# turpaultn/DCASE2019_task4

Measured on AMD Instinct MI355X. Metric: 10-s clips/sec mean-teacher train step (64-mel x 628), higher is better.
Workload: dtype f32

## Files before the change

dcase2019_task4_amd/_lib.py:

```python
import ctypes as C
import os

_HERE = os.path.dirname(os.path.abspath(__file__))
LIB_PATH = os.path.join(_HERE, "libdcase_sed_mi355.so")
if os.environ.get("SED_LIB"):
    if os.environ.get("SED_ALLOW_VARIANT") != "1":
        raise ImportError("SED_LIB is set but SED_ALLOW_VARIANT != 1: refusing to load a variant build of the library")
    LIB_PATH = os.environ["SED_LIB"]


class SedError(RuntimeError):
    pass


class SedDims(C.Structure):
    _fields_ = [("B", C.c_int32), ("T", C.c_int32), ("F", C.c_int32), ("C", C.c_int32), ("H", C.c_int32),
                ("nclass", C.c_int32), ("n_layers_rnn", C.c_int32), ("p_drop", C.c_float),
                ("bn_eps", C.c_float), ("bn_momentum", C.c_float), ("dtype", C.c_int32)]


FORK_CALLBACK = C.CFUNCTYPE(None, C.c_void_p)
DTYPE_F32, DTYPE_BF16, DTYPE_BF16X3, DTYPE_F16 = 0, 1, 2, 3
FFT_F64, FFT_F32 = 0, 1
FFT_DTYPES = {"f64": FFT_F64, "float64": FFT_F64, "f32": FFT_F32, "float32": FFT_F32}
DTYPES = {"f32": DTYPE_F32, "fp32": DTYPE_F32, "float32": DTYPE_F32, "bf16": DTYPE_BF16, "bfloat16": DTYPE_BF16,
          "bf16x3": DTYPE_BF16X3, "f16": DTYPE_F16, "fp16": DTYPE_F16, "float16": DTYPE_F16}


class SedStepState(C.Structure):
    _fields_ = [("global_step", C.c_int64), ("opt_step", C.c_int64), ("rampup_length", C.c_int64),
                ("base_seed", C.c_uint64), ("seed_student", C.c_uint64), ("seed_teacher", C.c_uint64),
                ("lr", C.c_double), ("beta1", C.c_double), ("beta2", C.c_double), ("eps", C.c_double),
                ("ema_decay", C.c_double), ("max_cons_cost", C.c_double),
                ("cons_weight", C.c_float), ("ema_alpha", C.c_float), ("adam_step_size", C.c_float),
                ("adam_sqrt_bc2", C.c_float)]


_P = C.c_void_p
_SIGS = {
    "sed_last_error": (C.c_char_p, []),
    "sed_resample": (C.c_int, [C.c_void_p, C.c_int, C.c_int, C.c_double, C.c_void_p, C.c_int, C.c_int, C.c_void_p, C.c_void_p,
                               C.c_int, C.c_void_p]),
    "sed_scaler_stats": (C.c_int, [C.c_void_p, C.c_longlong, C.c_int, C.c_void_p, C.c_void_p]),
    "sed_postprocess": (C.c_int, [C.c_void_p, C.c_int, C.c_int, C.c_int, C.c_float, C.c_int, C.c_void_p, C.c_void_p,
                                  C.c_void_p, C.c_int, C.c_void_p]),
    "sed_stitch_decode_ws_bytes": (C.c_size_t, [C.c_longlong, C.c_int, C.c_int]),
    "sed_stitch_tile_frames": (C.c_int, []),
    "sed_stitch_decode": (C.c_int, [_P, _P, _P, C.c_int, C.c_int, C.c_int, C.c_int, C.c_int, _P, _P, _P, _P, _P, _P, C.c_longlong,
                                    _P, C.c_size_t, _P, _P]),
    "sed_stitch_sweep_ws_bytes": (C.c_size_t, [C.c_longlong, C.c_int, C.c_int, C.c_int]),
    "sed_stitch_sweep_point_group": (C.c_int, []),
    "sed_stitch_sweep": (C.c_int, [_P, _P, _P, C.c_int, C.c_int, C.c_int, C.c_int, C.c_int, C.c_int, _P, _P, _P, _P, _P,
                                   C.c_longlong, _P, C.c_size_t, _P, _P]),
    "sed_event_counts": (C.c_int, [_P, C.c_int, C.c_int, C.c_int, C.c_int, _P, _P, C.c_double, C.c_double, _P, _P, _P, _P, _P, _P,
                                   C.c_double, C.c_double, C.c_double, _P, _P, _P, _P, _P, _P]),
    "sed_psds_counts": (C.c_int, [_P, C.c_int, C.c_int, C.c_int, C.c_int, _P, _P, C.c_double, C.c_double, _P, _P, _P, _P, _P, _P,
                                  C.c_double, C.c_double, C.c_double, _P, _P, _P, _P]),
    "sed_long_score_ws_bytes": (C.c_size_t, [C.c_longlong, C.c_longlong, C.c_int, C.c_int]),
    "sed_long_tile_events": (C.c_int, []),
    "sed_long_event_counts": (C.c_int, [_P, _P, C.c_double, C.c_double, _P, _P, C.c_longlong, _P, _P, _P, C.c_longlong, C.c_int,
                                        C.c_int, C.c_double, C.c_double, C.c_double, _P, _P, _P, _P, _P, _P, C.c_size_t, _P]),
    "sed_long_psds_counts": (C.c_int, [_P, _P, C.c_double, C.c_double, _P, _P, C.c_longlong, _P, _P, _P, C.c_longlong, C.c_int,
                                       C.c_int, C.c_double, C.c_double, C.c_double, _P, _P, _P, _P, C.c_size_t, _P]),
    "sed_long_sweep_ws_bytes": (C.c_size_t, [C.c_longlong, C.c_longlong, C.c_int, C.c_int, C.c_int]),
    "sed_long_sweep_event_counts": (C.c_int, [_P, _P, C.c_double, C.c_double, _P, _P, C.c_longlong, _P, _P, _P, C.c_longlong,
                                              C.c_int, C.c_int, C.c_int, C.c_double, C.c_double, C.c_double, _P, _P, _P, _P, _P,
                                              _P, C.c_size_t, _P]),
    "sed_long_sweep_psds_counts": (C.c_int, [_P, _P, C.c_double, C.c_double, _P, _P, C.c_longlong, _P, _P, _P, C.c_longlong,
                                             C.c_int, C.c_int, C.c_int, C.c_double, C.c_double, C.c_double, _P, _P, _P, _P,
                                             C.c_size_t, _P]),
    "sed_weak_counts": (C.c_int, [_P, _P, C.c_int, C.c_int, _P, C.c_int, _P, _P]),
    "sed_version": (C.c_int, []),
    "sed_param_count": (C.c_int, [C.POINTER(SedDims)]),
    "sed_param_layout": (C.c_int, [C.POINTER(SedDims), C.POINTER(C.c_int64)]),
    "sed_crnn_ctx_bytes": (C.c_size_t, [C.POINTER(SedDims)]),
    "sed_crnn_bwd_ws_bytes": (C.c_size_t, [C.POINTER(SedDims)]),
    "sed_crnn_forward": (C.c_int, [C.POINTER(SedDims), _P, _P, _P, _P, C.c_int, C.c_int, _P, _P, C.c_size_t, _P, _P, _P]),
    "sed_crnn_moments": (C.c_int, [C.POINTER(SedDims), _P, _P, C.c_size_t, _P]),
    "sed_crnn_backward": (C.c_int, [C.POINTER(SedDims), _P, _P, _P, _P, C.c_size_t, _P, _P, _P, _P, C.c_size_t, C.c_int, _P]),
    "sed_crnn_buffers_init": (C.c_int, [C.POINTER(SedDims), _P, C.c_size_t, _P, C.c_size_t, _P]),
    "sed_crnn_ctx_view": (C.c_int, [C.POINTER(SedDims), C.c_char_p, C.POINTER(C.c_size_t), C.POINTER(C.c_size_t)]),
    "sed_mt_loss": (C.c_int, [C.POINTER(SedDims), _P, _P, _P, _P, _P, C.c_int, C.c_int, C.c_int, C.c_int, _P, _P, _P, _P, _P]),
    "sed_mt_loss_backward": (C.c_int, [C.POINTER(SedDims), _P, _P, _P, _P, C.c_size_t, _P, _P, _P, C.c_int, C.c_int, C.c_int,
                                       C.c_int, _P, C.c_int, _P, _P, _P, _P, _P, C.c_size_t, C.c_int, _P]),
    "sed_mt_step_backward": (C.c_int, [C.POINTER(SedDims), _P, _P, _P, _P, C.c_size_t, _P, _P, _P, _P, _P, C.c_int, C.c_int, C.c_int,
                                       C.c_int, _P, C.c_int, _P, _P, _P, _P, _P, C.c_size_t, C.c_int, _P]),
    "sed_p2p_buffer_bytes": (C.c_size_t, [C.c_longlong]),
    "sed_p2p_alloc": (C.c_int, [C.c_size_t, C.c_int, C.POINTER(C.c_void_p), _P, C.POINTER(C.c_int)]),
    "sed_p2p_open": (C.c_int, [_P, C.POINTER(C.c_void_p)]),
    "sed_p2p_close": (C.c_int, [_P]),
    "sed_p2p_free": (C.c_int, [_P]),
    "sed_p2p_can_access": (C.c_int, [C.c_int]),
    "sed_p2p_errors": (C.c_int, [_P, C.POINTER(C.c_uint)]),
    "sed_p2p_configure": (C.c_int, [_P, C.c_double, _P, C.c_int]),
    "sed_p2p_allreduce": (C.c_int, [_P, C.c_longlong, C.c_int, C.c_int, C.POINTER(C.c_void_p), C.c_longlong, C.c_int, _P]),
    "sed_adam_ema": (C.c_int, [C.c_int64, _P, _P, _P, _P, _P, _P, C.c_float, _P]),
    "sed_ema_update": (C.c_int, [C.c_int64, _P, _P, C.c_float, _P]),
    "sed_step_state_init": (C.c_int, [_P, C.c_uint64, C.c_int64, C.c_double, C.c_double, C.c_double, C.c_double,
                                      C.c_double, C.c_double, _P]),
    "sed_step_state_advance": (C.c_int, [_P, _P]),
    "sed_step_state_update": (C.c_int, [_P, C.c_uint64, C.c_double, C.c_int, _P]),
    "sed_step_state_set_global_step": (C.c_int, [_P, C.c_int64, _P]),
    "sed_stream_prepare": (C.c_int, [_P]),
    "sed_stream_release": (C.c_int, [_P]),
    "sed_crnn_fork_callback": (C.c_int, [_P, _P, _P]),
    "sed_mel_spec_ws_bytes": (C.c_size_t, [C.c_int, C.c_int, C.c_int, C.c_int, C.c_int]),
    "sed_mel_spec": (C.c_int, [_P, C.c_int, C.c_int, C.c_int, C.c_int, _P, _P, C.c_int, _P, _P, C.c_size_t, _P]),
    "sed_mel_tables": (C.c_int, [C.c_int, _P, _P, C.c_int, _P, C.c_size_t, _P]),
    "sed_mel_frames": (C.c_int, [_P, C.c_int, C.c_int, C.c_int, C.c_int, _P, C.c_int, _P, _P, C.c_size_t, C.c_int, C.c_int, _P]),
    "sed_seed_advance": (C.c_int, [_P, _P]),
    "sed_logmel_transform_ws_bytes": (C.c_size_t, [C.c_int]),
    "sed_logmel_transform": (C.c_int, [_P, C.c_int, C.c_int, C.c_int, C.c_int, _P, _P, _P, _P, _P, _P, C.c_size_t, C.c_int, _P]),
    "sed_gather_logmel_transform": (C.c_int, [_P, _P, _P, C.c_int, C.c_int, _P, C.c_int, C.c_int, C.c_int, _P, _P, _P, _P, _P,
                                              _P, C.c_int, _P, _P, C.c_size_t, C.c_int, _P]),
    "sed_gather_window_logmel_transform": (C.c_int, [_P, _P, _P, C.c_int, C.c_int, _P, C.c_int, C.c_int, C.c_int, C.c_int, _P, _P,
                                                     _P, _P, _P, _P, _P, _P, C.c_int, C.c_int, _P, _P, C.c_size_t, C.c_int, _P]),
    "sed_batch_augment": (C.c_int, [_P, _P, _P, _P, C.c_int, C.c_int, C.c_int, C.c_int, C.c_int, _P, _P, _P, _P]),
    "sed_selftest": (C.c_int, [_P, _P, C.c_size_t, _P]),
    "sed_debug_set": (C.c_int, [C.c_int]),
    "sed_build_flags": (C.c_int, []),
    "sed_kernel_replay": (C.c_int, [C.c_char_p, C.POINTER(SedDims), _P, _P, _P, _P, C.c_size_t, _P, _P, C.c_size_t, _P]),
}

_lib = None


def exported_symbols():
    return sorted(_SIGS)


def lib():
    global _lib
    if _lib is None:
        if not os.path.exists(LIB_PATH):
            raise SedError(
                f"{LIB_PATH} not found: build it with `python -c 'import __graft_entry__ as g; g.build()'` "
                "or `make -C dcase2019_task4_amd/csrc` (needs hipcc). There is no CPU fallback.")
        l = C.CDLL(LIB_PATH)
        for name, (res, args) in _SIGS.items():
            fn = getattr(l, name)
            fn.restype = res
            fn.argtypes = args
        _lib = l
        if os.environ.get("SED_DEBUG"):
            l.sed_debug_set(int(os.environ["SED_DEBUG"]))
    return _lib


def scratch(nbytes, device):
    import torch
    t = torch.empty(nbytes, device=device, dtype=torch.uint8)
    if os.environ.get("SED_POISON") == "1" and nbytes:
        t.fill_(0xFF)
    return t


def check(status, what):
    if status != 0:
        msg = lib().sed_last_error()
        raise SedError(f"{what} failed with status {status}: {msg.decode() if msg else ''}")


def ptr(t):
    if t is None:
        return None
    return C.c_void_p(t.data_ptr())


def stream_ptr():
    import torch
    return C.c_void_p(torch.cuda.current_stream().cuda_stream)


def make_dims(B, T, F=64, C_=64, H=64, nclass=10, n_layers_rnn=2, p_drop=0.5, bn_eps=1e-3, bn_momentum=0.99, dtype=DTYPE_F32):
    return SedDims(B, T, F, C_, H, nclass, n_layers_rnn, p_drop, bn_eps, bn_momentum, dtype)


def param_layout(dims):
    l = lib()
    n = l.sed_param_count(C.byref(dims))
    if n <= 0:
        raise SedError(f"sed_param_count: {l.sed_last_error().decode()}")
    off = (C.c_int64 * (n + 1))()
    check(l.sed_param_layout(C.byref(dims), off), "sed_param_layout")
    return list(off)
```

dcase2019_task4_amd/crnn.py:

```python
import ctypes as C
import warnings

import torch
import torch.nn as nn

from . import _lib


class GLU(nn.Module):

    def __init__(self, input_num):
        super().__init__()
        self.sigmoid = nn.Sigmoid()
        self.linear = nn.Linear(input_num, input_num)

    def forward(self, x):
        lin = self.linear(x.permute(0, 2, 3, 1)).permute(0, 3, 1, 2)
        return lin * self.sigmoid(x)


class ContextGating(nn.Module):

    def __init__(self, input_num):
        super().__init__()
# ... 150 lines not shown
        self._C, self._H = int(self.cnn.nb_filters[-1]), int(n_RNN_cell)
        self._dtype = _lib.DTYPE_F32
        self.set_mfma_dtype(mfma_dtype)
        self._flat = None
        self._bn_flat = None
        self._bn_tracked = None
        self._layout = None
        self._flat_gen = 0
        self._last_ctx = None
        self._seed_base = None
        self._seed_calls = 0

    def load_cnn(self, parameters):
        self.cnn.load(parameters)
        if not self.train_cnn:
            for param in self.cnn.parameters():
                param.requires_grad = False

    def load(self, filename=None, parameters=None):
        if filename is not None:
            parameters = torch.load(filename)
        if parameters is None:
            raise NotImplementedError("load is a filename or a list of parameters (state_dict)")
        self.cnn.load(parameters=parameters["cnn"])
        self.rnn.load_state_dict(parameters["rnn"])
        self.dense.load_state_dict(parameters["dense"])
        if "dense_softmax" in parameters and self.attention:
            self.dense_softmax.load_state_dict(parameters["dense_softmax"])

    def state_dict(self, destination=None, prefix='', keep_vars=False):
        sd = {"cnn": self.cnn.state_dict(destination=destination, prefix=prefix, keep_vars=keep_vars),
              "rnn": self.rnn.state_dict(destination=destination, prefix=prefix, keep_vars=keep_vars),
              "dense": self.dense.state_dict(destination=destination, prefix=prefix, keep_vars=keep_vars)}
        if self.attention:
            sd["dense_softmax"] = self.dense_softmax.state_dict(destination=destination, prefix=prefix, keep_vars=keep_vars)
        return sd

    def save(self, filename):
        torch.save({k: v for k, v in self.state_dict().items()}, filename)

    def set_mfma_dtype(self, name):
        if name not in _lib.DTYPES:
            raise ValueError(f"mfma_dtype must be one of {sorted(_lib.DTYPES)}, got {name!r}")
        self._dtype = _lib.DTYPES[name]
        return self

    def make_dims(self, B, T, F=64, p_drop=None):
        if not self.hot_path:
            raise _lib.SedError("this CRNN configuration is outside the MI355X hot path (CRNN.hot_path is False): it runs on stock "
                                "torch operators through forward() only - no flat buffers, no fused step, no HIP inference")
        return _lib.make_dims(B, T, F, self._C, self._H, self._nclass, self._n_layers,
                              self._p_drop if p_drop is None else p_drop, 1e-3, 0.99, self._dtype)

    def _dims(self, x):
        B, _, T, F = x.shape
        return self.make_dims(B, T, F)

    def _bn_modules(self):
        return [getattr(self.cnn.cnn, f"batchnorm{i}") for i in range(3)]

    def flatten_parameters_(self, device=None):
        params = list(self.parameters())
        device = device if device is not None else params[0].device
        if self._layout is None:
            offs = _lib.param_layout(self.make_dims(1, 16, 64, 0.0))
            assert len(offs) == len(params) + 1, "parameter order does not match sed_param_layout"
            self._layout = [(offs[i], offs[i + 1], tuple(p.shape)) for i, p in enumerate(params)]
            for (o0, o1, shp), p in zip(self._layout, params):
                assert o1 - o0 == p.numel(), "parameter shape does not match sed_param_layout"
        ok = self._flat is not None and self._flat.device == device
        if ok:
            base = self._flat.data_ptr()
            for (o0, _, _), p in zip(self._layout, params):
                if p.data_ptr() != base + 4 * o0 or p.device != device or p.dtype != torch.float32:
                    ok = False
                    break
            bns = self._bn_modules()
            Cn = self._C
            for i, bn in enumerate(bns):
                if bn.running_mean.data_ptr() != self._bn_flat.data_ptr() + 4 * (2 * i) * Cn or \
                        bn.running_var.data_ptr() != self._bn_flat.data_ptr() + 4 * (2 * i + 1) * Cn or \
                        bn.num_batches_tracked.data_ptr() != self._bn_tracked.data_ptr() + 8 * i:
                    ok = False
                    break
        if ok:
            return
        with torch.no_grad():
            total = self._layout[-1][1]
            flat = torch.empty(total, device=device, dtype=torch.float32)
            for (o0, o1, shp), p in zip(self._layout, params):
                flat[o0:o1].copy_(p.data.reshape(-1).to(device=device, dtype=torch.float32))
                p.data = flat[o0:o1].view(shp)
                p.grad = None
            Cn = self._C
            bn_flat = torch.empty(3 * 2 * Cn, device=device, dtype=torch.float32)
            trk = torch.empty(3, device=device, dtype=torch.int64)
            for i, bn in enumerate(self._bn_modules()):
                bn_flat[(2 * i) * Cn:(2 * i + 1) * Cn].copy_(bn.running_mean.to(device))
                bn_flat[(2 * i + 1) * Cn:(2 * i + 2) * Cn].copy_(bn.running_var.to(device))
                trk[i] = bn.num_batches_tracked.to(device)
                bn._buffers["running_mean"] = bn_flat[(2 * i) * Cn:(2 * i + 1) * Cn]
                bn._buffers["running_var"] = bn_flat[(2 * i + 1) * Cn:(2 * i + 2) * Cn]
                bn._buffers["num_batches_tracked"] = trk[i]
            self._flat, self._bn_flat, self._bn_tracked = flat, bn_flat, trk
            self._flat_gen += 1

    def _next_seed(self, device):
        if self._seed_base is None:
            self._seed_base = int(torch.randint(0, 2 ** 62, (1,), dtype=torch.int64).item())
        self._seed_calls += 1
        s = (self._seed_base + 0x9E3779B97F4A7C15 * self._seed_calls) & 0x7FFFFFFFFFFFFFFF
        return torch.tensor([s], dtype=torch.int64, device=device)

    def forward(self, x, seed=None):
        if not self.hot_path:
            return self._stock_forward(x)
        if x.dim() != 4 or x.shape[1] != 1:
            raise ValueError(f"expected input [B, 1, T, F], got {tuple(x.shape)}")
        if not x.is_cuda:
            raise _lib.SedError("CRNN.forward needs a GPU tensor: the HIP path is the only path (no CPU fallback)")
        if x.shape[3] // 64 != 1 or x.shape[3] != 64:
            warnings.warn("Output shape is: {}".format((x.shape[0], x.shape[2] // 8, 64 * (x.shape[3] // 64))))
            raise NotImplementedError("hot path implements freq == 1 after pooling, i.e. 64 mel bins (CRNN.py:64-70)")
        x = x.contiguous().float()
        self.flatten_parameters_(x.device)
        use_drop = self.training and self._p_drop > 0
        seed_t = (seed if seed is not None else self._next_seed(x.device)) if use_drop else None
        params = list(self.parameters())
        strong, weak = _CRNNFunction.apply(self, x, self.training, seed_t, *params)
        return strong, weak

    def _stock_forward(self, x):
        if not self._warned_stock:
            self._warned_stock = True
            warnings.warn("CRNN: this configuration is outside the MI355X hot path (activation='glu', attention=True, 3 x 64 / 128 "
                          "filters, pooling (2,4) x 3, n_RNN_cell 64 / 256): running the reference graph on stock torch operators")
        x = self.cnn(x)
        bs, chan, frames, freq = x.size()
        if freq != 1:
            warnings.warn("Output shape is: {}".format((bs, frames, chan * freq)))
            x = x.permute(0, 2, 1, 3).contiguous().view(bs, frames, chan * freq)
        else:
            x = x.squeeze(-1).permute(0, 2, 1)
        x = self.dropout(self.rnn(x))
        strong = self.sigmoid(self.dense(x))
        if self.attention:
            sof = torch.clamp(self.softmax(self.dense_softmax(x)), min=1e-7, max=1)
            weak = (strong * sof).sum(1) / sof.sum(1)
        else:
            weak = strong.mean(1)
        return strong, weak

    def check_recurrence(self):
        if self._H == 256 and self._last_ctx is not None:
            n = int(self.ctx_view("gru_err").view(torch.int32)[0].item())
            if n:
                raise _lib.SedError(f"cluster GRU recurrence: {n} cross-workgroup waits timed out; the outputs are invalid")

    def ctx_view(self, name):
        cbuf, dims = self._last_ctx
        off, nb = C.c_size_t(), C.c_size_t()
        _lib.check(_lib.lib().sed_crnn_ctx_view(C.byref(dims), name.encode(), C.byref(off), C.byref(nb)), "sed_crnn_ctx_view")
        raw = cbuf[off.value:off.value + nb.value]
        if name in ("mom0", "stat1", "stat2"):
            return raw.view(torch.float64)
        if dims.dtype in (_lib.DTYPE_BF16, _lib.DTYPE_F16) and name in ("p0", "y1", "p1", "y2"):
            return raw.view(torch.bfloat16).float()
        return raw.view(torch.float32)
```

dcase2019_task4_amd/csrc/common.h:

```cpp
#pragma once
#include <hip/hip_runtime.h>
#include <stdint.h>
#include <stddef.h>
#include "../../include/dcase_sed.h"

typedef __attribute__((ext_vector_type(16))) float f32x16;
typedef __attribute__((ext_vector_type(4))) float f32x4;

#define SED_C 64
#define SED_HID 64
#define SED_WAVE 64

void sed_set_error(const char* fmt, ...);
#define SED_CHECK_ARG(cond, msg)                                   \
    do {                                                           \
        if (!(cond)) {                                             \
            sed_set_error("%s:%d: %s", __FILE__, __LINE__, msg);   \
            return SED_ERR_BAD_ARG;                                \
        }                                                          \
    } while (0)
#define SED_CHECK_HIP(expr)                                                                 \
    do {                                                                                    \
        hipError_t _e = (expr);                                                             \
        if (_e != hipSuccess) {                                                             \
            sed_set_error("%s:%d: %s -> %s", __FILE__, __LINE__, #expr, hipGetErrorString(_e)); \
            return SED_ERR_LAUNCH;                                                          \
        }                                                                                   \
    } while (0)
#define SED_CHECK_LAUNCH() SED_CHECK_HIP(hipGetLastError())
struct SedAttrOnce {
    bool done[64] = {};
    bool need() {
        int d = 0;
        if (hipGetDevice(&d) != hipSuccess || d < 0 || d >= 64) return true;
        if (done[d]) return false;
        done[d] = true;
        return true;
    }
};
#define SED_TRY(expr)               \
    do {                            \
        int _s = (expr);            \
        if (_s != SED_OK) return _s; \
    } while (0)

struct Geo {
    int B, T, F, C, H, NC, L;
    int mode;
    bool f16;
    bool generic;
    int H1, W1;
    int H2, W2;
    int T3;
    float p, eps, mom;
};
static inline Geo make_geo(const sed_dims* d) {
    Geo g;
    g.B = d->B; g.T = d->T; g.F = d->F; g.C = d->C; g.H = d->H; g.NC = d->nclass; g.L = d->n_layers_rnn;
    g.f16 = d->dtype == SED_DTYPE_F16;
    g.mode = g.f16 ? SED_DTYPE_BF16 : d->dtype;
    g.generic = !(d->C == 64 && d->H == 64 && d->dtype == SED_DTYPE_F32);
    g.H1 = g.T / 2; g.W1 = g.F / 4;
    g.H2 = g.H1 / 2; g.W2 = g.W1 / 4;
    g.T3 = g.H2 / 2;
    g.p = d->p_drop; g.eps = d->bn_eps; g.mom = d->bn_momentum;
    return g;
}
int sed_validate_dims(const sed_dims* d);

struct ParamOff {
    int64_t conv_w[3], conv_b[3], bn_g[3], bn_b[3], glu_w[3], glu_b[3];
    int64_t w_ih[2][2], w_hh[2][2], b_ih[2][2], b_hh[2][2];
    int64_t dense_w, dense_b, soft_w, soft_b;
    int64_t total;
    int count;
};
ParamOff make_param_off(const Geo& g, int64_t* offsets_out );

struct CtxLayout {
    size_t acc0;
    size_t mom0, wz0, wl0, bn0;
    size_t mompart;
    size_t wpkT1, wpkT2;
    size_t p0;
    size_t wpk1, y1, stat1, bn1, p1;
    size_t wpk2, y2, stat2, bn2, p2;
    size_t gates[2], out[2];
    size_t logits_s, strong_sv, weak_sv, den_sv;
    size_t mask0, mask1, mask2;
    size_t total;
};
CtxLayout make_ctx_layout(const Geo& g);

struct WsLayout {
    size_t d_out, dgi[2], dgh[2], hprev[2], d_in, heads_part;
    size_t dz2, dp1, dz1, dp0, dp2;
    size_t bwd_acc;
    size_t pad0;
    size_t gluacc1, gluacc2, coef[3], wg_part, de0, gemm_part;
    size_t total;
    int wgrad_blocks;
};
WsLayout make_ws_layout(const Geo& g);
#define SED_WGRAD_MAX_BLOCKS 256
#ifndef SED_GRU_SPLITK
#define SED_GRU_SPLITK 16
#endif
#define SED_GLUACC_N 4296
#define SED_WINO_OFF (9 * 4096)

__device__ __forceinline__ float wave_sum(float v) {
#pragma unroll
    for (int o = 32; o > 0; o >>= 1) v += __shfl_xor(v, o);
    return v;
}
__device__ __forceinline__ float wave_max(float v) {
#pragma unroll
    for (int o = 32; o > 0; o >>= 1) v = fmaxf(v, __shfl_xor(v, o));
    return v;
}
__device__ __forceinline__ void lds_barrier() { asm volatile("s_waitcnt lgkmcnt(0)\n\ts_barrier" ::: "memory"); }
__device__ __forceinline__ float rcp_fast(float x) { return __builtin_amdgcn_rcpf(x); }
__device__ __forceinline__ float sigmoidf_fast(float x) { return rcp_fast(1.0f + __expf(-x)); }
#define SED_NEG_LOG2E (-1.4426950408889634f)
__device__ __forceinline__ float sigmoid_from_scaled(float e) { return rcp_fast(1.0f + __builtin_amdgcn_exp2f(e)); }
struct TileWalk { int first, end, step; };
__device__ __forceinline__ TileWalk xcd_walk(int n_tiles) {
    const int w = blockIdx.x, g = (int)gridDim.x;
#ifndef SED_NO_XCD_ORDER
    if ((g & 7) == 0) {
        const int chunk = (n_tiles + 7) >> 3, lo = (w & 7) * chunk, hi = lo + chunk < n_tiles ? lo + chunk : n_tiles;
        return {lo + (w >> 3), hi, g >> 3};
    }
#endif
    return {w, n_tiles, g};
}
extern int g_sed_debug;

__device__ __forceinline__ f32x16 mfma32(float a, float b, f32x16 c) {
    return __builtin_amdgcn_mfma_f32_32x32x2f32(a, b, c, 0, 0, 0);
}
__device__ __forceinline__ int mfma32_row(int r, int lane) { return (r & 3) + 8 * (r >> 2) + 4 * (lane >> 5); }


#ifdef SED_TS
#define SED_TS_DEFINE(tag)                                                                                          \
    static __device__ unsigned long long g_ts[1024 * 16];                                                           \
    extern "C" int sed_debug_ts_##tag(unsigned long long* out, int n) {                                             \
        return (int)hipMemcpyFromSymbol(out, HIP_SYMBOL(g_ts), sizeof(unsigned long long) * (n < 1024 * 16 ? n : 1024 * 16)); \
    }
#define TS(k) do { if (threadIdx.x == 0 && blockIdx.x < 1024 && blockIdx.y == 0) g_ts[blockIdx.x * 16 + (k)] = wall_clock64(); } while (0)
#define TSC(k) do { if (threadIdx.x == 0 && blockIdx.x < 1024 && blockIdx.y == 0) g_ts[blockIdx.x * 16 + (k)] = clock64(); } while (0)
#else
#define SED_TS_DEFINE(tag)
#define TS(k) do { } while (0)
#define TSC(k) do { } while (0)
#endif
```

dcase2019_task4_amd/csrc/crnn.hip:

```cpp
#include <stdarg.h>
#include <map>
#include <mutex>
#include <utility>
#include <stdio.h>
#include <string.h>
#include "common.h"
#include "kernels.h"
#include "gkernels.h"
#include "rnn.h"

static thread_local char g_err[512] = "";
void sed_set_error(const char* fmt, ...) {
    va_list ap;
    va_start(ap, fmt);
    vsnprintf(g_err, sizeof(g_err), fmt, ap);
    va_end(ap);
}
extern "C" const char* sed_last_error(void) { return g_err; }
extern "C" int sed_version(void) { return 100; }
int g_sed_debug = 0;
extern "C" int sed_debug_set(int flags) { const int old = g_sed_debug; g_sed_debug = flags; return old; }

int sed_validate_dims(const sed_dims* d) {
    SED_CHECK_ARG(d != nullptr, "null dims");
    if (d->F != 64 || (d->C != 64 && d->C != 128) || (d->H != 64 && d->H != 256) ||
        (d->dtype != SED_DTYPE_F32 && d->dtype != SED_DTYPE_BF16 && d->dtype != SED_DTYPE_BF16X3 && d->dtype != SED_DTYPE_F16)) {
        sed_set_error("supported: F = 64, C in {64, 128}, H in {64, 256}, dtype in {f32, bf16, bf16x3, f16} (got F=%d C=%d H=%d dtype=%d)",
                      d->F, d->C, d->H, d->dtype);
        return SED_ERR_UNSUPPORTED;
    }
    SED_CHECK_ARG(d->B >= 1 && d->T >= 16, "need B >= 1 and T >= 16");
    SED_CHECK_ARG(d->nclass >= 1 && d->nclass <= 16, "nclass must be in [1, 16]");
    SED_CHECK_ARG(d->n_layers_rnn == 1 || d->n_layers_rnn == 2, "n_layers_rnn must be 1 or 2");
    SED_CHECK_ARG(d->p_drop >= 0.f && d->p_drop < 1.f, "p_drop must be in [0, 1)");
    SED_CHECK_ARG((int64_t)d->B * d->T * d->F * d->C < (1ll << 31), "batch too large for 32-bit pixel indices");
    return SED_OK;
}

ParamOff make_param_off(const Geo& g, int64_t* out) {
    ParamOff P;
    int64_t o = 0;
    int k = 0;
    auto put = [&](int64_t& field, int64_t n) {
        field = o;
        if (out) out[k] = o;
        ++k;
        o += n;
    };
    for (int i = 0; i < 3; ++i) {
        const int cin = (i == 0) ? 1 : g.C;
        put(P.conv_w[i], (int64_t)g.C * cin * 9);
        put(P.conv_b[i], g.C);
        put(P.bn_g[i], g.C);
        put(P.bn_b[i], g.C);
        put(P.glu_w[i], (int64_t)g.C * g.C);
        put(P.glu_b[i], g.C);
    }
    for (int l = 0; l < g.L; ++l) {
        const int nin = (l == 0) ? g.C : 2 * g.H;
        for (int dir = 0; dir < 2; ++dir) {
            put(P.w_ih[l][dir], (int64_t)3 * g.H * nin);
            put(P.w_hh[l][dir], (int64_t)3 * g.H * g.H);
            put(P.b_ih[l][dir], 3 * g.H);
            put(P.b_hh[l][dir], 3 * g.H);
        }
    }
    put(P.dense_w, (int64_t)g.NC * 2 * g.H);
    put(P.dense_b, g.NC);
    put(P.soft_w, (int64_t)g.NC * 2 * g.H);
    put(P.soft_b, g.NC);
    P.total = o;
    P.count = k;
    if (out) out[k] = o;
    return P;
}

static inline size_t al(size_t x) { return (x + 255) & ~(size_t)255; }

CtxLayout make_ctx_layout(const Geo& g) {
    CtxLayout L;
    size_t o = 0;
    auto put = [&](size_t& f, size_t bytes) { f = o; o = al(o + bytes); };
    const size_t n0 = (size_t)g.B * g.H1 * g.W1 * 64, n1 = (size_t)g.B * g.H2 * g.W2 * 64, n2 = (size_t)g.B * g.T3 * 64;
    put(L.acc0, 320 * sizeof(double));
    L.mom0 = L.acc0; L.stat1 = L.acc0 + 64 * sizeof(double); L.stat2 = L.acc0 + 192 * sizeof(double);
    put(L.wz0, 64 * 12 * 4); put(L.wl0, 64 * 12 * 4); put(L.bn0, 256 * 4);
    put(L.mompart, (size_t)x_moments_parts(g) * 54 * sizeof(double));
    put(L.p0, n0 * 4);
    put(L.wpk1, (9 + 16) * 4096 * 4); put(L.wpkT1, (9 + 16) * 4096 * 4); put(L.y1, n0 * 4); put(L.bn1, 256 * 4); put(L.p1, n1 * 4);
    put(L.wpk2, (9 + 16) * 4096 * 4); put(L.wpkT2, (9 + 16) * 4096 * 4); put(L.y2, n1 * 4); put(L.bn2, 256 * 4); put(L.p2, n2 * 4);
    const size_t bt = (size_t)g.B * g.T3;
    for (int l = 0; l < 2; ++l) {
        put(L.gates[l], bt * 512 * 4); put(L.out[l], bt * 128 * 4);
    }
    put(L.logits_s, bt * g.NC * 4); put(L.strong_sv, bt * g.NC * 4);
    put(L.weak_sv, (size_t)g.B * g.NC * 4); put(L.den_sv, (size_t)g.B * g.NC * 4);
    auto mask_bytes = [](size_t Q) { return ((Q + 3) / 4) * 2 * 64 * sizeof(uint16_t); };
    put(L.mask0, mask_bytes((size_t)g.B * g.H1 * g.W1)); put(L.mask1, mask_bytes((size_t)g.B * g.H2 * g.W2));
    put(L.mask2, mask_bytes((size_t)g.B * g.T3));
    L.total = o;
    return L;
}

WsLayout make_ws_layout(const Geo& g) {
    WsLayout W;
    size_t o = 0;
    auto put = [&](size_t& f, size_t bytes) { f = o; o = al(o + bytes); };
    const size_t n0 = (size_t)g.B * g.H1 * g.W1 * 64, n1 = (size_t)g.B * g.H2 * g.W2 * 64, bt = (size_t)g.B * g.T3;
    put(W.d_out, bt * 128 * 4);
    for (int l = 0; l < 2; ++l) { put(W.dgi[l], bt * 384 * 4); put(W.dgh[l], bt * 384 * 4); put(W.hprev[l], bt * 128 * 4); }
    put(W.d_in, 2 * bt * 128 * 4); put(W.heads_part, (size_t)g.B * 2 * (g.NC * 128 + g.NC) * 4);
    put(W.dp2, 2 * bt * 64 * 4); put(W.dz2, n1 * 4); put(W.dp1, n1 * 4); put(W.dz1, n0 * 4); put(W.dp0, n0 * 4);
    put(W.pad0, 256 * sizeof(double)); W.coef[0] = 0; put(W.coef[1], 192 * 4); put(W.coef[2], 192 * 4);
    put(W.bwd_acc, (2 * SED_GLUACC_N + 2 * 64 * 10) * sizeof(double));
    W.gluacc1 = W.bwd_acc; W.gluacc2 = W.bwd_acc + SED_GLUACC_N * sizeof(double); W.de0 = W.bwd_acc + 2 * SED_GLUACC_N * sizeof(double);
    W.wgrad_blocks = SED_WGRAD_MAX_BLOCKS;
    put(W.wg_part, (size_t)W.wgrad_blocks * 9 * 4096 * 4);
    put(W.gemm_part, gemm_part_floats(4, SED_GRU_SPLITK, 192, 129) * 4);
    W.total = o;
    return W;
}

extern "C" int sed_param_count(const sed_dims* d) {
    if (sed_validate_dims(d) != SED_OK) return -1;
    const Geo g = make_geo(d);
    return make_param_off(g, nullptr).count;
}
extern "C" int sed_param_layout(const sed_dims* d, int64_t* offsets) {
    SED_TRY(sed_validate_dims(d));
    SED_CHECK_ARG(offsets != nullptr, "null offsets");
    const Geo g = make_geo(d);
    make_param_off(g, offsets);
    return SED_OK;
}
extern "C" size_t sed_crnn_ctx_bytes(const sed_dims* d) {
    if (sed_validate_dims(d) != SED_OK) return 0;
    const Geo g = make_geo(d);
    return g.generic ? gen_ctx_bytes(g) : make_ctx_layout(g).total;
}
extern "C" size_t sed_crnn_bwd_ws_bytes(const sed_dims* d) {
    if (sed_validate_dims(d) != SED_OK) return 0;
    const Geo g = make_geo(d);
    return g.generic ? gen_ws_bytes(g) : make_ws_layout(g).total;
}

extern "C" int sed_crnn_buffers_init(const sed_dims* d, void* ctx, size_t ctx_bytes, void* ws, size_t ws_bytes, void* stream) {
    SED_TRY(sed_validate_dims(d));
    const Geo g = make_geo(d);
    if (g.generic) return gen_buffers_init(g, ctx, ctx_bytes, ws, ws_bytes, (hipStream_t)stream);
    return SED_OK;
}

extern "C" int sed_crnn_ctx_view(const sed_dims* d, const char* name, size_t* offset, size_t* bytes) {
    SED_TRY(sed_validate_dims(d));
    SED_CHECK_ARG(name && offset && bytes, "null argument");
    const Geo g = make_geo(d);
    if (g.generic) return gen_ctx_view(g, name, offset, bytes);
    const CtxLayout L = make_ctx_layout(g);
    const size_t n0 = (size_t)g.B * g.H1 * g.W1 * 64 * 4, n1 = (size_t)g.B * g.H2 * g.W2 * 64 * 4, bt = (size_t)g.B * g.T3;
    struct { const char* n; size_t o, b; } tab[] = {
        {"mom0", L.mom0, 64 * 8}, {"wz0", L.wz0, 64 * 12 * 4}, {"wl0", L.wl0, 64 * 12 * 4}, {"bn0", L.bn0, 1024},
        {"p0", L.p0, n0}, {"y1", L.y1, n0}, {"stat1", L.stat1, 1024}, {"bn1", L.bn1, 1024}, {"p1", L.p1, n1},
        {"y2", L.y2, n1}, {"stat2", L.stat2, 1024}, {"bn2", L.bn2, 1024}, {"p2", L.p2, bt * 64 * 4},
        {"gates0", L.gates[0], bt * 512 * 4}, {"gates1", L.gates[1], bt * 512 * 4},
        {"gru0", L.out[0], bt * 128 * 4}, {"gru1", L.out[1], bt * 128 * 4},
        {"logits_s", L.logits_s, bt * g.NC * 4}, {"den", L.den_sv, (size_t)g.B * g.NC * 4},
    };
    for (auto& t : tab)
        if (strcmp(t.n, name) == 0) { *offset = t.o; *bytes = t.b; return SED_OK; }
    sed_set_error("sed_crnn_ctx_view: unknown buffer '%s'", name);
    return SED_ERR_BAD_ARG;
}

struct SideStream {
    hipStream_t s = nullptr;
    hipEvent_t fork = nullptr, join = nullptr;
    hipStream_t idle = nullptr;
    hipEvent_t idle_ev = nullptr;
    bool ok = false;
};
static std::mutex g_side_mu;
static std::map<std::pair<int, hipStream_t>, SideStream*> g_side;
struct ForkHook { void (*fn)(void*) = nullptr; void* user = nullptr; };
static std::map<std::pair<int, hipStream_t>, ForkHook> g_fork_hooks;
static SideStream& side_stream(hipStream_t caller) {
    static SideStream none;
    int dev = 0;
    if (hipGetDevice(&dev) != hipSuccess) return none;
    std::lock_guard<std::mutex> lk(g_side_mu);
    SideStream*& slot = g_side[std::make_pair(dev, caller)];
    if (slot == nullptr) {
        slot = new SideStream();
        if (hipStreamCreateWithFlags(&slot->s, hipStreamNonBlocking) == hipSuccess &&
            hipEventCreateWithFlags(&slot->fork, hipEventDisableTiming) == hipSuccess &&
            hipEventCreateWithFlags(&slot->join, hipEventDisableTiming) == hipSuccess &&
            hipStreamCreateWithFlags(&slot->idle, hipStreamNonBlocking) == hipSuccess &&
            hipEventCreateWithFlags(&slot->idle_ev, hipEventDisableTiming) == hipSuccess)
            slot->ok = true;
    }
    return *slot;
}
extern "C" int sed_stream_prepare(void* stream) {
    SideStream& sd = side_stream((hipStream_t)stream);
    if (!sd.ok) {
        sed_set_error("sed_stream_prepare: could not create the helper stream / events");
        return SED_ERR_LAUNCH;
    }
    return SED_OK;
}
extern "C" int sed_stream_release(void* stream) {
    int dev = 0;
    SED_CHECK_HIP(hipGetDevice(&dev));
    SideStream* sd = nullptr;
    {
        std::lock_guard<std::mutex> lk(g_side_mu);
        const auto key = std::make_pair(dev, (hipStream_t)stream);
        auto it = g_side.find(key);
        if (it != g_side.end()) { sd = it->second; g_side.erase(it); }
        g_fork_hooks.erase(key);
    }
    if (sd == nullptr) return SED_OK;
    int rc = SED_OK;
    auto note = [&](hipError_t e) { if (e != hipSuccess && rc == SED_OK) { sed_set_error("sed_stream_release: %s", hipGetErrorString(e)); rc = SED_ERR_LAUNCH; } };
    if (sd->s) { note(hipStreamSynchronize(sd->s)); note(hipStreamDestroy(sd->s)); }
    if (sd->idle) note(hipStreamDestroy(sd->idle));
    if (sd->fork) note(hipEventDestroy(sd->fork));
    if (sd->join) note(hipEventDestroy(sd->join));
    if (sd->idle_ev) note(hipEventDestroy(sd->idle_ev));
    delete sd;
    return rc;
}
extern "C" int sed_crnn_fork_callback(void* stream, void (*fn)(void*), void* user) {
    int dev = 0;
    SED_CHECK_HIP(hipGetDevice(&dev));
    std::lock_guard<std::mutex> lk(g_side_mu);
    const auto key = std::make_pair(dev, (hipStream_t)stream);
    if (fn == nullptr) { g_fork_hooks.erase(key); return SED_OK; }
    ForkHook& h = g_fork_hooks[key];
    h.fn = fn;
    h.user = user;
    return SED_OK;
}
int sed_fork_point(hipStream_t st) {
    int dev = 0;
    if (hipGetDevice(&dev) != hipSuccess) return SED_OK;
    ForkHook h;
    {
        std::lock_guard<std::mutex> lk(g_side_mu);
        auto it = g_fork_hooks.find(std::make_pair(dev, st));
        if (it == g_fork_hooks.end()) return SED_OK;
        h = it->second;
        g_fork_hooks.erase(it);
    }
    if (h.fn) h.fn(h.user);
    return SED_OK;
}
static SideFork side_fork(hipStream_t st) {
    SideStream& sd = side_stream(st);
    const bool ok = sd.ok && !(g_sed_debug & SED_DEBUG_NO_SIDE_STREAM);
    return SideFork{ok ? sd.s : st, sd.fork, sd.join, ok, false};
}

#define CTXF(off) ((float*)((char*)ctx + (off)))
#define CTXD(off) ((double*)((char*)ctx + (off)))
#define WSF(off) ((float*)((char*)ws + (off)))
#define WSD(off) ((double*)((char*)ws + (off)))
#define CTXM(off) ((uint16_t*)((char*)ctx + (off)))

static RnnBufs rnn_bufs(const CtxLayout& L, void* ctx, const WsLayout* Wp, void* ws) {
    RnnBufs R;
    R.p2 = CTXF(L.p2);
    for (int l = 0; l < 2; ++l) { R.out[l] = CTXF(L.out[l]); R.gates[l] = CTXF(L.gates[l]); }
    R.logits_s = CTXF(L.logits_s); R.strong_sv = CTXF(L.strong_sv); R.weak_sv = CTXF(L.weak_sv); R.den_sv = CTXF(L.den_sv);
    if (ws == nullptr) return R;
    const WsLayout& W = *Wp;
    R.d_out = WSF(W.d_out); R.d_in = WSF(W.d_in); R.dp2 = WSF(W.dp2); R.heads_part = WSF(W.heads_part);
    for (int l = 0; l < 2; ++l) { R.dgi[l] = WSF(W.dgi[l]); R.dgh[l] = WSF(W.dgh[l]); R.hprev[l] = WSF(W.hprev[l]); }
    R.gemm_part = WSF(W.gemm_part); R.gemm_part_floats = gemm_part_floats(4, SED_GRU_SPLITK, 192, 129); R.splitk = SED_GRU_SPLITK;
    R.zero = WSD(W.bwd_acc); R.n_zero = 2 * SED_GLUACC_N + 2 * 64 * 10;
    return R;
}

extern "C" int sed_crnn_forward(const sed_dims* d, const float* params, float* bn_running, int64_t* bn_tracked,
                                const float* x, int train, int update_bn, const uint64_t* seed_dev, void* ctx,
                                size_t ctx_bytes, float* strong, float* weak, void* stream) {
    SED_TRY(sed_validate_dims(d));
    SED_CHECK_ARG(params && bn_running && x && ctx, "sed_crnn_forward: null argument");
    const int mom_ready = (train & 4) ? 1 : 0;
    train &= 3;
    SED_CHECK_ARG((strong && weak) || (!strong && !weak && train), "sed_crnn_forward: strong and weak must both be given (or both NULL in train mode: heads deferred)");
    const Geo g = make_geo(d);
    const ParamOff P = make_param_off(g, nullptr);
    if (g.generic) {
        SED_CHECK_ARG(!(train && g.p > 0.f) || seed_dev, "sed_crnn_forward: dropout enabled but seed_dev is null");
        side_stream((hipStream_t)stream);
        return gen_forward(g, P, params, bn_running, bn_tracked, x, train | (mom_ready ? 4 : 0), update_bn, seed_dev, ctx, ctx_bytes, strong,
                           weak, (hipStream_t)stream);
    }
    const CtxLayout L = make_ctx_layout(g);
    if (ctx_bytes < L.total) {
        sed_set_error("sed_crnn_forward: ctx has %zu bytes, needs %zu", ctx_bytes, L.total);
        return SED_ERR_WORKSPACE;
    }
    const int use_drop = (train && g.p > 0.f) ? 1 : 0;
    SED_CHECK_ARG(!use_drop || seed_dev, "sed_crnn_forward: dropout enabled but seed_dev is null");
    hipStream_t st = (hipStream_t)stream;
    const int upd = (train && update_bn) ? 1 : 0;
    int64_t* trk[3] = {bn_tracked ? bn_tracked + 0 : nullptr, bn_tracked ? bn_tracked + 1 : nullptr,
                       bn_tracked ? bn_tracked + 2 : nullptr};

    const ConvPackArgs pack = {params + P.conv_w[1], params + P.conv_w[2], CTXF(L.wpk1), CTXF(L.wpk2),
                               train ? CTXF(L.wpkT1) : nullptr, train ? CTXF(L.wpkT2) : nullptr, CTXD(L.stat1), train ? 256 : 0};
    SED_TRY(launch_blk0_forward(g, x, params + P.conv_w[0], params + P.conv_b[0], params + P.bn_g[0], params + P.bn_b[0],
                                params + P.glu_w[0], params + P.glu_b[0], bn_running + 0, bn_running + 64, trk[0], train,
                                upd, seed_dev, CTXD(L.mom0), CTXD(L.mompart), CTXF(L.wz0), CTXF(L.wl0), CTXF(L.bn0), CTXF(L.p0),
                                use_drop ? CTXM(L.mask0) : nullptr, train ? &pack : nullptr, st, 0, nullptr, nullptr, mom_ready));
    if (!train) SED_TRY(launch_conv_pack(pack, st));
    const float* in = CTXF(L.p0);
    const size_t wpk[3] = {0, L.wpk1, L.wpk2}, yo[3] = {0, L.y1, L.y2}, so[3] = {0, L.stat1, L.stat2},
                 bo[3] = {0, L.bn1, L.bn2}, po[3] = {0, L.p1, L.p2}, mo[3] = {L.mask0, L.mask1, L.mask2};
    const int Hs[3] = {0, g.H1, g.H2}, Ws[3] = {0, g.W1, g.W2};
    for (int i = 1; i <= 2; ++i) {
        SED_TRY(launch_conv_fwd(in, CTXF(wpk[i]), params + P.conv_b[i], CTXF(yo[i]), train ? CTXD(so[i]) : nullptr, 0, g.B,
                                Hs[i], Ws[i], st));
        SED_TRY(launch_glu_pool_fwd(CTXF(yo[i]), CTXD(so[i]), (double)g.B * Hs[i] * Ws[i], params + P.bn_g[i], params + P.bn_b[i],
                                    bn_running + (2 * i) * 64, bn_running + (2 * i + 1) * 64, trk[i], train, upd, g.eps, g.mom,
                                    CTXF(bo[i]), params + P.glu_w[i], params + P.glu_b[i], CTXF(po[i]), g.B, Hs[i], Ws[i], i,
                                    use_drop, g.p, seed_dev, use_drop ? CTXM(mo[i]) : nullptr, st));
        in = CTXF(po[i]);
    }
    return rnn_forward(g, P, params, rnn_bufs(L, ctx, nullptr, nullptr), train, seed_dev, strong, weak, 0, st);
}

extern "C" int sed_crnn_moments(const sed_dims* d, const float* x, void* ctx, size_t ctx_bytes, void* stream) {
    SED_TRY(sed_validate_dims(d));
    SED_CHECK_ARG(x && ctx, "sed_crnn_moments: null argument");
    const Geo g = make_geo(d);
    double* mompart = nullptr;
    if (g.generic) {
        SED_TRY(gen_mompart(g, ctx, ctx_bytes, &mompart));
    } else {
        const CtxLayout L = make_ctx_layout(g);
        if (ctx_bytes < L.total) {
            sed_set_error("sed_crnn_moments: ctx has %zu bytes, needs %zu", ctx_bytes, L.total);
            return SED_ERR_WORKSPACE;
        }
        mompart = CTXD(L.mompart);
    }
    return launch_x_moments(g, x, mompart, nullptr, (hipStream_t)stream);
}

static int crnn_backward_impl(const sed_dims* d, const float* params, const float* x, const uint64_t* seed_dev,
                              void* ctx, size_t ctx_bytes, const float* d_strong, const float* d_weak, float* grads,
                              void* ws, size_t ws_bytes, int parts, void* stream, const HeadsLoss* hl,
                              const HeadsOut* ho = nullptr) {
    SED_TRY(sed_validate_dims(d));
    SED_CHECK_ARG(params && x && ctx && (hl || (d_strong && d_weak)) && grads && ws, "sed_crnn_backward: null argument");
    SED_CHECK_ARG(parts == 1 || parts == 2 || parts == 3 || parts == 5 || parts == 8,
                  "sed_crnn_backward: parts must be 1, 2, 3, 5 or 8");
    const Geo g = make_geo(d);
    const ParamOff P = make_param_off(g, nullptr);
    if (g.generic) {
        SED_CHECK_ARG(!(g.p > 0.f) || seed_dev, "sed_crnn_backward: dropout enabled but seed_dev is null");
        SideFork side0 = side_fork((hipStream_t)stream);
        return gen_backward(g, P, params, x, seed_dev, ctx, ctx_bytes, d_strong, d_weak, grads, ws, ws_bytes, parts, (hipStream_t)stream,
                            side0, hl, ho);
    }
    const CtxLayout L = make_ctx_layout(g);
    const WsLayout W = make_ws_layout(g);
    if (ctx_bytes < L.total || ws_bytes < W.total) {
        sed_set_error("sed_crnn_backward: ctx %zu/%zu bytes, ws %zu/%zu bytes", ctx_bytes, L.total, ws_bytes, W.total);
        return SED_ERR_WORKSPACE;
    }
    const int use_drop = (g.p > 0.f) ? 1 : 0;
    SED_CHECK_ARG(!use_drop || seed_dev, "sed_crnn_backward: dropout enabled but seed_dev is null");
    hipStream_t st = (hipStream_t)stream;
    const int BT = g.B * g.T3;
    SideFork side = side_fork(st);
    const RnnBwd rb = rnn_backward_plan(g, P, rnn_bufs(L, ctx, &W, ws), params, grads, seed_dev, hl, ho, parts, &side);
    SED_TRY(rnn_backward(rb, d_strong, d_weak, st));
    if (!(parts & 2)) return SED_OK;
    const size_t wpkT[3] = {0, L.wpkT1, L.wpkT2}, yo[3] = {0, L.y1, L.y2}, bo[3] = {0, L.bn1, L.bn2};
    const size_t pin[3] = {0, L.p0, L.p1}, gacc[3] = {0, W.gluacc1, W.gluacc2}, mo[3] = {L.mask0, L.mask1, L.mask2};
    const size_t dzo[3] = {0, W.dz1, W.dz2}, dpo[3] = {W.dp0, W.dp1, W.dp2};
    const int Hs[3] = {0, g.H1, g.H2}, Wd[3] = {0, g.W1, g.W2};
    if (!(parts & 1)) SED_CHECK_HIP(hipMemsetAsync(WSD(W.bwd_acc), 0, (2 * SED_GLUACC_N + 2 * 64 * 10) * sizeof(double), st));
    const bool fuse_prep = (g_sed_debug & (SED_DEBUG_DIRECT_CONV | SED_DEBUG_DIRECT_WGRAD)) == 0;
    BnBwdPrepArgs prep[3] = {};
    for (int i = 2; i >= 1; --i) {
        const BnBwdPrepArgs* pp = fuse_prep ? &prep[i] : nullptr;
        SED_TRY(launch_glu_pool_bwd(CTXF(yo[i]), CTXF(bo[i]), params + P.glu_w[i], params + P.glu_b[i], WSF(dpo[i]),
                                    i == 2 ? WSF(dpo[i]) + (size_t)BT * 64 : nullptr,
                                    WSF(dzo[i]), WSD(gacc[i]), 0, g.B, Hs[i], Wd[i], use_drop, g.p, CTXM(mo[i]),
                                    params + P.bn_g[i], WSF(W.coef[i]), grads + P.bn_g[i], grads + P.bn_b[i],
                                    grads + P.glu_w[i], grads + P.glu_b[i], grads + P.conv_b[i], fuse_prep ? &prep[i] : nullptr, st));
        SED_TRY(side.mark(st));
        if (i == 1) SED_TRY(side.start());
        SED_TRY(launch_conv_dgrad(WSF(dzo[i]), CTXF(yo[i]), WSF(W.coef[i]), CTXF(wpkT[i]), WSF(dpo[i - 1]), g.B, Hs[i], Wd[i], pp, st));
        if (i == 2) SED_TRY(side.start());
        SED_TRY(launch_conv_wgrad(WSF(dzo[i]), CTXF(yo[i]), WSF(W.coef[i]), CTXF(pin[i]), WSF(W.wg_part), W.wgrad_blocks,
                                  grads + P.conv_w[i], g.B, Hs[i], Wd[i], pp, side.s));
        if (i == 2) SED_TRY(rnn_deferred_weight_grads(rb));
        if (i == 1) SED_TRY(rnn_tail_weight_grads(rb));
    }
    SED_TRY(launch_blk0_backward(g, x, params + P.conv_w[0], params + P.conv_b[0], params + P.bn_g[0], params + P.bn_b[0],
                                 params + P.glu_w[0], CTXM(L.mask0), CTXD(L.mom0), CTXF(L.wz0), CTXF(L.wl0), CTXF(L.bn0),
                                 WSF(W.dp0), WSD(W.de0), 0, grads + P.conv_w[0], grads + P.conv_b[0], grads + P.bn_g[0],
                                 grads + P.bn_b[0], grads + P.glu_w[0], grads + P.glu_b[0], st));
    return side.join(st);
}

extern "C" int sed_crnn_backward(const sed_dims* d, const float* params, const float* x, const uint64_t* seed_dev,
                                 void* ctx, size_t ctx_bytes, const float* d_strong, const float* d_weak, float* grads,
                                 void* ws, size_t ws_bytes, int parts, void* stream) {
    return crnn_backward_impl(d, params, x, seed_dev, ctx, ctx_bytes, d_strong, d_weak, grads, ws, ws_bytes, parts, stream, nullptr);
}

extern "C" int sed_mt_loss_backward(const sed_dims* d, const float* params, const float* x, const uint64_t* seed_dev,
                                    void* ctx, size_t ctx_bytes, const float* strong_ema, const float* weak_ema,
                                    const float* target, int weak_lo, int weak_hi, int strong_lo, int strong_hi,
                                    sed_step_state* state_dev, int advance_state, float* losses, float* d_strong,
                                    float* d_weak, float* grads, void* ws, size_t ws_bytes, int parts, void* stream) {
    SED_CHECK_ARG(d && strong_ema && weak_ema && target && state_dev && losses, "sed_mt_loss_backward: null argument");
    SED_CHECK_ARG(parts == 1 || parts == 3 || parts == 5, "sed_mt_loss_backward: parts must include the heads (1, 3 or 5)");
    SED_CHECK_ARG(weak_lo >= 0 && weak_hi <= d->B && weak_lo <= weak_hi && strong_lo >= 0 && strong_hi <= d->B &&
                      strong_lo <= strong_hi, "sed_mt_loss_backward: bad mask range");
// ... 103 lines not shown
```

dcase2019_task4_amd/csrc/gcrnn.hip:

```cpp
#include <string.h>
#include "common.h"
#include "kernels.h"
#include "gkernels.h"
#include "gpack.h"
#include "rnn.h"

static inline size_t al(size_t x) { return (x + 255) & ~(size_t)255; }
static inline size_t esz(const Geo& g) { return g.mode == SED_DTYPE_BF16 ? 2 : 4; }
static inline int gru_splitk(const Geo& g) { return g.H == 64 ? SED_GRU_SPLITK : 4; }
static inline size_t gru_gemm_part_floats(const Geo& g) {
    int max_n = g.H > g.C ? g.H : g.C;
    if (g.L > 1 && 2 * g.H > max_n) max_n = 2 * g.H;
    return gemm_part_floats(4, gru_splitk(g), 3 * g.H, max_n + 1);
}

struct GCtx {
    size_t acc0, mom0, stat1, stat2;
    size_t wz0, wl0, bn0, mompart, p0;
    size_t wpk[3], wpkT[3], wg[3], wgT[3], bg[3], y[3], bn[3], p[3];
    size_t ph[2], yh[3];
    size_t gi[2], gates[2], out[2], whh[2], whhT[2];
    size_t wihT[2];
    size_t xch[2], epoch[2], err;
    size_t logits_s, strong_sv, weak_sv, den_sv;
    size_t mask[3];
    size_t sg0;
    size_t total;
};
static inline bool blk0_saves_gates(const Geo& g) { return g.mode == SED_DTYPE_BF16 && (g_sed_debug & SED_DEBUG_SAVED_GATES); }
static size_t mask_bytes(size_t Q, int C) { return ((Q + 3) / 4) * (size_t)(C / 32) * 64 * sizeof(uint16_t); }

static GCtx make_gctx(const Geo& g) {
    GCtx L;
    size_t o = 0;
    auto put = [&](size_t& f, size_t bytes) { f = o; o = al(o + bytes); };
    const size_t C = g.C, H = g.H, E = esz(g);
    const size_t n0 = (size_t)g.B * g.H1 * g.W1 * C, n1 = (size_t)g.B * g.H2 * g.W2 * C, n2 = (size_t)g.B * g.T3 * C;
    put(L.acc0, (64 + 4 * C) * sizeof(double));
    L.mom0 = L.acc0; L.stat1 = L.acc0 + 64 * sizeof(double); L.stat2 = L.stat1 + 2 * C * sizeof(double);
    put(L.wz0, C * 12 * 4); put(L.wl0, C * 12 * 4); put(L.bn0, 4 * C * 4);
    put(L.mompart, (size_t)x_moments_parts(g) * 54 * sizeof(double));
    put(L.p0, n0 * E);
    L.p[0] = L.p0;
    const size_t nn[3] = {0, n0, n1}, np[3] = {n0, n1, n2};
    for (int i = 1; i <= 2; ++i) {
        put(L.wpk[i], 9 * C * C * E); put(L.wpkT[i], 9 * C * C * E); put(L.wg[i], C * C * E); put(L.wgT[i], C * C * E);
        put(L.bg[i], C * 4); put(L.y[i], nn[i] * E); put(L.bn[i], 4 * C * 4); put(L.p[i], np[i] * (i == 2 ? 4 : E));
    }
    L.ph[0] = L.ph[1] = 0; L.yh[0] = L.yh[1] = L.yh[2] = 0;
    if (g.f16) { put(L.ph[0], n0 * 2); put(L.yh[1], n0 * 2); put(L.ph[1], n1 * 2); put(L.yh[2], n1 * 2); }
    const size_t bt = (size_t)g.B * g.T3;
    for (int l = 0; l < 2; ++l) {
        put(L.gi[l], g.H == 64 ? 0 : bt * 6 * H * 4);
        put(L.gates[l], bt * 8 * H * 4); put(L.out[l], bt * 2 * H * 4);
        put(L.whh[l], g.H == 64 ? 0 : 2 * 3 * H * H * 4); put(L.whhT[l], g.H == 64 ? 0 : 2 * 3 * H * H * 4);
        put(L.xch[l], g.H == 256 ? gclu_xch_bytes(g.B, g.H, 0) : 0); put(L.epoch[l], (size_t)2 * g.B * 4);
        put(L.wihT[l], g.H == 64 ? 0 : (size_t)(l == 0 ? C : 2 * H) * 6 * H * 4);
    }
    put(L.err, 256);
    put(L.logits_s, bt * g.NC * 4); put(L.strong_sv, bt * g.NC * 4);
    put(L.weak_sv, (size_t)g.B * g.NC * 4); put(L.den_sv, (size_t)g.B * g.NC * 4);
    put(L.mask[0], mask_bytes((size_t)g.B * g.H1 * g.W1, g.C)); put(L.mask[1], mask_bytes((size_t)g.B * g.H2 * g.W2, g.C));
    put(L.mask[2], mask_bytes((size_t)g.B * g.T3, g.C));
    put(L.sg0, g.mode == SED_DTYPE_BF16 ? mask_bytes((size_t)g.B * g.H1 * g.W1, g.C) * 8 : 0);
    L.total = o;
    return L;
}

struct GWs {
    size_t d_out, dgi[2], dgh[2], hprev[2], d_in, heads_part;
    size_t dp[3], dz[3], coef[3];
    size_t glu_part, glu_part2, de0, wg_part, gemm_part;
    size_t xch[2], epoch[2];
    size_t total;
};
static GWs make_gws(const Geo& g) {
    GWs W;
    size_t o = 0;
    auto put = [&](size_t& f, size_t bytes) { f = o; o = al(o + bytes); };
    const size_t C = g.C, H = g.H, bt = (size_t)g.B * g.T3;
    const size_t n0 = (size_t)g.B * g.H1 * g.W1 * C, n1 = (size_t)g.B * g.H2 * g.W2 * C;
    put(W.d_out, bt * 2 * H * 4);
    for (int l = 0; l < 2; ++l) { put(W.dgi[l], bt * 6 * H * 4); put(W.dgh[l], bt * 6 * H * 4); put(W.hprev[l], bt * 2 * H * 4); }
    put(W.d_in, 2 * bt * 2 * H * 4);
    put(W.heads_part, heads_part_floats(g.B, g.T3, g.NC, 2 * H) * 4);
    const size_t E = esz(g);
    put(W.dp[2], 2 * bt * C * 4); put(W.dz[2], n1 * E); put(W.dp[1], n1 * E); put(W.dz[1], n0 * E); put(W.dp[0], n0 * E);
    W.dz[0] = 0; W.coef[0] = 0;
    put(W.coef[1], 3 * C * 4); put(W.coef[2], 3 * C * 4);
    put(W.glu_part, (size_t)(g.mode == SED_DTYPE_BF16 ? bglu_bwd_grid(g.C, g.B, g.H1, g.W1) : gglu_bwd_grid(g.B, g.H1, g.W1)) * (C * C + 3 * C) * 4);
    put(W.glu_part2, (size_t)GPART_SLICES * (C * C + 3 * C) * 4);
    put(W.de0, 2 * C * 10 * sizeof(double));
    put(W.wg_part, (size_t)gwgrad_slabs(g.C) * 9 * C * C * 4);
    put(W.gemm_part, 2 * gru_gemm_part_floats(g) * 4);
    for (int l = 0; l < 2; ++l) { put(W.xch[l], g.H == 256 ? gclu_xch_bytes(g.B, g.H, 1) : 0); put(W.epoch[l], (size_t)2 * g.B * 4); }
    W.total = o;
    return W;
}

size_t gen_ctx_bytes(const Geo& g) { return make_gctx(g).total; }
size_t gen_ws_bytes(const Geo& g) { return make_gws(g).total; }

int gen_ctx_view(const Geo& g, const char* name, size_t* offset, size_t* bytes) {
    const GCtx L = make_gctx(g);
    const size_t C = g.C, H = g.H, bt = (size_t)g.B * g.T3;
    const size_t n0 = (size_t)g.B * g.H1 * g.W1 * C * esz(g), n1 = (size_t)g.B * g.H2 * g.W2 * C * esz(g);
    struct { const char* n; size_t o, b; } tab[] = {
        {"mom0", L.mom0, 64 * 8}, {"bn0", L.bn0, 4 * C * 4}, {"p0", L.p[0], n0}, {"y1", L.y[1], n0}, {"stat1", L.stat1, 2 * C * 8},
        {"bn1", L.bn[1], 4 * C * 4}, {"p1", L.p[1], n1}, {"y2", L.y[2], n1}, {"stat2", L.stat2, 2 * C * 8}, {"bn2", L.bn[2], 4 * C * 4},
        {"p2", L.p[2], bt * C * 4}, {"gates0", L.gates[0], bt * 8 * H * 4}, {"gates1", L.gates[1], bt * 8 * H * 4},
        {"gru0", L.out[0], bt * 2 * H * 4}, {"gru1", L.out[1], bt * 2 * H * 4}, {"logits_s", L.logits_s, bt * g.NC * 4},
        {"den", L.den_sv, (size_t)g.B * g.NC * 4}, {"gru_err", L.err, 4},
    };
    for (auto& t : tab)
        if (strcmp(t.n, name) == 0) { *offset = t.o; *bytes = t.b; return SED_OK; }
    sed_set_error("sed_crnn_ctx_view: unknown buffer '%s'", name);
    return SED_ERR_BAD_ARG;
}

int gen_buffers_init(const Geo& g, void* ctx, size_t ctx_bytes, void* ws, size_t ws_bytes, hipStream_t st) {
    if (ctx) {
        const GCtx L = make_gctx(g);
        if (ctx_bytes < L.total) { sed_set_error("sed_crnn_buffers_init: ctx has %zu bytes, needs %zu", ctx_bytes, L.total); return SED_ERR_WORKSPACE; }
        for (int l = 0; l < 2; ++l) {
            if (g.H == 256) SED_CHECK_HIP(hipMemsetAsync((char*)ctx + L.xch[l], 0, gclu_xch_bytes(g.B, g.H, 0), st));
            SED_CHECK_HIP(hipMemsetAsync((char*)ctx + L.epoch[l], 0, (size_t)2 * g.B * 4, st));
        }
        SED_CHECK_HIP(hipMemsetAsync((char*)ctx + L.err, 0, 256, st));
    }
    if (ws) {
        const GWs W = make_gws(g);
        if (ws_bytes < W.total) { sed_set_error("sed_crnn_buffers_init: ws has %zu bytes, needs %zu", ws_bytes, W.total); return SED_ERR_WORKSPACE; }
        for (int l = 0; l < 2; ++l) {
            if (g.H == 256) SED_CHECK_HIP(hipMemsetAsync((char*)ws + W.xch[l], 0, gclu_xch_bytes(g.B, g.H, 1), st));
            SED_CHECK_HIP(hipMemsetAsync((char*)ws + W.epoch[l], 0, (size_t)2 * g.B * 4, st));
        }
    }
    return SED_OK;
}

#define CTXF(off) ((float*)((char*)ctx + (off)))
#define CTXD(off) ((double*)((char*)ctx + (off)))
#define CTXV(off) ((void*)((char*)ctx + (off)))
#define CTXM(off) ((uint16_t*)((char*)ctx + (off)))
#define WSF(off) ((float*)((char*)ws + (off)))
#define WSD(off) ((double*)((char*)ws + (off)))

static RnnBufs rnn_bufs(const Geo& g, const GCtx& L, void* ctx, const GWs* Wp, void* ws) {
    RnnBufs R;
    R.p2 = CTXF(L.p[2]);
    R.logits_s = CTXF(L.logits_s); R.strong_sv = CTXF(L.strong_sv); R.weak_sv = CTXF(L.weak_sv); R.den_sv = CTXF(L.den_sv);
    R.err = (int*)CTXV(L.err);
    for (int l = 0; l < 2; ++l) {
        R.out[l] = CTXF(L.out[l]); R.gates[l] = CTXF(L.gates[l]);
        R.gi[l] = CTXF(L.gi[l]); R.wihT[l] = CTXF(L.wihT[l]); R.whh[l] = CTXV(L.whh[l]); R.whhT[l] = CTXV(L.whhT[l]);
        R.xch[l] = ws ? (void*)((char*)ws + Wp->xch[l]) : CTXV(L.xch[l]);
        R.epoch[l] = (unsigned int*)(ws ? (void*)((char*)ws + Wp->epoch[l]) : CTXV(L.epoch[l]));
    }
    if (ws == nullptr) return R;
    const GWs& W = *Wp;
    R.d_out = WSF(W.d_out); R.d_in = WSF(W.d_in); R.dp2 = WSF(W.dp[2]); R.heads_part = WSF(W.heads_part);
    for (int l = 0; l < 2; ++l) { R.dgi[l] = WSF(W.dgi[l]); R.dgh[l] = WSF(W.dgh[l]); R.hprev[l] = WSF(W.hprev[l]); }
    R.gemm_part = WSF(W.gemm_part); R.gemm_part_floats = R.gemm_part_stride = gru_gemm_part_floats(g); R.splitk = gru_splitk(g);
    R.zero = WSD(W.de0); R.n_zero = 2 * g.C * 10;
    return R;
}

int gen_mompart(const Geo& g, void* ctx, size_t ctx_bytes, double** out) {
    const GCtx L = make_gctx(g);
    if (ctx_bytes < L.total) {
        sed_set_error("sed_crnn_moments: ctx has %zu bytes, needs %zu", ctx_bytes, L.total);
        return SED_ERR_WORKSPACE;
    }
    *out = (double*)((char*)ctx + L.mompart);
    return SED_OK;
}

int gen_forward(const Geo& g, const ParamOff& P, const float* params, float* bn_running, int64_t* bn_tracked, const float* x,
                int train, int update_bn, const uint64_t* seed_dev, void* ctx, size_t ctx_bytes, float* strong, float* weak,
                hipStream_t st) {
    const int mom_ready = (train & 4) ? 1 : 0;
    train &= 3;
    const GCtx L = make_gctx(g);
    if (ctx_bytes < L.total) {
        sed_set_error("sed_crnn_forward: ctx has %zu bytes, needs %zu", ctx_bytes, L.total);
        return SED_ERR_WORKSPACE;
    }
    const int C = g.C, H = g.H;
    const int use_drop = (train && g.p > 0.f) ? 1 : 0;
    const int upd = (train && update_bn) ? 1 : 0;
    const bool keep_b16 = train && !(train & 2);
    int64_t* trk[3] = {bn_tracked ? bn_tracked + 0 : nullptr, bn_tracked ? bn_tracked + 1 : nullptr,
                       bn_tracked ? bn_tracked + 2 : nullptr};
    GenPackArgs pk = {};
    pk.C = C;
    pk.w1 = params + P.conv_w[1]; pk.w2 = params + P.conv_w[2];
    pk.wpk1 = CTXV(L.wpk[1]); pk.wpk2 = CTXV(L.wpk[2]);
    pk.wpkT1 = train ? CTXV(L.wpkT[1]) : nullptr; pk.wpkT2 = train ? CTXV(L.wpkT[2]) : nullptr;
    pk.glu_w1 = params + P.glu_w[1]; pk.glu_w2 = params + P.glu_w[2]; pk.glu_b1 = params + P.glu_b[1]; pk.glu_b2 = params + P.glu_b[2];
    pk.gamma1 = params + P.bn_g[1]; pk.gamma2 = params + P.bn_g[2]; pk.beta1 = params + P.bn_b[1]; pk.beta2 = params + P.bn_b[2];
    pk.wg1 = CTXV(L.wg[1]); pk.wg2 = CTXV(L.wg[2]);
    pk.wgT1 = train ? CTXV(L.wgT[1]) : nullptr; pk.wgT2 = train ? CTXV(L.wgT[2]) : nullptr;
    pk.bg1 = CTXF(L.bg[1]); pk.bg2 = CTXF(L.bg[2]);
    pk.zero = CTXD(L.stat1); pk.n_zero = train ? 4 * C : 0;
    pk.f16 = g.f16 ? 1 : 0;
    const bool aux_pack = train != 0;
    GenAuxPack aux = {};
    if (aux_pack) {
        aux.pk = pk; aux.mode = g.mode; aux.n_gnt = 0;
        if (H != 64)
            for (int l = 0; l < g.L && l < 2; ++l) {
                aux.gw0[l] = params + P.w_ih[l][0]; aux.gw1[l] = params + P.w_ih[l][1]; aux.gout[l] = CTXF(L.wihT[l]);
                aux.gR[l] = 3 * H; aux.gN[l] = (l == 0) ? C : 2 * H;
                aux.n_gnt = l + 1;
            }
        if (H == 256 && g.mode == SED_DTYPE_BF16)
            for (int l = 0; l < g.L && l < 2; ++l) {
                aux.rw0[l] = params + P.w_hh[l][0]; aux.rw1[l] = params + P.w_hh[l][1];
                aux.rwp[l] = CTXV(L.whh[l]); aux.rwpT[l] = CTXV(L.whhT[l]);
                aux.n_grec = l + 1;
            }
    } else {
        SED_TRY(launch_gen_pack(pk, g.mode, st));
    }

    SED_TRY(launch_blk0_forward(g, x, params + P.conv_w[0], params + P.conv_b[0], params + P.bn_g[0], params + P.bn_b[0],
                                params + P.glu_w[0], params + P.glu_b[0], bn_running + 0, bn_running + C, trk[0], train, upd,
                                seed_dev, CTXD(L.mom0), CTXD(L.mompart), CTXF(L.wz0), CTXF(L.wl0), CTXF(L.bn0),
                                g.f16 ? CTXF(L.ph[0]) : CTXF(L.p[0]),
                                use_drop ? CTXM(L.mask[0]) : nullptr, nullptr, st, 0, aux_pack ? &aux : nullptr,
                                (g.f16 && keep_b16) ? CTXV(L.p[0]) : nullptr, mom_ready,
                                (train && !(train & 2) && blk0_saves_gates(g)) ? CTXV(L.sg0) : nullptr));
    const size_t so[3] = {0, L.stat1, L.stat2};
    const int Hs[3] = {0, g.H1, g.H2}, Wd[3] = {0, g.W1, g.W2};
    auto bn_args = [&](int i) {
        GBnArgs bn;
        bn.stat = CTXD(so[i]); bn.N = (double)g.B * Hs[i] * Wd[i]; bn.gamma = params + P.bn_g[i]; bn.beta = params + P.bn_b[i];
        bn.run_mean = bn_running + (2 * i) * C; bn.run_var = bn_running + (2 * i + 1) * C; bn.tracked = trk[i];
        bn.train = train; bn.update = upd; bn.eps = g.eps; bn.momentum = g.mom; bn.bn = CTXF(L.bn[i]);
        return bn;
    };
    for (int i = 1; i <= 2; ++i) {
        const GBnArgs bn = bn_args(i);
        if (g.f16) {
            SED_TRY(launch_bconv_fwd(2, C, CTXV(L.ph[i - 1]), CTXV(L.wpk[i]), params + P.conv_b[i], CTXV(L.yh[i]),
                                     train ? CTXD(so[i]) : nullptr, g.B, Hs[i], Wd[i], st));
            SED_TRY(launch_bglu_fwd(C, CTXV(L.yh[i]), bn, params + P.glu_w[i], params + P.glu_b[i], i == 1 ? CTXV(L.ph[1]) : CTXV(L.p[2]),
                                    i == 1 ? 1 : 0, g.B, Hs[i], Wd[i], i, use_drop, g.p, seed_dev, use_drop ? CTXM(L.mask[i]) : nullptr,
                                    train ? CTXV(L.wg[i]) : nullptr, train ? CTXF(L.bg[i]) : nullptr, st, 1,
                                    (i == 1 && keep_b16) ? CTXV(L.p[1]) : nullptr, keep_b16 ? CTXV(L.y[i]) : nullptr));
            continue;
        }
        if (g.mode != SED_DTYPE_F32)
            SED_TRY(launch_bconv_fwd(g.mode == SED_DTYPE_BF16X3, C, CTXV(L.p[i - 1]), CTXV(L.wpk[i]), params + P.conv_b[i], CTXV(L.y[i]),
                                     train ? CTXD(so[i]) : nullptr, g.B, Hs[i], Wd[i], st));
        else
            SED_TRY(launch_gconv_fwd(C, CTXF(L.p[i - 1]), CTXV(L.wpk[i]), params + P.conv_b[i], CTXF(L.y[i]),
                                     train ? CTXD(so[i]) : nullptr, g.B, Hs[i], Wd[i], st));
        if (g.mode == SED_DTYPE_BF16)
            SED_TRY(launch_bglu_fwd(C, CTXV(L.y[i]), bn, params + P.glu_w[i], params + P.glu_b[i], CTXV(L.p[i]), i == 1 ? 1 : 0, g.B,
                                    Hs[i], Wd[i], i, use_drop, g.p, seed_dev, use_drop ? CTXM(L.mask[i]) : nullptr,
                                    train ? CTXV(L.wg[i]) : nullptr, train ? CTXF(L.bg[i]) : nullptr, st));
        else if (g.mode == SED_DTYPE_BF16X3)
            SED_TRY(launch_bglu_fwd_x3(C, CTXV(L.y[i]), bn, params + P.glu_w[i], params + P.glu_b[i], CTXV(L.p[i]), g.B, Hs[i], Wd[i], i,
                                       use_drop, g.p, seed_dev, use_drop ? CTXM(L.mask[i]) : nullptr, st));
        else
            SED_TRY(launch_gglu_fwd(C, CTXV(L.y[i]), bn, CTXV(L.wg[i]), CTXF(L.bg[i]), CTXV(L.p[i]), g.B, Hs[i], Wd[i], i, use_drop, g.p,
                                    seed_dev, use_drop ? CTXM(L.mask[i]) : nullptr, st));
    }
// ... 56 lines not shown
```

dcase2019_task4_amd/csrc/gkernels.h:

```cpp
#pragma once
#include "common.h"

struct GenPackArgs {
    int C;
    const float *w1, *w2;
    void *wpk1, *wpk2, *wpkT1, *wpkT2;
    const float *glu_w1, *glu_w2, *glu_b1, *glu_b2, *gamma1, *gamma2, *beta1, *beta2;
    void *wg1, *wg2, *wgT1, *wgT2;
    float *bg1, *bg2;
    double* zero; int n_zero;
    void* pad0;
    int f16;
};
int launch_gen_pack(const GenPackArgs& a, int mode, hipStream_t st);
int launch_gconv_fwd(int C, const float* in, const void* wpk, const float* bias, float* y, double* stat, int B, int H, int W,
                     hipStream_t st);
int launch_gconv_dgrad(int C, const float* dz, const float* yin, const float* coef, const void* wpkT, float* dx, int B, int H,
                       int W, hipStream_t st);
int gwgrad_slabs(int C);
int launch_gwgrad(int mode, int C, const void* dz, const void* yin, const float* coef, const void* xin, float* part, float* g_w, int B,
                  int H, int W, hipStream_t st);

int launch_bconv_fwd(int x3, int C, const void* in, const void* wpk, const float* bias, void* y, double* stat, int B, int H, int W,
                     hipStream_t st, void* y_bf16_copy = nullptr);
int launch_bconv_dgrad(int x3, int C, const void* dz, const void* yin, const float* coef, const void* wpkT, void* dx, int B, int H,
                       int W, hipStream_t st);

struct GBnArgs {
    const double* stat; double N;
    const float *gamma, *beta;
    float *run_mean, *run_var; int64_t* tracked;
    int train, update; float eps, momentum;
    float* bn;
};
int launch_gglu_fwd(int C, const void* y, const GBnArgs& bn, const void* wg, const float* bg, void* p, int B, int H, int W,
                    int block_id, int use_drop, float p_drop, const uint64_t* seed, uint16_t* mask_out, hipStream_t st);
int gglu_bwd_grid(int B, int H, int W);
int launch_gglu_bwd(int C, const void* y, const float* bn, const float* gamma, const float* beta, const void* wg, const void* wgT,
                    const float* bg, const void* dp, void* dz, float* part, int B, int H, int W, int use_drop, float p_drop,
                    const uint16_t* mask_in, hipStream_t st, const float* dp2 = nullptr);
#define GPART_SLICES 8
struct GBnBwdArgs {
    const float* part; int n_part; int C; double N;
    float* part2;
    const float *gamma, *beta, *bn;
    float *coef, *g_gamma, *g_beta, *g_wglu, *g_bglu, *g_convb;
};
int launch_gbn_bwd_prep(const GBnBwdArgs& a, hipStream_t st);

size_t gclu_xch_bytes(int B, int H, int bwd);
int launch_gclu_fwd(const float* gi, const float* w_hh_f, const float* w_hh_r, const float* b_hh_f, const float* b_hh_r, float* out,
                    float* gates, void* xch, unsigned int* epoch, int* err, int B, int T, hipStream_t st);
int launch_gclu_bwd(const float* d_out, const float* out, const float* gates, const float* w_hh_f, const float* w_hh_r, float* dgi,
                    float* dgh, float* hprev, void* xch, unsigned int* epoch, int* err, int B, int T, hipStream_t st);

int launch_bglu_fwd(int C, const void* y, const GBnArgs& bn, const float* wglu, const float* bglu, void* p, int p_bf16, int B, int H,
                    int W, int block_id, int use_drop, float p_drop, const uint64_t* seed, uint16_t* mask_out, void* wfold_out,
                    float* bfold_out, hipStream_t st, int f16 = 0 , void* p_b16 = nullptr ,
                    void* y_b16 = nullptr );

int launch_bglu_fwd_x3(int C, const void* y, const GBnArgs& bn, const float* wglu, const float* bglu, void* p, int B, int H, int W,
                       int block_id, int use_drop, float p_drop, const uint64_t* seed, uint16_t* mask_out, hipStream_t st);
int bglu_bwd_grid(int C, int B, int H, int W);
int launch_bglu_bwd(int C, const void* y, const float* bn, const void* wfold, const float* bfold, const void* wgT,
                    const void* dp, int dp_bf16, void* dz, float* part, int B, int H, int W, int use_drop, float p_drop,
                    const uint16_t* mask_in, hipStream_t st, const float* dp2 = nullptr);

int launch_grec_pack(const float* w_hh_f, const float* w_hh_r, void* wp, void* wpT , hipStream_t st, int f16 = 0);
int launch_grec_fwd(const float* gi, const void* wp, const float* b_hh_f, const float* b_hh_r, float* out, float* gates, int B, int T,
                    hipStream_t st, int f16 = 0);
int launch_grec_bwd(const float* d_out, const float* out, const float* gates, const void* wpT, float* dgi, float* dgh, float* hprev,
                    int B, int T, hipStream_t st);

struct GntProb { const float* A; int lda; const float* B; int ldb; float* C; int ldc; const float* bias; int M, N, K; };
struct GntBatch { GntProb p[2]; int n_prob; };
int launch_gnt_gemm(const GntBatch& gb, hipStream_t st);
int launch_gnt_gemm_bf16(const GntBatch& gb, hipStream_t st, int x3 = 0);

struct HeadsLoss;
struct SideFork;
size_t gen_ctx_bytes(const Geo& g);
size_t gen_ws_bytes(const Geo& g);
int gen_buffers_init(const Geo& g, void* ctx, size_t ctx_bytes, void* ws, size_t ws_bytes, hipStream_t st);
int gen_ctx_view(const Geo& g, const char* name, size_t* offset, size_t* bytes);
int gen_mompart(const Geo& g, void* ctx, size_t ctx_bytes, double** out);
int gen_forward(const Geo& g, const ParamOff& P, const float* params, float* bn_running, int64_t* bn_tracked, const float* x,
                int train, int update_bn, const uint64_t* seed_dev, void* ctx, size_t ctx_bytes, float* strong, float* weak,
                hipStream_t st);
int gen_backward(const Geo& g, const ParamOff& P, const float* params, const float* x, const uint64_t* seed_dev, void* ctx,
                 size_t ctx_bytes, const float* d_strong, const float* d_weak, float* grads, void* ws, size_t ws_bytes, int parts,
                 hipStream_t st, SideFork& side, const HeadsLoss* hl, const HeadsOut* ho);
```

dcase2019_task4_amd/csrc/gru4.hip:

```cpp
#include "common.h"
#include "kernels.h"
#include "hfuse.h"
#include <type_traits>
SED_TS_DEFINE(gru4)
#ifdef SED_TS
#define TSW(k, t) do { if (threadIdx.x == (t) && blockIdx.y == 0 && blockIdx.x < 1024) g_ts[blockIdx.x * 16 + (k)] = wall_clock64(); } while (0)
#else
#define TSW(k, t) do { } while (0)
#endif

typedef float v2f __attribute__((ext_vector_type(2)));
typedef float v4f __attribute__((ext_vector_type(4)));

#define G4_SB 16
#define G4_THREADS 576
#define G4B_THREADS 640
#define G4_HS 452

__device__ __forceinline__ float g4_tanh(float x) { return 1.0f - 2.0f * rcp_fast(1.0f + __expf(2.0f * x)); }
__device__ __forceinline__ v2f g4_pkfma(v2f a, v2f b, v2f c) { return __builtin_elementwise_fma(a, b, c); }
__device__ __forceinline__ float g4_quad_sum(float x) {
    x += __int_as_float(__builtin_amdgcn_mov_dpp(__float_as_int(x), 0xB1, 0xF, 0xF, true));
    x += __int_as_float(__builtin_amdgcn_mov_dpp(__float_as_int(x), 0x4E, 0xF, 0xF, true));
    return x;
// ... 319 lines not shown
            for (int a = 3; a < 6; ++a) dgh[bt * 192 + 64 * (a - 3) + l] = v[a];
            hprev_out[bt * 64 + l] = v[6];
        };
        if constexpr (HEADS) {
            float first2[G4_SB / 2];
#pragma unroll
            for (int i = 0; i < G4_SB / 2; ++i) {
                bool ok = false;
                pre[6 * i] = op_load(2 * i + io, 0, ok);
                pre_ok |= (ok ? 1ull : 0ull) << (6 * i);
                first2[i] = 0.f;
            }
            ops_store(0, pre, first2, pre_ok);
        } else {
            float first[6 * G4_SB / 2], first2[G4_SB / 2];
            unsigned long long okm;
            ops_load(0, first, first2, okm);
            ops_store(0, first, first2, okm);
        }
        __syncthreads();
        for (int blk = 0; blk < nblk; ++blk) {
            const int s0 = blk * G4_SB, sb = min(G4_SB, T - s0);
            float nxt[6 * G4_SB / 2], nxt2[G4_SB / 2];
            unsigned long long okm = 0;
            const bool more = s0 + G4_SB < T;
            if (more) ops_load(blk + 1, nxt, nxt2, okm);
            for (int s = 0; s < sb; ++s) {
#ifndef G4_EXP_NOIO
                if (blk > 0 && (s & 1) == io) put_row(blk - 1, s);
#endif
                if (s == sb - 1 && more) ops_store(blk + 1, nxt, nxt2, okm);
                lds_barrier();
            }
        }
        {
            const int blk = nblk - 1, sb = T - blk * G4_SB;
            if (blk > 0)
                for (int s = sb + ((sb ^ io) & 1); s < G4_SB; s += 2) put_row(blk - 1, s);
            for (int s = io; s < sb; s += 2) put_row(blk, s);
        }
        TSW(4, 256);
        return;
    }
    if (role >= 6) {
        constexpr int CT = NIN / 64;
        const int gw = role - 6, i16 = l & 15, kq = l >> 4;
        const float* wih = dir ? w_ih_r : w_ih_f;
        float bw[CT][48];
#pragma unroll
        for (int c = 0; c < CT; ++c)
#pragma unroll
            for (int s4 = 0; s4 < 48; ++s4) bw[c][s4] = wih[(size_t)(4 * s4 + kq) * NIN + 16 * (gw * CT + c) + i16];
        float* plane = dx_planes + (size_t)dir * B * T * NIN;
        lds_barrier();
        auto gemm_block = [&](int blk, int n_sync, auto sync_tag) {
            constexpr bool SYNC = decltype(sync_tag)::value;
            const int s0 = blk * G4_SB, sb = min(G4_SB, T - s0);
            const float* hp = hist + (blk & 1) * G4_SB * G4_HS + i16 * G4_HS + kq;
            const bool rowok = i16 < sb;
            v4f acc[CT];
#pragma unroll
            for (int c = 0; c < CT; ++c) acc[c] = (v4f){0.f, 0.f, 0.f, 0.f};
#pragma unroll
            for (int s4 = 0; s4 < 48; ++s4) {
                const float a = rowok ? hp[4 * s4] : 0.f;
#ifndef G4_EXP_NODX
#pragma unroll
                for (int c = 0; c < CT; ++c) acc[c] = __builtin_amdgcn_mfma_f32_16x16x4f32(a, bw[c][s4], acc[c], 0, 0, 0);
#endif
                if (SYNC && (s4 + 1) % 3 == 0 && (s4 + 1) / 3 <= n_sync) lds_barrier();
            }
#pragma unroll
            for (int r = 0; r < 4; ++r) {
                const int s = 4 * kq + r;
                if (s < sb) {
                    float* dst = plane + (size_t)(b * T + t_of(s0 + s)) * NIN + 16 * gw * CT + i16;
#pragma unroll
                    for (int c = 0; c < CT; ++c) dst[16 * c] = acc[c][r];
                }
            }
        };
        for (int blk = 0; blk < nblk; ++blk) {
            const int sb = min(G4_SB, T - blk * G4_SB);
            if (blk > 0) gemm_block(blk - 1, sb, std::true_type{});
            else
                for (int s = 0; s < sb; ++s) lds_barrier();
        }
        TSW(5, 384);
        gemm_block(nblk - 1, 0, std::false_type{});
        TSW(6, 384);
        return;
    }
    const int w = role, kq = l >> 4, u = l & 15, j = 16 * w + u;
    const float* whh = dir ? w_hh_r : w_hh_f;
    float (&wt)[48] = pre;
    if constexpr (!HEADS) G4Rot<0>::load_bwd(wt, whh, kq, u, j);
    for (int e = tid; e < 192; e += 256) zero[e] = 0.f;
#pragma unroll
    for (int i = 0; i < 48; ++i) asm volatile("" : "+v"(wt[i]));
    TSW(7, 0);
    __syncthreads();
    TSW(1, 0);
    __builtin_amdgcn_s_setprio(3);
    const int wofs1 = (kq < 3) ? 64 * kq + j : 384 + j;
    const int wofs2 = (kq < 3) ? 192 + 64 * kq + j : 384 + j;
    const int rofs = 48 * kq + u;
    const float* dgrow = zero;
    float dhz = 0.f;
    const bool is1 = kq == 1, is2 = kq == 2, is3 = kq == 3;
    for (int blk = 0; blk < nblk; ++blk) {
        const int cur = blk & 1, sb = min(G4_SB, T - blk * G4_SB);
        const float* ob = ops + cur * G4_SB * 384;
        float* hb = hist + cur * G4_SB * G4_HS;
        float dout = ob[j], r = ob[64 + j], z = ob[128 + j], nn = ob[192 + j], ghn = ob[256 + j], hp = ob[320 + j];
        for (int s = 0; s < sb; ++s) {
            float dgv[3];
#pragma unroll
            for (int m = 0; m < 3; ++m) dgv[m] = dgrow[rofs + 16 * m];
            const float* o = ob + min(s + 1, G4_SB - 1) * 384;
            const float n_dout = o[j], n_r = o[64 + j], n_z = o[128 + j], n_nn = o[192 + j], n_ghn = o[256 + j], n_hp = o[320 + j];
            __builtin_amdgcn_sched_barrier(0);
            float acc[3] = {0.f, 0.f, 0.f};
#ifdef G4_EXP_NOMV
            acc[0] = dgv[0] * wt[0]; acc[1] = dgv[1] * wt[1]; acc[2] = dgv[2] * wt[2];
#else
            G4Rot<0>::dot3(acc, dgv, wt);
#endif
#ifdef G4_EXP_NOSUM
            const float dh = dout + (dhz + ((acc[0] + acc[1]) + acc[2]));
#else
            const float dh = dout + (dhz + g4_row4_sum((acc[0] + acc[1]) + acc[2]));
#endif
            const float dn_pre = dh * (1.0f - z) * (1.0f - nn * nn);
            const float dz_pre = dh * (hp - nn) * z * (1.0f - z);
            const float dr_pre = dn_pre * ghn * r * (1.0f - r);
            const float dghn = dn_pre * r;
            float* ho = hb + s * G4_HS;
            float v1 = dr_pre, v2 = dr_pre;
            v1 = is1 ? dz_pre : v1; v2 = is1 ? dz_pre : v2;
            v1 = is2 ? dn_pre : v1; v2 = is2 ? dghn : v2;
            v1 = is3 ? hp : v1;     v2 = is3 ? hp : v2;
            ho[wofs1] = v1;
            ho[wofs2] = v2;
            dgrow = ho + 192;
            dhz = dh * z;
            dout = n_dout; r = n_r; z = n_z; nn = n_nn; ghn = n_ghn; hp = n_hp;
            lds_barrier();
        }
        if (blk == 0) TSW(2, 0);
    }
    TSW(3, 0);
}

template <int NIN> static constexpr size_t gru4_fwd_lds() { return (size_t)(64 + 2 * G4_SB * 192 + 2 * G4_SB * 320 + 2 * G4_SB * (NIN + 4)) * sizeof(float); }
static const size_t GRU4_BWD_LDS = (size_t)(192 + 2 * G4_SB * 384 + 2 * G4_SB * G4_HS) * sizeof(float);
static_assert(2 * G4_SB * 384 + 2 * G4_SB * G4_HS >= HF_TMAX * HF_S + HF_MAXO * HF_S + HF_TMAX * HF_SD + HF_TMAX * 8 + HF_MISC,
              "the heads phase's scratch must fit the ops / history rings it aliases");
static const size_t GRU4_BWD_HEADS_LDS_MAX = GRU4_BWD_LDS + (size_t)HF_TMAX * 64 * sizeof(float);

int launch_gru_fwd(const float* x, int nin, const float* w_ih_f, const float* w_ih_r, const float* b_ih_f, const float* b_ih_r,
                   const float* w_hh_f, const float* w_hh_r, const float* b_hh_f, const float* b_hh_r, float* out, float* gates,
                   int B, int T, hipStream_t st) {
    static thread_local SedAttrOnce attr_done;
    if (attr_done.need()) {
        SED_CHECK_HIP(hipFuncSetAttribute((const void*)k_gru4_fwd<64>, hipFuncAttributeMaxDynamicSharedMemorySize, (int)gru4_fwd_lds<64>()));
        SED_CHECK_HIP(hipFuncSetAttribute((const void*)k_gru4_fwd<128>, hipFuncAttributeMaxDynamicSharedMemorySize, (int)gru4_fwd_lds<128>()));
    }
    if (nin == 128)
        k_gru4_fwd<128><<<dim3(B, 2), G4_THREADS, gru4_fwd_lds<128>(), st>>>(x, w_ih_f, w_ih_r, b_ih_f, b_ih_r, w_hh_f, w_hh_r, b_hh_f, b_hh_r, out, gates, T);
    else if (nin == 64)
        k_gru4_fwd<64><<<dim3(B, 2), G4_THREADS, gru4_fwd_lds<64>(), st>>>(x, w_ih_f, w_ih_r, b_ih_f, b_ih_r, w_hh_f, w_hh_r, b_hh_f, b_hh_r, out, gates, T);
    else {
        sed_set_error("gru forward: unsupported input width %d", nin);
        return SED_ERR_UNSUPPORTED;
    }
    SED_CHECK_LAUNCH();
    return SED_OK;
}

int launch_gru_bwd(const float* d_out, const float* d_out2, const float* out, const float* gates, const float* w_hh_f,
                   const float* w_hh_r, const float* w_ih_f, const float* w_ih_r, int nin, float* dgi, float* dgh, float* hprev,
                   float* dx_planes, int B, int T, hipStream_t st) {
    static thread_local SedAttrOnce attr_done;
    if (attr_done.need()) {
        SED_CHECK_HIP(hipFuncSetAttribute((const void*)k_gru4_bwd<64, false>, hipFuncAttributeMaxDynamicSharedMemorySize, (int)GRU4_BWD_LDS));
        SED_CHECK_HIP(hipFuncSetAttribute((const void*)k_gru4_bwd<128, false>, hipFuncAttributeMaxDynamicSharedMemorySize, (int)GRU4_BWD_LDS));
    }
    if (nin == 128)
        k_gru4_bwd<128, false><<<dim3(B, 2), G4B_THREADS, GRU4_BWD_LDS, st>>>(d_out, d_out2, out, gates, w_hh_f, w_hh_r, w_ih_f, w_ih_r, dgi, dgh,
                                                                             hprev, dx_planes, B, T, HeadsFuse{});
    else if (nin == 64)
        k_gru4_bwd<64, false><<<dim3(B, 2), G4B_THREADS, GRU4_BWD_LDS, st>>>(d_out, d_out2, out, gates, w_hh_f, w_hh_r, w_ih_f, w_ih_r, dgi, dgh,
                                                                            hprev, dx_planes, B, T, HeadsFuse{});
    else {
        sed_set_error("gru backward: unsupported input width %d", nin);
        return SED_ERR_UNSUPPORTED;
    }
    SED_CHECK_LAUNCH();
    return SED_OK;
}

int launch_gru_bwd_heads(const float* out, const float* gates, const float* w_hh_f, const float* w_hh_r, const float* w_ih_f,
                         const float* w_ih_r, int nin, float* dgi, float* dgh, float* hprev, float* dx_planes, int B, int T,
                         const HeadsFuse& hf, hipStream_t st) {
    if (T > HF_TMAX || hf.NC < 1 || hf.NC > 16 || hf.hl.strong_ema == nullptr) {
        sed_set_error("fused heads + gru backward: needs T/8 <= %d, nclass <= 16 and the loss inputs (got T/8 = %d)", HF_TMAX, T);
        return SED_ERR_UNSUPPORTED;
    }
    static thread_local SedAttrOnce attr_done;
    if (attr_done.need()) {
        SED_CHECK_HIP(hipFuncSetAttribute((const void*)k_gru4_bwd<64, true>, hipFuncAttributeMaxDynamicSharedMemorySize, (int)GRU4_BWD_HEADS_LDS_MAX));
        SED_CHECK_HIP(hipFuncSetAttribute((const void*)k_gru4_bwd<128, true>, hipFuncAttributeMaxDynamicSharedMemorySize, (int)GRU4_BWD_HEADS_LDS_MAX));
    }
    const size_t lds = GRU4_BWD_LDS + (size_t)((T + 15) & ~15) * 64 * sizeof(float);
    if (nin == 128)
        k_gru4_bwd<128, true><<<dim3(B, 2), G4B_THREADS, lds, st>>>(nullptr, nullptr, out, gates, w_hh_f, w_hh_r, w_ih_f, w_ih_r, dgi, dgh,
                                                                    hprev, dx_planes, B, T, hf);
    else if (nin == 64)
        k_gru4_bwd<64, true><<<dim3(B, 2), G4B_THREADS, lds, st>>>(nullptr, nullptr, out, gates, w_hh_f, w_hh_r, w_ih_f, w_ih_r, dgi, dgh,
                                                                   hprev, dx_planes, B, T, hf);
    else {
        sed_set_error("gru backward: unsupported input width %d", nin);
        return SED_ERR_UNSUPPORTED;
    }
    SED_CHECK_LAUNCH();
    return SED_OK;
}
```

dcase2019_task4_amd/csrc/kernels.h:

```cpp
#pragma once
#include "common.h"

struct ConvPackArgs;
int x_moments_parts(const Geo& g);
struct GenAuxPack;
int launch_x_moments(const Geo& g, const float* x, double* mompart, const ConvPackArgs* pack, hipStream_t st,
                     const GenAuxPack* aux = nullptr);
int launch_blk0_forward(const Geo& g, const float* x, const float* w0, const float* b0, const float* gamma,
                        const float* beta, const float* wglu, const float* bglu, float* run_mean, float* run_var,
                        int64_t* tracked, int train, int update, const uint64_t* seed, double* mom, double* mompart,
                        float* wz, float* wl, float* bn, float* p0, uint16_t* mask_out, const ConvPackArgs* pack ,
                        hipStream_t st,
                        int main_kernel_only = 0, const GenAuxPack* aux = nullptr,
                        void* p0_b16 = nullptr ,
                        int mom_ready = 0 ,
                        void* sg_out = nullptr );
int launch_blk0_backward(const Geo& g, const float* x, const float* w0, const float* b0, const float* gamma,
                         const float* beta, const float* wglu, const uint16_t* mask_in, const double* mom,
                         const float* wz, const float* wl, const float* bn, const float* dp0, double* de, int zero_de,
                         float* g_w0, float* g_b0, float* g_gamma, float* g_beta, float* g_wglu, float* g_bglu,
                         hipStream_t st, const void* sg_in = nullptr );

struct ConvPackArgs {
    const float *w1, *w2;
// ... 10 lines not shown
        t[0][b] = g[0][b];
        t[1][b] = 0.5f * (g[0][b] + g[1][b] + g[2][b]);
        t[2][b] = 0.5f * (g[0][b] - g[1][b] + g[2][b]);
        t[3][b] = g[2][b];
    }
    const int kq = k & 3, s4 = k >> 2, sq = s4 >> 2, e = s4 & 3, cg = n >> 4, i16 = n & 15;
#pragma unroll
    for (int i2 = 0; i2 < 4; ++i2) {
        const int ph = i2 >> 1, p8b = (i2 == 0 || i2 == 3) ? 0 : 4;
        float* d = U + ((((size_t)(ph * 4 + cg) * 8 + p8b) * 4 + sq) * 64 + 16 * kq + i16) * 4 + e;
        const size_t pstride = 4 * 64 * 4;
        d[0 * pstride] = t[i2][0];
        d[1 * pstride] = 0.5f * (t[i2][0] + t[i2][1] + t[i2][2]);
        d[2 * pstride] = 0.5f * (t[i2][0] - t[i2][1] + t[i2][2]);
        d[3 * pstride] = t[i2][2];
    }
}
__device__ __forceinline__ void conv_pack_body(const ConvPackArgs& a, int i) {
    if (i < a.n_zero) a.zero[i] = 0.0;
    if (i < 4 * 4096) {
        const int which = i >> 12, kn = i & 4095, k = kn >> 6, n2 = kn & 63;
        const float* w = (which >> 1) ? a.w2 : a.w1;
        float* dst = (which >> 1) ? ((which & 1) ? a.wpkT2 : a.wpk2) : ((which & 1) ? a.wpkT1 : a.wpk1);
        if (dst != nullptr) {
            float g[3][3];
#pragma unroll
            for (int a = 0; a < 3; ++a)
#pragma unroll
                for (int b = 0; b < 3; ++b)
                    g[a][b] = (which & 1) ? w[(k * 64 + n2) * 9 + 3 * (2 - a) + (2 - b)] : w[(n2 * 64 + k) * 9 + 3 * a + b];
            wino_u(g, dst + SED_WINO_OFF, k, n2);
        }
    }
    const int layer = i / (9 * 4096);
    i -= layer * 9 * 4096;
    const float* w = layer ? a.w2 : a.w1;
    float* wpk = layer ? a.wpk2 : a.wpk1;
    float* wpkT = layer ? a.wpkT2 : a.wpkT1;
    const int tap = i / 4096, ci = (i / 64) % 64, co = i % 64;
    wpk[i] = w[(co * 64 + ci) * 9 + tap];
    if (wpkT) {
        const int k = ci, n = co;
        wpkT[i] = w[(k * 64 + n) * 9 + (8 - tap)];
    }
}
#endif

int launch_conv_pack(const ConvPackArgs& a, hipStream_t st);
int launch_conv_fwd(const float* in, const float* wpk, const float* bias, float* y, double* stat, int zero_stat, int B,
                    int H, int W, hipStream_t st);
struct BnBwdPrepArgs {
    const double* acc; double N;
    const float *gamma, *bn;
    float *coef, *g_gamma, *g_beta, *g_wglu, *g_bglu, *g_convb;
};
#ifdef __HIPCC__
__device__ __forceinline__ void bn_bwd_coef(const BnBwdPrepArgs& a, int c, float& ca, float& cb, float& cc) {
    const double mean = a.bn[c], invstd = a.bn[64 + c], scale = a.bn[128 + c];
    const double Sdz = a.acc[4160 + c], Sdzy = a.acc[4224 + c];
    const double Sdzxhat = invstd * (Sdzy - mean * Sdz);
    const double m1 = Sdz / a.N, m2 = Sdzxhat / a.N;
    ca = (float)scale;
    cb = (float)(-scale * m2 * invstd);
    cc = (float)(scale * (m2 * invstd * mean - m1));
}
__device__ __forceinline__ void bn_bwd_prep_body(const BnBwdPrepArgs& a, int tid, int nthreads) {
    if (tid < 64) {
        const int c = tid;
        const double mean = a.bn[c], invstd = a.bn[64 + c];
        const double Sdz = a.acc[4160 + c], Sdzy = a.acc[4224 + c];
        a.g_beta[c] = (float)Sdz;
        a.g_gamma[c] = (float)(invstd * (Sdzy - mean * Sdz));
        float ca, cb, cc;
        bn_bwd_coef(a, c, ca, cb, cc);
        a.coef[c] = ca; a.coef[64 + c] = cb; a.coef[128 + c] = cc;
        a.g_bglu[c] = (float)a.acc[4096 + c];
        a.g_convb[c] = 0.f;
    }
    for (int e = tid; e < 4096; e += nthreads) a.g_wglu[e] = (float)a.acc[e];
}
#endif
int launch_conv_dgrad(const float* dz, const float* yin, const float* coef , const float* wpkT, float* dx,
                      int B, int H, int W, const BnBwdPrepArgs* prep, hipStream_t st);
int launch_conv_wgrad(const float* dz, const float* yin, const float* coef, const float* xin, float* part, int n_blocks,
                      float* g_w , int B, int H, int W, const BnBwdPrepArgs* prep, hipStream_t st);

int launch_glu_pool_fwd(const float* y, const double* stat, double N, const float* gamma, const float* beta, float* run_mean,
                        float* run_var, int64_t* tracked, int train, int update, float eps, float momentum, float* bn ,
                        const float* wglu, const float* bglu, float* p, int B, int H, int W, int block_id, int use_drop,
                        float p_drop, const uint64_t* seed, uint16_t* mask_out, hipStream_t st);
int launch_glu_pool_bwd(const float* y, const float* bn, const float* wglu, const float* bglu, const float* dp, const float* dp_b, float* dz,
                        double* acc, int zero_acc, int B, int H, int W, int use_drop, float p_drop,
                        const uint16_t* mask_in, const float* gamma, float* coef, float* g_gamma, float* g_beta, float* g_wglu,
                        float* g_bglu, float* g_convb, BnBwdPrepArgs* prep_out ,
                        hipStream_t st);

struct GemmProb {
    const float* A; int64_t sAm, sAk;
    const float* B; int64_t sBk, sBn;
    const float* B2; int k2;
    float* C; int64_t ldc;
    const float* bias;
    float* Cones;
    int M, N, K;
    int accumulate;
    int vec_ok;
};
struct GemmBatch {
    GemmProb p[4];
    int n_prob;
    int splits;
    float* part;
    size_t part_floats;
    size_t part_stride;
    int bf16 = 0;
};
static inline GemmProb gemm_prob(const float* A, int64_t sAm, int64_t sAk, const float* B, int64_t sBk, int64_t sBn, float* C,
                                 int64_t ldc, int M, int N, int K) {
    GemmProb q;
    q.A = A; q.sAm = sAm; q.sAk = sAk; q.B = B; q.sBk = sBk; q.sBn = sBn; q.B2 = nullptr; q.k2 = 0;
    q.C = C; q.ldc = ldc; q.bias = nullptr; q.Cones = nullptr; q.M = M; q.N = N; q.K = K; q.accumulate = 0; q.vec_ok = 0;
    return q;
}
size_t gemm_part_floats(int n_prob, int splits, int max_m, int max_nx);
int launch_gemm_batch(GemmBatch& gb, hipStream_t st);
int launch_colsum(const float* A, int M, int N, int64_t lda, float* out, hipStream_t st);

struct GruWgradLayer {
    const float *dgi, *dgh;
    const float* hprev;
    const float* input; int nin;
    float *w_ih[2], *w_hh[2], *b_ih[2], *b_hh[2];
};
struct GruWgradTile {
    const float *A, *B; float *C, *bias;
    int lda, ldb, ldc;
};
#define SED_GRUW_MAX_TILES 36
struct GruWgradArgs {
    GruWgradTile t[SED_GRUW_MAX_TILES];
    int n_tiles, BT;
    float* part;
};
size_t gru_wgrad_part_floats(int n_tiles);
int launch_gru_wgrad(const GruWgradLayer* layers, int n_layers, int BT, float* part, size_t part_floats, hipStream_t st);

int sed_fork_point(hipStream_t st);
int launch_gru_fwd(const float* x, int nin, const float* w_ih_f, const float* w_ih_r, const float* b_ih_f, const float* b_ih_r,
                   const float* w_hh_f, const float* w_hh_r, const float* b_hh_f, const float* b_hh_r, float* out, float* gates,
                   int B, int T, hipStream_t st);
int launch_gru_bwd(const float* d_out, const float* d_out2, const float* out, const float* gates, const float* w_hh_f,
                   const float* w_hh_r, const float* w_ih_f, const float* w_ih_r, int nin, float* dgi, float* dgh, float* hprev,
                   float* dx_planes, int B, int T, hipStream_t st);

int launch_heads_fwd(const float* h , const float* wd, const float* bd, const float* ws, const float* bs,
                     float* strong, float* weak, float* strong_sv, float* weak_sv, float* logits_s, float* den, int B, int T,
                     int NC, int use_drop, float p_drop, const uint64_t* seed, hipStream_t st, int HF = 128);
int launch_heads_colsum(const float* part, float* g_wd, int B, int NC, hipStream_t st, int HF = 128);
#ifdef __HIPCC__
__device__ __forceinline__ uint64_t splitmix64(uint64_t x) {
    x += 0x9E3779B97F4A7C15ull;
    x = (x ^ (x >> 30)) * 0xBF58476D1CE4E5B9ull;
    x = (x ^ (x >> 27)) * 0x94D049BB133111EBull;
    return x ^ (x >> 31);
}
__device__ __forceinline__ void step_state_derive_forward(sed_step_state* s) {
    const int64_t gs = s->global_step;
    double r = 1.0;
    if (gs < s->rampup_length && s->rampup_length > 0) {
        double cur = (double)gs;
        if (cur < 0) cur = 0;
        const double phase = 1.0 - cur / (double)s->rampup_length;
        r = exp(-5.0 * phase * phase);
    }
    s->cons_weight = (float)(s->max_cons_cost * r);
    s->seed_student = splitmix64(s->base_seed + 2ull * (uint64_t)gs * 0x9E3779B97F4A7C15ull + 1ull);
    s->seed_teacher = splitmix64(s->base_seed + (2ull * (uint64_t)gs + 1ull) * 0x9E3779B97F4A7C15ull + 1ull);
}
__device__ __forceinline__ void step_state_derive_update(sed_step_state* s) {
    const int64_t gs = s->global_step;
    const double a = 1.0 - 1.0 / ((double)(gs + 1) + 1.0);
    s->ema_alpha = (float)(a < s->ema_decay ? a : s->ema_decay);
    const double bc1 = 1.0 - pow(s->beta1, (double)s->opt_step);
    const double bc2 = 1.0 - pow(s->beta2, (double)s->opt_step);
    s->adam_step_size = (float)(s->lr / bc1);
    s->adam_sqrt_bc2 = (float)sqrt(bc2);
}
__device__ __forceinline__ void step_state_derive(sed_step_state* s) {
    step_state_derive_forward(s);
    step_state_derive_update(s);
}
__device__ __forceinline__ void step_state_advance_early(sed_step_state* s) {
    step_state_derive_update(s);
    s->global_step += 1;
    s->opt_step += 1;
    step_state_derive_forward(s);
}
#endif

struct HeadsLoss {
    const float* strong_ema; const float* weak_ema; const float* target;
    int wlo, whi, slo, shi;
    const sed_step_state* state;
    float* losses; float* d_strong_out; float* d_weak_out;
    sed_step_state* advance;
};
int launch_heads_bwd(const float* h, const float* wd, const float* ws, const float* strong, const float* weak,
                     const float* logits_s, const float* den, const float* d_strong, const float* d_weak, float* dh,
                     float* part, float* g_wd, float* g_bd, float* g_ws, float* g_bs, int B, int T, int NC, int use_drop,
                     float p_drop, const uint64_t* seed, double* zero, int n_zero, int defer_colsum, const HeadsLoss* hl, hipStream_t st,
                     int HF = 128);

struct HeadsFuse {
    const float* wd;
    float *strong, *weak;
    float* part;
    int NC, use_drop;
    float p_drop;
    const uint64_t* seed;
    double* zero; int n_zero;
    HeadsLoss hl;
};
static inline int heads_bwd_chunks(int HF, int T3) {
    if (HF != 512) return 1;
    const int n = (T3 + 31) / 32;
    return n < 1 ? 1 : (n > 8 ? 8 : n);
}
static inline size_t heads_part_floats(int B, int T3, int NC, int HF) {
    const int ny = heads_bwd_chunks(HF, T3);
    return (size_t)B * ny * 2 * (NC * HF + NC) + (size_t)8 * B * ny;
}
struct HeadsOut { float *strong, *weak; };
static inline bool heads_fusable(int H, int T3) { return H == 64 && T3 <= 128; }
int launch_gru_bwd_heads(const float* out, const float* gates, const float* w_hh_f, const float* w_hh_r, const float* w_ih_f,
                         const float* w_ih_r, int nin, float* dgi, float* dgh, float* hprev, float* dx_planes, int B, int T,
                         const HeadsFuse& hf, hipStream_t st);
int launch_heads_fin(const float* part, float* g_wd, int B, int T, int NC, int n_cols, const HeadsLoss& hl, hipStream_t st);
```

dcase2019_task4_amd/csrc/rnn.hip:

```cpp
#include "rnn.h"
#include "gkernels.h"

int rnn_forward(const Geo& g, const ParamOff& P, const float* params, const RnnBufs& R, int train, const uint64_t* seed_dev,
                float* strong, float* weak, int n_whh_packed, hipStream_t st) {
    const int H = g.H, BT = g.B * g.T3, use_drop = (train && g.p > 0.f) ? 1 : 0;
    const bool rec16 = H == 256 && g.mode == SED_DTYPE_BF16;
    SED_TRY(sed_fork_point(st));
    const float* in = R.p2;
    int nin = g.C;
    for (int l = 0; l < g.L; ++l) {
        if (H == 64) {
            SED_TRY(launch_gru_fwd(in, nin, params + P.w_ih[l][0], params + P.w_ih[l][1], params + P.b_ih[l][0], params + P.b_ih[l][1],
                                   params + P.w_hh[l][0], params + P.w_hh[l][1], params + P.b_hh[l][0], params + P.b_hh[l][1],
                                   R.out[l], train ? R.gates[l] : nullptr, g.B, g.T3, st));
        } else {
            GntBatch gb;
            gb.n_prob = 2;
            for (int dir = 0; dir < 2; ++dir)
                gb.p[dir] = GntProb{in, nin, params + P.w_ih[l][dir], nin, R.gi[l] + dir * 3 * H, 6 * H, params + P.b_ih[l][dir], BT, 3 * H, nin};
            SED_TRY(g.mode != SED_DTYPE_F32 ? launch_gnt_gemm_bf16(gb, st, g.f16 ? 2 : (g.mode == SED_DTYPE_BF16X3 ? 1 : 0)) : launch_gnt_gemm(gb, st));
            if (rec16) {
                if (l >= n_whh_packed)
                    SED_TRY(launch_grec_pack(params + P.w_hh[l][0], params + P.w_hh[l][1], R.whh[l], train ? R.whhT[l] : nullptr, st, g.f16 ? 1 : 0));
                SED_TRY(launch_grec_fwd(R.gi[l], R.whh[l], params + P.b_hh[l][0], params + P.b_hh[l][1], R.out[l],
                                        train ? R.gates[l] : nullptr, g.B, g.T3, st, g.f16 ? 1 : 0));
            } else
                SED_TRY(launch_gclu_fwd(R.gi[l], params + P.w_hh[l][0], params + P.w_hh[l][1], params + P.b_hh[l][0], params + P.b_hh[l][1],
                                        R.out[l], train ? R.gates[l] : nullptr, R.xch[l], R.epoch[l], R.err, g.B, g.T3, st));
        }
        in = R.out[l];
        nin = 2 * H;
    }
    if (strong == nullptr) return SED_OK;
    return launch_heads_fwd(in, params + P.dense_w, params + P.dense_b, params + P.soft_w, params + P.soft_b, strong, weak,
                            train ? R.strong_sv : nullptr, train ? R.weak_sv : nullptr, R.logits_s, R.den_sv, g.B, g.T3, g.NC,
                            use_drop, g.p, seed_dev, st, 2 * H);
}

RnnBwd rnn_backward_plan(const Geo& g, const ParamOff& P, const RnnBufs& R, const float* params, float* grads,
                         const uint64_t* seed_dev, const HeadsLoss* hl, const HeadsOut* ho, int parts, SideFork* side) {
    RnnBwd rb = {g, P, R, params, grads, seed_dev, hl, ho, parts, side, false, false, false};
    rb.fuse = ho && hl && (parts & 1) && heads_fusable(g.H, g.T3) && !(g_sed_debug & SED_DEBUG_SEPARATE_HEADS) && !hl->d_strong_out && !hl->d_weak_out;
    rb.defer_colsum = ((parts & 2) && side->ok) || (parts & 4);
    rb.early_gru_w = parts == 3 && side->ok && g.H != 64;
    return rb;
}

int rnn_weight_grads_layer(const RnnBwd& rb, int l, hipStream_t s2) {
    const Geo& g = rb.g; const ParamOff& P = rb.P; const RnnBufs& R = rb.R;
    const int H = g.H, BT = g.B * g.T3, nin = (l == 0) ? g.C : 2 * H;
    const float* input = (l == 0) ? R.p2 : R.out[l - 1];
    GemmBatch gb;
    gb.n_prob = 4; gb.splits = R.splitk; gb.part = R.gemm_part + (size_t)l * R.gemm_part_stride; gb.part_floats = R.gemm_part_floats; gb.part_stride = 0;
    gb.bf16 = g.mode == SED_DTYPE_BF16 ? 1 : (g.mode == SED_DTYPE_BF16X3 ? 2 : 0);
    for (int dir = 0; dir < 2; ++dir) {
        gb.p[2 * dir] = gemm_prob(R.dgi[l] + dir * 3 * H, 1, 6 * H, input, nin, 1, rb.grads + P.w_ih[l][dir], nin, 3 * H, nin, BT);
        gb.p[2 * dir].Cones = rb.grads + P.b_ih[l][dir];
        gb.p[2 * dir + 1] = gemm_prob(R.dgh[l] + dir * 3 * H, 1, 6 * H, R.hprev[l] + dir * H, 2 * H, 1, rb.grads + P.w_hh[l][dir], H, 3 * H, H, BT);
        gb.p[2 * dir + 1].Cones = rb.grads + P.b_hh[l][dir];
    }
    return launch_gemm_batch(gb, s2);
}
static bool rnn_weight_grads_fused(const Geo& g) { return g.H == 64 && g.mode == SED_DTYPE_F32 && (g.C == 64 || g.C == 128); }
int rnn_weight_grads(const RnnBwd& rb, hipStream_t s2) {
    const Geo& g = rb.g; const ParamOff& P = rb.P; const RnnBufs& R = rb.R;
    if (!rnn_weight_grads_fused(g)) {
        for (int l = g.L - 1; l >= 0; --l) SED_TRY(rnn_weight_grads_layer(rb, l, s2));
        return SED_OK;
    }
    GruWgradLayer ly[2];
    for (int l = 0; l < g.L; ++l) {
        ly[l].dgi = R.dgi[l]; ly[l].dgh = R.dgh[l]; ly[l].hprev = R.hprev[l];
        ly[l].input = (l == 0) ? R.p2 : R.out[l - 1];
        ly[l].nin = (l == 0) ? g.C : 2 * g.H;
        for (int dir = 0; dir < 2; ++dir) {
            ly[l].w_ih[dir] = rb.grads + P.w_ih[l][dir]; ly[l].w_hh[dir] = rb.grads + P.w_hh[l][dir];
            ly[l].b_ih[dir] = rb.grads + P.b_ih[l][dir]; ly[l].b_hh[dir] = rb.grads + P.b_hh[l][dir];
        }
    }
    return launch_gru_wgrad(ly, g.L, g.B * g.T3, R.gemm_part, R.gemm_part_floats + R.gemm_part_stride, s2);
}

int rnn_heads_colsum(const RnnBwd& rb, hipStream_t s2) {
    const Geo& g = rb.g;
    if (rb.fuse)
        return launch_heads_fin(rb.R.heads_part, rb.grads + rb.P.dense_w, g.B, g.T3, g.NC, 2 * (g.NC * 2 * g.H + g.NC), *rb.hl, s2);
    return launch_heads_colsum(rb.R.heads_part, rb.grads + rb.P.dense_w, g.B * heads_bwd_chunks(2 * g.H, g.T3), g.NC, s2, 2 * g.H);
}

static bool rnn_gru_w_at_tail(const RnnBwd& rb) { return rb.parts == 3 && !rb.early_gru_w && !rb.g.generic && rnn_weight_grads_fused(rb.g); }
int rnn_deferred_weight_grads(const RnnBwd& rb) {
    if (rb.parts != 3 || rb.early_gru_w) return SED_OK;
    if (rb.defer_colsum) SED_TRY(rnn_heads_colsum(rb, rb.side->s));
    return rnn_gru_w_at_tail(rb) ? SED_OK : rnn_weight_grads(rb, rb.side->s);
}
int rnn_tail_weight_grads(const RnnBwd& rb) { return rnn_gru_w_at_tail(rb) ? rnn_weight_grads(rb, rb.side->s) : SED_OK; }

int rnn_backward(const RnnBwd& rb, const float* d_strong, const float* d_weak, hipStream_t st) {
    const Geo& g = rb.g; const ParamOff& P = rb.P; const RnnBufs& R = rb.R;
    const float* params = rb.params; float* grads = rb.grads;
    const int H = g.H, BT = g.B * g.T3, parts = rb.parts, use_drop = (g.p > 0.f) ? 1 : 0;
    SideFork& side = *rb.side;
    if (parts & 1) {
        const float* h_last = R.out[g.L - 1];
        if (rb.ho && !rb.fuse)
            SED_TRY(launch_heads_fwd(h_last, params + P.dense_w, params + P.dense_b, params + P.soft_w, params + P.soft_b, rb.ho->strong,
                                     rb.ho->weak, R.strong_sv, R.weak_sv, R.logits_s, R.den_sv, g.B, g.T3, g.NC, use_drop, g.p,
                                     rb.seed_dev, st, 2 * H));
        if (!rb.fuse)
            SED_TRY(launch_heads_bwd(h_last, params + P.dense_w, params + P.soft_w, R.strong_sv, R.weak_sv, R.logits_s, R.den_sv, d_strong,
                                     d_weak, R.d_out, R.heads_part, grads + P.dense_w, grads + P.dense_b, grads + P.soft_w,
                                     grads + P.soft_b, g.B, g.T3, g.NC, use_drop, g.p, rb.seed_dev, (parts & 2) ? R.zero : nullptr,
                                     R.n_zero, rb.defer_colsum ? 1 : 0, rb.hl, st, 2 * H));
        const float* d_cur = R.d_out;
        const float* d_cur2 = nullptr;
        for (int l = g.L - 1; l >= 0; --l) {
            const int nin = (l == 0) ? g.C : 2 * H;
            float* d_in = (l == 0) ? R.dp2 : R.d_in;
            if (H == 64) {
                if (rb.fuse && l == g.L - 1) {
                    HeadsFuse hf = {};
                    hf.wd = params + P.dense_w; hf.strong = rb.ho->strong; hf.weak = rb.ho->weak; hf.part = R.heads_part;
                    hf.NC = g.NC; hf.use_drop = use_drop; hf.p_drop = g.p; hf.seed = rb.seed_dev;
                    hf.zero = (parts & 2) ? R.zero : nullptr; hf.n_zero = (parts & 2) ? R.n_zero : 0; hf.hl = *rb.hl;
                    SED_TRY(launch_gru_bwd_heads(R.out[l], R.gates[l], params + P.w_hh[l][0], params + P.w_hh[l][1], params + P.w_ih[l][0],
                                                 params + P.w_ih[l][1], nin, R.dgi[l], R.dgh[l], R.hprev[l], d_in, g.B, g.T3, hf, st));
                    if (!rb.defer_colsum) SED_TRY(rnn_heads_colsum(rb, st));
                    else if (parts & 4) SED_TRY(launch_heads_fin(R.heads_part, grads + P.dense_w, g.B, g.T3, g.NC, 0, *rb.hl, st));
                } else
                    SED_TRY(launch_gru_bwd(d_cur, d_cur2, R.out[l], R.gates[l], params + P.w_hh[l][0], params + P.w_hh[l][1], params + P.w_ih[l][0],
                                           params + P.w_ih[l][1], nin, R.dgi[l], R.dgh[l], R.hprev[l], d_in, g.B, g.T3, st));
            } else {
                if (g.mode == SED_DTYPE_BF16)
                    SED_TRY(launch_grec_bwd(d_cur, R.out[l], R.gates[l], R.whhT[l], R.dgi[l], R.dgh[l], R.hprev[l], g.B, g.T3, st));
                else
                    SED_TRY(launch_gclu_bwd(d_cur, R.out[l], R.gates[l], params + P.w_hh[l][0], params + P.w_hh[l][1], R.dgi[l], R.dgh[l],
                                            R.hprev[l], R.xch[l], R.epoch[l], R.err, g.B, g.T3, st));
                if (rb.early_gru_w) SED_TRY(side.mark(st));
                GntBatch gb;
                gb.n_prob = 1; gb.p[0] = GntProb{R.dgi[l], 6 * H, R.wihT[l], 6 * H, d_in, nin, nullptr, BT, nin, 6 * H};
                SED_TRY(g.mode != SED_DTYPE_F32 ? launch_gnt_gemm_bf16(gb, st, g.mode == SED_DTYPE_BF16X3) : launch_gnt_gemm(gb, st));
                if (rb.early_gru_w) {
                    SED_TRY(side.start());
                    if (l == g.L - 1) SED_TRY(rnn_heads_colsum(rb, side.s));
                    SED_TRY(rnn_weight_grads_layer(rb, l, side.s));
                }
            }
            d_cur = d_in;
            d_cur2 = (H == 64) ? d_in + (size_t)BT * nin : nullptr;
        }
    }
    if (parts == 1) SED_TRY(rnn_weight_grads(rb, st));
    if (parts == 8) {
        SED_TRY(rnn_heads_colsum(rb, st));
        SED_TRY(rnn_weight_grads(rb, st));
    }
    return SED_OK;
}
```

dcase2019_task4_amd/train.py:

```python
import ctypes as C
import os
import time

import numpy as np
import torch

from . import _lib
from . import dist as sdist
from .crnn import CRNN

LOSS_NAMES = ("loss", "weak_class_loss", "strong_loss", "cons_strong", "cons_weak", "weak_ema_loss",
              "strong_ema_loss", "cons_weight")


def update_ema_variables(model, ema_model, alpha, global_step):
    alpha = min(1 - 1 / (global_step + 1), alpha)
    model.flatten_parameters_()
    ema_model.flatten_parameters_()
    n = model._flat.numel()
    _lib.check(_lib.lib().sed_ema_update(n, _lib.ptr(model._flat), _lib.ptr(ema_model._flat), float(alpha),
                                         _lib.stream_ptr()), "sed_ema_update")


_STREAM_POOL = {}


def shared_stream(device, role, priority=0):
    key = (torch.device(device).index or 0, role, int(priority))
    st = _STREAM_POOL.get(key)
    if st is None:
        st = _STREAM_POOL[key] = torch.cuda.Stream(device=device, priority=int(priority))
    return st


def _slice_range(s, B):
    if s is None:
        return 0, 0
    lo, hi, st = s.indices(B)
    if st != 1:
        raise NotImplementedError("masks must be contiguous slices (main.py:241,247)")
    return lo, max(lo, hi)


class MeanTeacherStep:

    def __init__(self, student, teacher, batch_size, n_frames, rampup_length, weak_mask, strong_mask, lr=1e-3,
                 betas=(0.9, 0.999), eps=1e-8, ema_decay=0.999, max_consistency_cost=2.0, seed=0, use_graph=True,
                 process_group=None, overlap_streams=True, dp_schedule=None, pool_streams=True, collective=None):
        assert isinstance(student, CRNN) and (teacher is None or isinstance(teacher, CRNN))
        if not student.hot_path or (teacher is not None and not teacher.hot_path):
            raise _lib.SedError("MeanTeacherStep runs the HIP hot path only: this CRNN configuration is served by stock torch "
                                "operators (CRNN.hot_path is False) - use the reference's own loop for it")
        self.l = _lib.lib()
        self.student, self.teacher = student, teacher
        self.supervised = teacher is None
        dev = next(student.parameters()).device
        if dev.type != "cuda":
            raise _lib.SedError("MeanTeacherStep needs the models on the GPU (no CPU fallback)")
        self.device = dev
        student.flatten_parameters_(dev)
        if teacher is not None:
            teacher.flatten_parameters_(dev)
        self.B, self.T = int(batch_size), int(n_frames)
        if teacher is not None and (teacher._C, teacher._H, teacher._dtype) != (student._C, student._H, student._dtype):
            raise ValueError("student and teacher must have the same geometry and mfma_dtype")
        self.dims = student.make_dims(self.B, self.T)
        self._pool_streams = bool(pool_streams)
        self._owned_streams = []
        self.T3, self.NC = self.T // 8, student._nclass
        self._defer_heads = (student._H == 64 and self.T3 <= 128)
        if os.environ.get("SED_DEFER_HEADS") in ("0", "1"):
            self._defer_heads = os.environ["SED_DEFER_HEADS"] == "1"
        self.wlo, self.whi = _slice_range(weak_mask, self.B) if weak_mask is not None else (0, 0)
        self.slo, self.shi = _slice_range(strong_mask, self.B) if strong_mask is not None else (0, 0)
        n = student._flat.numel()
        self.n = n
        f32 = dict(device=dev, dtype=torch.float32)
        self.grads = torch.zeros(n, **f32)
        self.exp_avg = torch.zeros(n, **f32)
        self.exp_avg_sq = torch.zeros(n, **f32)
        self.state = torch.zeros(C.sizeof(_lib.SedStepState), device=dev, dtype=torch.uint8)
        self.steps_done = 0
        self._gs_offset = 0
        self.pg = process_group
        self.world, self.rank = 1, 0
        if process_group is not None:
            import torch.distributed as dist
            self.world = dist.get_world_size(process_group)
            self.rank = dist.get_rank(process_group)
        self.seed_user = int(seed) & (2 ** 64 - 1)
        _lib.check(self.l.sed_step_state_init(_lib.ptr(self.state), self._folded_seed(), int(rampup_length),
                                              float(lr), float(betas[0]), float(betas[1]), float(eps),
                                              float(ema_decay), float(max_consistency_cost), _lib.stream_ptr()),
                   "sed_step_state_init")
        self.lr = float(lr)
        base = self.state.data_ptr()
        self._seed_s = C.c_void_p(base + _lib.SedStepState.seed_student.offset)
        self._seed_t = C.c_void_p(base + _lib.SedStepState.seed_teacher.offset)
        self.ctx_bytes = self.l.sed_crnn_ctx_bytes(C.byref(self.dims))
        self.ws_bytes = self.l.sed_crnn_bwd_ws_bytes(C.byref(self.dims))
        if self.ctx_bytes == 0 or self.ws_bytes == 0:
            raise _lib.SedError(self.l.sed_last_error().decode())
        self.ctx_s = _lib.scratch(self.ctx_bytes, dev)
        self.ctx_t = _lib.scratch(self.ctx_bytes if teacher is not None else 0, dev)
        self.ws = _lib.scratch(self.ws_bytes, dev)
        _lib.check(self.l.sed_crnn_buffers_init(C.byref(self.dims), _lib.ptr(self.ctx_s), self.ctx_bytes, _lib.ptr(self.ws),
                                                self.ws_bytes, _lib.stream_ptr()), "sed_crnn_buffers_init")
        if teacher is not None:
            _lib.check(self.l.sed_crnn_buffers_init(C.byref(self.dims), _lib.ptr(self.ctx_t), self.ctx_bytes, None, 0,
                                                    _lib.stream_ptr()), "sed_crnn_buffers_init")
        self._err_view = None
        if student._H == 256:
            off, nb = C.c_size_t(), C.c_size_t()
            _lib.check(self.l.sed_crnn_ctx_view(C.byref(self.dims), b"gru_err", C.byref(off), C.byref(nb)), "sed_crnn_ctx_view")
            self._err_view = (off.value, nb.value)
        self.x = torch.zeros(self.B, 1, self.T, 64, **f32)
        self.x_ema = torch.zeros(self.B, 1, self.T, 64, **f32)
        self.target = torch.zeros(self.B, self.T3, self.NC, **f32)
        self.strong = torch.empty(self.B, self.T3, self.NC, **f32)
        self.weak = torch.empty(self.B, self.NC, **f32)
        self.strong_ema = torch.empty(self.B, self.T3, self.NC, **f32) if teacher is not None else self.strong
        self.weak_ema = torch.empty(self.B, self.NC, **f32) if teacher is not None else self.weak
        self.d_strong = torch.empty(self.B, self.T3, self.NC, **f32)
        self.d_weak = torch.empty(self.B, self.NC, **f32)
        self.losses = torch.zeros(8 + 8 * self.B + 8, **f32)
        self.dp = process_group is not None and (self.world > 1 or os.environ.get("SED_FORCE_DP") == "1")
        self._cap_stream = self._stream("capture")
        want_coll = collective or os.environ.get("SED_DP_COLLECTIVE") or "auto"
        if want_coll not in ("auto", "p2p", "pg"):
            raise ValueError(f"unknown collective {want_coll!r}")
        self._buckets = sdist.grad_buckets(student._layout)
        self._p2p = None
        self.collective_record = None
        if self.dp and want_coll != "pg":
            if sdist.PeerAllReduce.aligned(self.grads, self._buckets + ((0, n),)):
                self._p2p = sdist.PeerAllReduce.create(n, dev, process_group)
            else:
                sdist.PeerAllReduce.last_error = "a gradient bucket does not start on a 16-byte boundary"
            if self._p2p is None and want_coll == "p2p":
                raise _lib.SedError(f"collective='p2p' is not available here: {sdist.PeerAllReduce.last_error}")
            if want_coll == "auto":
                choice, self.collective_record = sdist.choose_collective(self._p2p, self.grads, self._buckets, process_group, dev)
                if choice == "pg" and self._p2p is not None:
                    self._p2p.close()
                    self._p2p = None
        self.collective = "p2p" if self._p2p is not None else ("pg" if self.dp else None)
        env_cap = os.environ.get("SED_DP_CAPTURE")
        want = dp_schedule or os.environ.get("SED_DP_SCHEDULE")
        if want == "split":
            want = "overlap"
        if want not in (None, "overlap", "single"):
            raise ValueError(f"unknown data-parallel schedule {want!r}")
        self.dp_capture = False
        if self.dp and use_graph and env_cap != "0" and (want != "single" or env_cap == "1"):
            self.dp_capture = (env_cap == "1") or self._p2p is not None or self._collective_capture_works()
        self.dp_schedule = want or ("overlap" if (self.dp_capture or not self.dp) else "single")
        self._dp_stream = self._stream("collective") if self.dp else None
        frozen = [not p.requires_grad for p in student.parameters()]
        self.cnn_frozen = all(frozen[:18]) and not any(frozen[18:])
        if any(frozen) and not self.cnn_frozen:
            raise NotImplementedError("MeanTeacherStep supports all parameters trainable, or the whole CNN frozen "
                                      "(train_cnn=False); other requires_grad patterns are not implemented")
        if process_group is not None:
            self.sync_replicas()
        self.use_graph = bool(use_graph)
        self.overlap = bool(overlap_streams)
        self._side = (self._stream("teacher", int(os.environ.get("SED_SIDE_PRIO", "0")))
                      if (self.overlap and teacher is not None) else None)
        self._capture_error = None
        self._graph_a = None
        self._graph_w = None
        self._graph_c = None
        self._graph_b = None
        for st in (torch.cuda.current_stream(dev), self._cap_stream, self._side, self._dp_stream):
            if st is not None:
                _lib.check(self.l.sed_stream_prepare(C.c_void_p(st.cuda_stream)), "sed_stream_prepare")
        self._warm = 0
        self.moments_ahead = os.environ.get("SED_MOMENTS_AHEAD", "0") == "1"
        self._mom_valid = False
        self._resident = False
        self._mom_ready = self._mom_next = False
        self._mom_stream = self._stream("moments", int(os.environ.get("SED_MOM_PRIO", "0")))
        self._mom_fork = os.environ.get("SED_MOM_FORK", "backward")
        self._graph_sets = {}

    @property
    def global_step_host(self):
        return self.steps_done + self._gs_offset

    def _stream(self, role, priority=0):
        if self._pool_streams:
            return shared_stream(self.device, role, priority)
        st = torch.cuda.Stream(device=self.device, priority=int(priority))
        self._owned_streams.append(st)
        return st

    def close(self):
        torch.cuda.synchronize(self.device)
        self._graph_a = self._graph_w = self._graph_c = self._graph_b = None
        self._graph_sets = {}
        if self._p2p is not None:
            self._p2p.close()
            self._p2p = None
        for st in self._owned_streams:
            _lib.check(self.l.sed_stream_release(C.c_void_p(st.cuda_stream)), "sed_stream_release")
        self._owned_streams = []

    def _forward(self, model, x, ctx, seed, strong, weak):
        train = 3 if (model is self.teacher and model is not None) else 1
        if self._mom_ready:
            train |= 4
        _lib.check(self.l.sed_crnn_forward(C.byref(self.dims), _lib.ptr(model._flat), _lib.ptr(model._bn_flat),
                                           _lib.ptr(model._bn_tracked), _lib.ptr(x), train, 1, seed, _lib.ptr(ctx),
                                           self.ctx_bytes, _lib.ptr(strong), _lib.ptr(weak), _lib.stream_ptr()),
                   "sed_crnn_forward")

    def _fwd_bwd(self, after_forward=None, at_recurrence=None):
        self._fork_exc = None
        if self._mom_next and self._mom_fork == "gru" and at_recurrence is None:
            at_recurrence = self._moments_ahead
        try:
            self._fwd_bwd_impl(after_forward, at_recurrence)
        finally:
            if at_recurrence is not None:
                self.l.sed_crnn_fork_callback(_lib.stream_ptr(), None, None)
        if self._fork_exc is not None:
            exc, self._fork_exc = self._fork_exc, None
            raise exc

    def _student_forward(self, at_recurrence):
        if at_recurrence is not None:
            def hook(_user):
                try:
                    at_recurrence()
                except BaseException as e:
                    self._fork_exc = e
            self._fork_cb = _lib.FORK_CALLBACK(hook)
            _lib.check(self.l.sed_crnn_fork_callback(_lib.stream_ptr(), self._fork_cb, None), "sed_crnn_fork_callback")
        if self._defer_heads:
            self._forward(self.student, self.x, self.ctx_s, self._seed_s, None, None)
        else:
            self._forward(self.student, self.x, self.ctx_s, self._seed_s, self.strong, self.weak)

    def _fwd_bwd_impl(self, after_forward=None, at_recurrence=None):
        if self.supervised:
            self._student_forward(at_recurrence)
        elif self._side is not None:
            cur = torch.cuda.current_stream()
            self._side.wait_stream(cur)
            with torch.cuda.stream(self._side):
                self._forward(self.teacher, self.x_ema, self.ctx_t, self._seed_t, self.strong_ema, self.weak_ema)
            self._student_forward(at_recurrence)
            cur.wait_stream(self._side)
        else:
            self._forward(self.teacher, self.x_ema, self.ctx_t, self._seed_t, self.strong_ema, self.weak_ema)
            self._student_forward(at_recurrence)
        if after_forward is not None:
            after_forward()
        if self._mom_next and self._mom_fork != "gru":
            self._moments_ahead()
        if self.cnn_frozen:
            parts = 1
        elif self.dp and self.dp_schedule == "overlap":
            parts = 5
        else:
            parts = 3
        if self._defer_heads:
            _lib.check(self.l.sed_mt_step_backward(C.byref(self.dims), _lib.ptr(self.student._flat), _lib.ptr(self.x),
# ... 120 lines not shown
        cur = torch.cuda.current_stream()
        self._graph_a.replay() if graph else self._fwd_bwd()
        self._dp_stream.wait_stream(cur)
        with torch.cuda.stream(self._dp_stream):
            self._graph_w.replay() if graph else self._dp_tail()
            w1 = self._allreduce(tlo, thi, True)
        self._graph_c.replay() if graph else self._backward(2)
        with torch.cuda.stream(self._dp_stream):
            if w1 is not None:
                w1.wait()
        cur.wait_stream(self._dp_stream)
        w2 = self._allreduce(hlo, hhi, True)
        if w2 is not None:
            w2.wait()
        self._graph_b.replay() if graph else self._update()

    def _dp_step_body(self, after_forward=None, at_recurrence=None):
        (tlo, thi), (hlo, hhi) = self._buckets
        self._fwd_bwd(after_forward, at_recurrence)
        if self.dp_schedule == "single" or self.cnn_frozen:
            self._allreduce(tlo if self.cnn_frozen else 0, thi if self.cnn_frozen else self.n, False)
        else:
            cur = torch.cuda.current_stream()
            self._dp_stream.wait_stream(cur)
            with torch.cuda.stream(self._dp_stream):
                self._dp_tail()
                self._allreduce(tlo, thi, False)
            self._backward(2)
            cur.wait_stream(self._dp_stream)
            self._allreduce(hlo, hhi, False)
        self._update()

    def _step_body(self, after_forward=None, at_recurrence=None):
        if self.dp:
            self._dp_step_body(after_forward, at_recurrence)
        else:
            self._fwd_bwd(after_forward, at_recurrence)
            self._update()

    @property
    def single_graph(self):
        return self.use_graph and (not self.dp or self.dp_capture)

    def load_batch(self, x, x_ema, target):
        self.invalidate_batch()
        self.x.copy_(x.reshape(self.x.shape), non_blocking=True)
        if x_ema is not None:
            self.x_ema.copy_(x_ema.reshape(self.x.shape), non_blocking=True)
        self.target.copy_(target, non_blocking=True)

    def run(self):
        if self._p2p is not None and self._p2p.poll():
            raise _lib.SedError(f"peer all-reduce: {self._p2p.poll()} cross-rank waits ran out of their budget (a rank did not "
                                "launch the same sequence of collectives, died, or fell further behind than SED_P2P_TIMEOUT_S); "
                                "the gradients of that step were filled with NaN")
        key = (self._mom_valid, self._resident and self.moments_ahead)
        self._mom_ready, self._mom_next = key
        graph = self.use_graph and self._warm >= 2
        if graph:
            gs = self._graph_sets.get(key)
            if gs is None:
                mode = (self.dp_capture, self.dp_schedule)
                self._graph_a = self._graph_w = self._graph_c = self._graph_b = None
                self._capture()
                if (self.dp_capture, self.dp_schedule) != mode:
                    self._graph_sets = {}
                gs = self._graph_sets[key] = (self._graph_a, self._graph_w, self._graph_c, self._graph_b)
            self._graph_a, self._graph_w, self._graph_c, self._graph_b = gs
        if not self.dp:
            if graph:
                self._graph_a.replay()
            else:
                self._fwd_bwd()
                self._update()
        elif self.dp_capture:
            self._graph_a.replay() if graph else self._dp_step_body()
        else:
            self._dp_step_eager_collectives(graph)
        self._warm += 1
        self.steps_done += 1
        self._mom_valid = self._mom_next
        self._resident = True
        self._mom_ready = self._mom_next = False

    def step(self, x, x_ema, target):
        self.load_batch(x, x_ema, target)
        self.run()

    def _capture(self):
        torch.cuda.synchronize(self.device)
        cap = dict(stream=self._cap_stream)
        if self.dp:
            cap["capture_error_mode"] = "thread_local"
        if self.dp and not self.dp_capture:
            overlap = self.dp_schedule == "overlap" and not self.cnn_frozen
            ga, gb = torch.cuda.CUDAGraph(), torch.cuda.CUDAGraph()
            with torch.cuda.graph(ga, **cap):
                self._fwd_bwd()
            if overlap:
                gw, gc = torch.cuda.CUDAGraph(), torch.cuda.CUDAGraph()
                with torch.cuda.graph(gw, **cap):
                    self._dp_tail()
                with torch.cuda.graph(gc, **cap):
                    self._backward(2)
                self._graph_w, self._graph_c = gw, gc
            with torch.cuda.graph(gb, **cap):
                self._update()
            self._graph_a, self._graph_b = ga, gb
        elif self.dp:
            import torch.distributed as dist
            ok = 1.0
            try:
                ga = torch.cuda.CUDAGraph()
                with torch.cuda.graph(ga, **cap):
                    self._dp_step_body()
            except Exception as e:
                ok, ga = 0.0, None
                self._capture_error = repr(e)
            flag = torch.tensor([ok], device=self.device)
            dist.all_reduce(flag, op=dist.ReduceOp.MIN, group=self.pg)
            if flag.item() == 1.0:
                self._graph_a = ga
            else:
                self.dp_capture, self.dp_schedule = False, "single"
                torch.cuda.synchronize(self.device)
                self._capture()
        else:
            ga = torch.cuda.CUDAGraph()
            with torch.cuda.graph(ga, **cap):
                self._fwd_bwd()
                self._update()
            self._graph_a = ga

    def meters(self, reduce=False):
        m = self.losses[:8].clone()
        if reduce and self.pg is not None and self.world > 1:
            import torch.distributed as dist
            dist.all_reduce(m, op=dist.ReduceOp.SUM, group=self.pg)
            m /= self.world
        return dict(zip(LOSS_NAMES, m.tolist()))

    def rendezvous(self):
        torch.cuda.synchronize(self.device)
        if self.pg is not None and self.world > 1:
            import torch.distributed as dist
            dist.barrier(group=self.pg)

    def check_health(self):
        if self._p2p is not None:
            n = self._p2p.errors()
            if n:
                raise _lib.SedError(f"peer all-reduce: {n} cross-rank waits timed out (a rank did not launch the same "
                                    "sequence of collectives, or died); gradients since then are invalid")
        if self._err_view is None:
            return
        off, nb = self._err_view
        for name, ctx in (("student", self.ctx_s), ("teacher", self.ctx_t)):
            if ctx.numel():
                n = int(ctx[off:off + 4].view(torch.int32).item())
                if n:
                    raise _lib.SedError(f"cluster GRU recurrence: {n} cross-workgroup waits timed out in the {name} model "
                                        "(the four workgroups of a chain were not co-resident); results are invalid")

    def read_state(self):
        raw = bytes(self.state.cpu().numpy().tobytes())
        return _lib.SedStepState.from_buffer_copy(raw)

    def optimizer_state_dict(self):
        st = self.read_state()
        params = list(self.student.parameters())
        state = {}
        for i, ((o0, o1, shp), _) in enumerate(zip(self.student._layout, params)):
            state[i] = {"step": torch.tensor(float(st.opt_step - 1)),
                        "exp_avg": self.exp_avg[o0:o1].reshape(shp).detach().cpu().clone(),
                        "exp_avg_sq": self.exp_avg_sq[o0:o1].reshape(shp).detach().cpu().clone()}
        group = {"lr": st.lr, "betas": (st.beta1, st.beta2), "eps": st.eps, "weight_decay": 0, "amsgrad": False,
                 "maximize": False, "foreach": None, "capturable": False, "differentiable": False, "fused": None,
                 "params": list(range(len(params)))}
        return {"state": state, "param_groups": [group]}

    def load_optimizer_state_dict(self, sd):
        for i, (o0, o1, _) in enumerate(self.student._layout):
            if i in sd["state"]:
                self.exp_avg[o0:o1].copy_(sd["state"][i]["exp_avg"].reshape(-1))
                self.exp_avg_sq[o0:o1].copy_(sd["state"][i]["exp_avg_sq"].reshape(-1))

    def state_dict(self):
        return {"format": 1,
                "model": {k: {n: t.detach().cpu().clone() for n, t in v.items()} for k, v in self.student.state_dict().items()},
                "model_ema": ({k: {n: t.detach().cpu().clone() for n, t in v.items()}
                               for k, v in self.teacher.state_dict().items()} if self.teacher is not None else None),
                "optimizer": self.optimizer_state_dict(),
                "step_state": bytes(self.state.cpu().numpy().tobytes()),
                "seed_user": self.seed_user,
                "steps_done": self.steps_done}

    def load_state_dict(self, sd):
        assert sd.get("format") == 1, "unknown checkpoint format"
        self.invalidate_batch()
        self.student.load(parameters=sd["model"])
        if self.teacher is not None and sd.get("model_ema") is not None:
            self.teacher.load(parameters=sd["model_ema"])
        self.student.flatten_parameters_(self.device)
        if self.teacher is not None:
            self.teacher.flatten_parameters_(self.device)
        self.load_optimizer_state_dict(sd["optimizer"])
        raw = np.frombuffer(sd["step_state"], dtype=np.uint8).copy()
        assert raw.size == self.state.numel(), "step state size mismatch"
        self.state.copy_(torch.from_numpy(raw))
        self.seed_user = int(sd.get("seed_user", self.seed_user))
        self.steps_done = int(sd.get("steps_done", 0))
        self._gs_offset = int(_lib.SedStepState.from_buffer_copy(bytes(sd["step_state"])).global_step) - self.steps_done
        if self.rank != 0:
            _lib.check(self.l.sed_step_state_update(_lib.ptr(self.state), self._folded_seed(), 0.0, 1, _lib.stream_ptr()),
                       "sed_step_state_update")
        torch.cuda.synchronize(self.device)

    def save_checkpoint(self, path, extra=None):
        self.check_health()
        torch.save(dict(self.state_dict(), **(extra or {})), path)

    def load_checkpoint(self, path):
        sd = torch.load(path, map_location="cpu", weights_only=False)
        self.load_state_dict(sd)
        return sd


def _check_loss(m):
    loss = m["loss"]
    assert not (loss != loss or loss > 1e5), 'Loss explosion: {}'.format(loss)
    assert not loss < 0, 'Loss problem, cannot be negative'


def _epoch_start(step_obj, pg0, epoch, n_batches):
    step_obj.set_lr(pg0["lr"])
    if step_obj.global_step_host != int(epoch) * n_batches:
        step_obj.set_global_step(int(epoch) * n_batches)


def _epoch_end(step_obj, epoch, start, log):
    m = step_obj.meters()
    _check_loss(m)
    step_obj.check_health()
    log('Epoch: {}\tTime {:.2f}\t{}'.format(epoch, time.time() - start,
                                            "\t".join(f"{k} {v:.4g}" for k, v in m.items())))
    return m


def _train_resident(rset, model, optimizer, epoch, ema_model, weak_mask, strong_mask, n_epoch, log, check_every):
    from .resident import ResidentFrontEnd
    start = time.time()
    n_batches = len(rset)
    pg0 = optimizer.param_groups[0]
    weak_mask, strong_mask = rset.step_masks(weak_mask, strong_mask)
    step_obj = getattr(model, "_mt_step", None)
    if step_obj is not None and rset.process_group is not None:
        B = step_obj.B
        have = (step_obj.wlo, step_obj.whi, step_obj.slo, step_obj.shi)
        want = (_slice_range(weak_mask, B) if weak_mask is not None else (0, 0)) + \
               (_slice_range(strong_mask, B) if strong_mask is not None else (0, 0))
        if have != want:
            raise ValueError(f"the model's step was built with masks {have} (weak lo, hi, strong lo, hi); this rank's share of the "
                             f"set needs {want}")
    if step_obj is None:
        model.to(rset.device)
        if ema_model is not None:
            ema_model.to(rset.device)
        step_obj = MeanTeacherStep(model, ema_model, rset.batch, rset.frames, n_batches * n_epoch // 2, weak_mask, strong_mask,
                                   lr=pg0["lr"], betas=pg0["betas"], eps=pg0["eps"], process_group=rset.process_group)
        model._mt_step = step_obj
    fe = getattr(model, "_mt_frontend", None)
    if fe is None or fe.rs is not rset or fe.step is not step_obj:
        fe = model._mt_frontend = ResidentFrontEnd(step_obj, rset)
        fe.aug_epoch = int(epoch)
    _epoch_start(step_obj, pg0, epoch, n_batches)
    for i in range(n_batches):
        fe.run()
        if (i + 1) % check_every == 0:
            _check_loss(step_obj.meters())
            step_obj.check_health()
    return _epoch_end(step_obj, epoch, start, log)


def train(train_loader, model, optimizer, epoch, ema_model=None, weak_mask=None, strong_mask=None, n_epoch=100,
          log=print, check_every=50):
    from .resident import ResidentFeatureSet
    if isinstance(train_loader, ResidentFeatureSet):
        return _train_resident(train_loader, model, optimizer, epoch, ema_model, weak_mask, strong_mask, n_epoch, log,
                               check_every)
    start = time.time()
    step_obj = getattr(model, "_mt_step", None)
    it = iter(train_loader)
    n_batches = len(train_loader)
    pg0 = optimizer.param_groups[0]

    for i in range(n_batches):
        batch = next(it)
        if ema_model is None:
            (batch_input, target), ema_batch_input = batch, None
        else:
            batch_input, ema_batch_input, target = batch
        if step_obj is None:
            B, T = batch_input.shape[0], batch_input.shape[-2]
            dev = torch.device("cuda", torch.cuda.current_device())
            model.to(dev)
            if ema_model is not None:
                ema_model.to(dev)
            step_obj = MeanTeacherStep(model, ema_model, B, T, n_batches * n_epoch // 2, weak_mask, strong_mask,
                                       lr=pg0["lr"], betas=pg0["betas"], eps=pg0["eps"])
            model._mt_step = step_obj
        if i == 0:
            _epoch_start(step_obj, pg0, epoch, n_batches)
        step_obj.step(batch_input.to(step_obj.device, non_blocking=True),
                      ema_batch_input.to(step_obj.device, non_blocking=True) if ema_batch_input is not None else None,
                      target.to(step_obj.device, non_blocking=True))
# ... 5 lines not shown
```

include/dcase_sed.h:

```cpp
#ifndef DCASE_SED_H
#define DCASE_SED_H

#include <stddef.h>
#include <stdint.h>

#ifdef __cplusplus
extern "C" {
#endif

typedef enum {
    SED_OK = 0,
    SED_ERR_BAD_ARG = -1,
    SED_ERR_WORKSPACE = -2,
    SED_ERR_LAUNCH = -3,
    SED_ERR_UNSUPPORTED = -4
} sed_status;

#define SED_DTYPE_F32 0
#define SED_DTYPE_BF16 1
#define SED_DTYPE_BF16X3 2
#define SED_DTYPE_F16 3
typedef struct {
    int32_t B;
    int32_t T;
    int32_t F;
    int32_t C;
    int32_t H;
    int32_t nclass;
    int32_t n_layers_rnn;
    float   p_drop;
    float   bn_eps;
    float   bn_momentum;
    int32_t dtype;
} sed_dims;

typedef struct {
    int64_t  global_step;
    int64_t  opt_step;
    int64_t  rampup_length;
    uint64_t base_seed;
    uint64_t seed_student;
    uint64_t seed_teacher;
    double   lr, beta1, beta2, eps;
    double   ema_decay;
    double   max_cons_cost;
    float    cons_weight;
    float    ema_alpha;
    float    adam_step_size;
    float    adam_sqrt_bc2;
} sed_step_state;

const char* sed_last_error(void);
int sed_version(void);

int sed_param_count(const sed_dims* d);
int sed_param_layout(const sed_dims* d, int64_t* offsets);

size_t sed_crnn_ctx_bytes(const sed_dims* d);
int sed_crnn_forward(const sed_dims* d, const float* params, float* bn_running, int64_t* bn_tracked,
                     const float* x, int train, int update_bn, const uint64_t* seed_dev,
                     void* ctx, size_t ctx_bytes, float* strong, float* weak, void* stream);

int sed_crnn_moments(const sed_dims* d, const float* x, void* ctx, size_t ctx_bytes, void* stream);

int sed_stream_prepare(void* stream);
int sed_stream_release(void* stream);
int sed_crnn_fork_callback(void* stream, void (*fn)(void*), void* user);
size_t sed_crnn_bwd_ws_bytes(const sed_dims* d);
int sed_crnn_backward(const sed_dims* d, const float* params, const float* x, const uint64_t* seed_dev,
                      void* ctx, size_t ctx_bytes, const float* d_strong, const float* d_weak,
                      float* grads, void* ws, size_t ws_bytes, int parts, void* stream);

int sed_crnn_buffers_init(const sed_dims* d, void* ctx, size_t ctx_bytes, void* ws, size_t ws_bytes, void* stream);

int sed_crnn_ctx_view(const sed_dims* d, const char* name, size_t* offset, size_t* bytes);

#define SED_LOSS_FLOATS(B) (8 + 8 * (B) + 8)
int sed_mt_loss(const sed_dims* d, const float* strong, const float* weak, const float* strong_ema,
                const float* weak_ema, const float* target, int weak_lo, int weak_hi, int strong_lo,
                int strong_hi, const sed_step_state* state_dev, float* losses, float* d_strong,
                float* d_weak, void* stream);

int sed_mt_loss_backward(const sed_dims* d, const float* params, const float* x, const uint64_t* seed_dev,
                         void* ctx, size_t ctx_bytes, const float* strong_ema, const float* weak_ema,
                         const float* target, int weak_lo, int weak_hi, int strong_lo, int strong_hi,
                         sed_step_state* state_dev, int advance_state, float* losses, float* d_strong, float* d_weak,
                         float* grads, void* ws, size_t ws_bytes, int parts, void* stream);

int sed_mt_step_backward(const sed_dims* d, const float* params, const float* x, const uint64_t* seed_dev,
                         void* ctx, size_t ctx_bytes, float* strong, float* weak, const float* strong_ema,
                         const float* weak_ema, const float* target, int weak_lo, int weak_hi, int strong_lo, int strong_hi,
                         sed_step_state* state_dev, int advance_state, float* losses, float* d_strong, float* d_weak,
                         float* grads, void* ws, size_t ws_bytes, int parts, void* stream);

size_t sed_p2p_buffer_bytes(long long n_floats_max);
int sed_p2p_alloc(size_t bytes, int fine_grained, void** ptr_out, void* handle_out, int* fine_grained_out);
int sed_p2p_open(const void* handle, void** ptr_out);
int sed_p2p_close(void* peer_ptr);
int sed_p2p_free(void* own_ptr);
int sed_p2p_can_access(int peer_device);
int sed_p2p_errors(const void* own_ptr, unsigned int* out);
int sed_p2p_configure(void* own_ptr, double timeout_s, unsigned int* host_err, int clear_host_err);
int sed_p2p_allreduce(float* data, long long n, int rank, int world, void* const* bufs, long long n_floats_max,
                      int workgroups, void* stream);

int sed_adam_ema(int64_t n, float* params, const float* grads, float* exp_avg, float* exp_avg_sq,
                 float* ema_params, const sed_step_state* state_dev, float grad_scale, void* stream);

int sed_ema_update(int64_t n, const float* params, float* ema_params, float alpha, void* stream);

int sed_step_state_init(sed_step_state* state_dev, uint64_t base_seed, int64_t rampup_length,
                        double lr, double beta1, double beta2, double eps, double ema_decay,
                        double max_cons_cost, void* stream);
int sed_step_state_advance(sed_step_state* state_dev, void* stream);
int sed_step_state_update(sed_step_state* state_dev, uint64_t base_seed, double lr, int flags, void* stream);
int sed_step_state_set_global_step(sed_step_state* state_dev, int64_t global_step, void* stream);

size_t sed_mel_spec_ws_bytes(int n_clips, int n_samples, int hop, int n_fft, int n_mels);
int sed_mel_spec(const float* wave, int n_clips, int n_samples, int hop, int n_fft,
                 const float* window, const float* mel_basis, int n_mels, float* mel,
                 void* ws, size_t ws_bytes, void* stream);
#define SED_FFT_F64 0
#define SED_FFT_F32 1
int sed_mel_tables(int n_fft, const float* window, const float* mel_basis, int n_mels, void* ws, size_t ws_bytes,
                   void* stream);
int sed_mel_frames(const float* wave, int n_clips, int n_samples, int hop, int n_fft, const float* mel_basis,
                   int n_mels, float* mel, const void* ws, size_t ws_bytes, int fft_dtype, int max_workgroups,
                   void* stream);

size_t sed_logmel_transform_ws_bytes(int n_clips);
int sed_seed_advance(uint64_t* key_dev, void* stream);
int sed_logmel_transform(const float* mel, int n_clips, int frames, int n_mels, int max_frames,
                         const double* mean, const double* std, const uint64_t* seed_dev,
                         float* out_clean, float* out_noisy, void* ws, size_t ws_bytes, int math_dtype, void* stream);
int sed_gather_logmel_transform(const float* pool, const int64_t* clip_offset, const int32_t* clip_frames, int n_pool,
                                int max_clip_frames, const int32_t* idx, int B, int n_mels, int max_frames,
                                const double* mean, const double* std, const uint64_t* seed_dev, float* out_clean,
                                float* out_noisy, const float* tgt_pool, int tgt_elems, float* out_target, void* ws,
                                size_t ws_bytes, int math_dtype, void* stream);
int sed_gather_window_logmel_transform(const float* pool, const int64_t* clip_offset, const int32_t* clip_frames, int n_pool,
                                       int max_win_frames, const int32_t* win, int B, int n_mels, int max_frames,
                                       int pool_ratio, const double* mean, const double* std, const uint64_t* seed_dev,
                                       float* out_clean, float* out_noisy, const float* label_pool,
                                       const int64_t* label_offset, const int32_t* label_rows, int T3, int nclass,
                                       float* out_target, void* ws, size_t ws_bytes, int math_dtype, void* stream);

int sed_batch_augment(const float* x, const float* x_ema, const float* target, const int32_t* table, int B, int T,
                      int M, int T3, int NC, float* out_x, float* out_x_ema, float* out_target, void* stream);

int sed_resample(const double* x, int n_clips, int n_in, double ratio, const double* interp_win, int nwin,
                 int num_table, const double* time_reg, double* y, int n_out, void* stream);

int sed_scaler_stats(const float* x, long long n_rows, int n_cols, double* sums, void* stream);

int sed_postprocess(const float* strong, int n_clips, int T, int nclass, float threshold,
                    int median_window, uint8_t* binary, int32_t* ev_count, int32_t* ev_pairs,
                    int max_events, void* stream);

size_t sed_stitch_decode_ws_bytes(long long total_frames, int n_rec, int nclass);
int sed_stitch_tile_frames(void);
int sed_stitch_decode(const float* win_strong, const int32_t* rec_win0, const int64_t* rec_frame0, int n_rec, int T3,
                      int NC, int hop3, int weighting, const float* thr, const int32_t* win, float* timeline,
                      uint8_t* binary, int64_t* ev_ptr, int32_t* ev_pairs, long long capacity, void* ws,
                      size_t ws_bytes, int32_t* err, void* stream);

size_t sed_stitch_sweep_ws_bytes(long long total_frames, int n_rec, int nclass, int n_points);
int sed_stitch_sweep_point_group(void);
int sed_stitch_sweep(const float* win_strong, const int32_t* rec_win0, const int64_t* rec_frame0, int n_rec, int T3,
                     int NC, int hop3, int weighting, int n_points, const float* thr, const int32_t* win,
                     float* timeline, int64_t* ev_ptr, int32_t* ev_pairs, long long capacity, void* ws, size_t ws_bytes,
                     int32_t* err, void* stream);

int sed_event_counts(const float* strong, int n_clips, int T, int nclass, int n_points, const float* thr,
                     const int32_t* win, double num, double den, const int32_t* est_ptr, const double* est_on,
                     const double* est_off, const int32_t* ref_ptr, const double* ref_on, const double* ref_off,
                     double t_collar, double percentage_of_length, double time_resolution, int32_t* ev_counts,
                     int32_t* seg_counts, int64_t* ev_total, int64_t* seg_total, int32_t* err, void* stream);
int sed_weak_counts(const float* weak, const uint8_t* labels, int n_clips, int nclass, const float* thr,
                    int n_points, int64_t* counts, void* stream);

int sed_psds_counts(const float* strong, int n_clips, int T, int nclass, int n_points, const float* thr,
                    const int32_t* win, double num, double den, const int32_t* est_ptr, const double* est_on,
                    const double* est_off, const int32_t* ref_ptr, const double* ref_on, const double* ref_off,
                    double dtc, double gtc, double cttc, int32_t* columns, int64_t* totals, int32_t* err,
                    void* stream);

size_t sed_long_score_ws_bytes(long long est_capacity, long long ref_events, int n_rec, int nclass);
int sed_long_tile_events(void);
int sed_long_event_counts(const int64_t* ev_ptr, const int32_t* ev_pairs, double num, double den, const double* est_on,
                          const double* est_off, long long est_capacity, const int64_t* ref_ptr, const double* ref_on,
                          const double* ref_off, long long ref_events, int n_rec, int nclass, double t_collar,
                          double percentage_of_length, double time_resolution, int32_t* ev_counts, int32_t* seg_counts,
                          int64_t* ev_total, int64_t* seg_total, int32_t* err, void* ws, size_t ws_bytes, void* stream);
int sed_long_psds_counts(const int64_t* ev_ptr, const int32_t* ev_pairs, double num, double den, const double* est_on,
                         const double* est_off, long long est_capacity, const int64_t* ref_ptr, const double* ref_on,
                         const double* ref_off, long long ref_events, int n_rec, int nclass, double dtc, double gtc,
                         double cttc, int32_t* columns, int64_t* totals, int32_t* err, void* ws, size_t ws_bytes,
                         void* stream);

size_t sed_long_sweep_ws_bytes(long long est_capacity, long long ref_events, int n_rec, int nclass, int n_points);
int sed_long_sweep_event_counts(const int64_t* ev_ptr, const int32_t* ev_pairs, double num, double den,
                                const double* est_on, const double* est_off, long long est_capacity,
                                const int64_t* ref_ptr, const double* ref_on, const double* ref_off, long long ref_events,
                                int n_rec, int nclass, int n_points, double t_collar, double percentage_of_length,
                                double time_resolution, int32_t* ev_counts, int32_t* seg_counts, int64_t* ev_total,
                                int64_t* seg_total, int32_t* err, void* ws, size_t ws_bytes, void* stream);
int sed_long_sweep_psds_counts(const int64_t* ev_ptr, const int32_t* ev_pairs, double num, double den,
                               const double* est_on, const double* est_off, long long est_capacity,
                               const int64_t* ref_ptr, const double* ref_on, const double* ref_off, long long ref_events,
                               int n_rec, int nclass, int n_points, double dtc, double gtc, double cttc, int32_t* columns,
                               int64_t* totals, int32_t* err, void* ws, size_t ws_bytes, void* stream);

int sed_kernel_replay(const char* name, const sed_dims* d, const float* params, const float* x,
                      const uint64_t* seed_dev, void* ctx, size_t ctx_bytes, float* grads, void* ws,
                      size_t ws_bytes, void* stream);

#define SED_DEBUG_DIRECT_CONV    (1 << 6)
#define SED_DEBUG_DIRECT_WGRAD   (1 << 7)
#define SED_DEBUG_STFT_R2        (1 << 19)
#define SED_DEBUG_STFT_R3        (1 << 21)
#define SED_DEBUG_SEPARATE_HEADS (1 << 24)
#define SED_DEBUG_SLAB_WGRAD     (1 << 26)
#define SED_DEBUG_STRICT_F32     (1 << 27)
#define SED_DEBUG_SAVED_GATES    (1 << 28)
#define SED_DEBUG_NO_SIDE_STREAM (1 << 30)
int sed_debug_set(int flags);
int sed_build_flags(void);

int sed_selftest(float* out_dev4, void* ws, size_t ws_bytes, void* stream);

#ifdef __cplusplus
}
#endif
#endif
```

Before: 34440.

## Fuse both bidirectional GRU layers into one kernel with cross-workgroup handover

```diff
diff --git a/dcase2019_task4_amd/_lib.py b/dcase2019_task4_amd/_lib.py
--- a/dcase2019_task4_amd/_lib.py
+++ b/dcase2019_task4_amd/_lib.py
@@ -80,6 +80,7 @@
     "sed_crnn_backward": (C.c_int, [C.POINTER(SedDims), _P, _P, _P, _P, C.c_size_t, _P, _P, _P, _P, C.c_size_t, C.c_int, _P]),
     "sed_crnn_buffers_init": (C.c_int, [C.POINTER(SedDims), _P, C.c_size_t, _P, C.c_size_t, _P]),
     "sed_crnn_ctx_view": (C.c_int, [C.POINTER(SedDims), C.c_char_p, C.POINTER(C.c_size_t), C.POINTER(C.c_size_t)]),
+    "sed_crnn_ws_view": (C.c_int, [C.POINTER(SedDims), C.c_char_p, C.POINTER(C.c_size_t), C.POINTER(C.c_size_t)]),
     "sed_mt_loss": (C.c_int, [C.POINTER(SedDims), _P, _P, _P, _P, _P, C.c_int, C.c_int, C.c_int, C.c_int, _P, _P, _P, _P, _P]),
     "sed_mt_loss_backward": (C.c_int, [C.POINTER(SedDims), _P, _P, _P, _P, C.c_size_t, _P, _P, _P, C.c_int, C.c_int, C.c_int,
                                        C.c_int, _P, C.c_int, _P, _P, _P, _P, _P, C.c_size_t, C.c_int, _P]),
diff --git a/dcase2019_task4_amd/crnn.py b/dcase2019_task4_amd/crnn.py
--- a/dcase2019_task4_amd/crnn.py
+++ b/dcase2019_task4_amd/crnn.py
@@ -326,10 +326,10 @@
         return strong, weak
 
     def check_recurrence(self):
-        if self._H == 256 and self._last_ctx is not None:
+        if self._last_ctx is not None:
             n = int(self.ctx_view("gru_err").view(torch.int32)[0].item())
             if n:
-                raise _lib.SedError(f"cluster GRU recurrence: {n} cross-workgroup waits timed out; the outputs are invalid")
+                raise _lib.SedError(f"GRU recurrence: {n} cross-workgroup waits timed out; the outputs are invalid")
 
     def ctx_view(self, name):
         cbuf, dims = self._last_ctx
diff --git a/dcase2019_task4_amd/csrc/common.h b/dcase2019_task4_amd/csrc/common.h
--- a/dcase2019_task4_amd/csrc/common.h
+++ b/dcase2019_task4_amd/csrc/common.h
@@ -88,6 +88,7 @@
     size_t gates[2], out[2];
     size_t logits_s, strong_sv, weak_sv, den_sv;
     size_t mask0, mask1, mask2;
+    size_t gru_err, gru_flag[2], gru_epoch[2];
     size_t total;
 };
 CtxLayout make_ctx_layout(const Geo& g);
diff --git a/dcase2019_task4_amd/csrc/crnn.hip b/dcase2019_task4_amd/csrc/crnn.hip
--- a/dcase2019_task4_amd/csrc/crnn.hip
+++ b/dcase2019_task4_amd/csrc/crnn.hip
@@ -98,6 +98,8 @@
     auto mask_bytes = [](size_t Q) { return ((Q + 3) / 4) * 2 * 64 * sizeof(uint16_t); };
     put(L.mask0, mask_bytes((size_t)g.B * g.H1 * g.W1)); put(L.mask1, mask_bytes((size_t)g.B * g.H2 * g.W2));
     put(L.mask2, mask_bytes((size_t)g.B * g.T3));
+    put(L.gru_err, 256);
+    for (int i = 0; i < 2; ++i) { put(L.gru_flag[i], (size_t)2 * g.B * 4); put(L.gru_epoch[i], (size_t)g.B * 4); }
     L.total = o;
     return L;
 }
@@ -148,6 +150,11 @@
     SED_TRY(sed_validate_dims(d));
     const Geo g = make_geo(d);
     if (g.generic) return gen_buffers_init(g, ctx, ctx_bytes, ws, ws_bytes, (hipStream_t)stream);
+    if (ctx) {
+        const CtxLayout L = make_ctx_layout(g);
+        if (ctx_bytes < L.total) { sed_set_error("sed_crnn_buffers_init: ctx has %zu bytes, needs %zu", ctx_bytes, L.total); return SED_ERR_WORKSPACE; }
+        SED_CHECK_HIP(hipMemsetAsync((char*)ctx + L.gru_err, 0, L.total - L.gru_err, (hipStream_t)stream));
+    }
     return SED_OK;
 }
 
@@ -164,11 +171,29 @@
         {"y2", L.y2, n1}, {"stat2", L.stat2, 1024}, {"bn2", L.bn2, 1024}, {"p2", L.p2, bt * 64 * 4},
         {"gates0", L.gates[0], bt * 512 * 4}, {"gates1", L.gates[1], bt * 512 * 4},
         {"gru0", L.out[0], bt * 128 * 4}, {"gru1", L.out[1], bt * 128 * 4},
-        {"logits_s", L.logits_s, bt * g.NC * 4}, {"den", L.den_sv, (size_t)g.B * g.NC * 4},
+        {"logits_s", L.logits_s, bt * g.NC * 4}, {"den", L.den_sv, (size_t)g.B * g.NC * 4}, {"gru_err", L.gru_err, 4},
     };
     for (auto& t : tab)
         if (strcmp(t.n, name) == 0) { *offset = t.o; *bytes = t.b; return SED_OK; }
     sed_set_error("sed_crnn_ctx_view: unknown buffer '%s'", name);
+    return SED_ERR_BAD_ARG;
+}
+
+extern "C" int sed_crnn_ws_view(const sed_dims* d, const char* name, size_t* offset, size_t* bytes) {
+    SED_TRY(sed_validate_dims(d));
+    SED_CHECK_ARG(name && offset && bytes, "null argument");
+    const Geo g = make_geo(d);
+    if (g.generic) return gen_ws_view(g, name, offset, bytes);
+    const WsLayout W = make_ws_layout(g);
+    const size_t bt = (size_t)g.B * g.T3;
+    struct { const char* n; size_t o, b; } tab[] = {
+        {"d_out", W.d_out, bt * 128 * 4}, {"dgi0", W.dgi[0], bt * 384 * 4}, {"dgh0", W.dgh[0], bt * 384 * 4}, {"hprev0", W.hprev[0], bt * 128 * 4},
+        {"dgi1", W.dgi[1], bt * 384 * 4}, {"dgh1", W.dgh[1], bt * 384 * 4}, {"hprev1", W.hprev[1], bt * 128 * 4},
+        {"d_in", W.d_in, 2 * bt * 128 * 4}, {"dp2", W.dp2, 2 * bt * 64 * 4},
+    };
+    for (auto& t : tab)
+        if (strcmp(t.n, name) == 0) { *offset = t.o; *bytes = t.b; return SED_OK; }
+    sed_set_error("sed_crnn_ws_view: unknown buffer '%s'", name);
     return SED_ERR_BAD_ARG;
 }
 
@@ -272,6 +297,8 @@
     R.p2 = CTXF(L.p2);
     for (int l = 0; l < 2; ++l) { R.out[l] = CTXF(L.out[l]); R.gates[l] = CTXF(L.gates[l]); }
     R.logits_s = CTXF(L.logits_s); R.strong_sv = CTXF(L.strong_sv); R.weak_sv = CTXF(L.weak_sv); R.den_sv = CTXF(L.den_sv);
+    R.err = (int*)((char*)ctx + L.gru_err);
+    R.epoch[0] = (unsigned int*)((char*)ctx + L.gru_flag[ws ? 1 : 0]); R.epoch[1] = (unsigned int*)((char*)ctx + L.gru_epoch[ws ? 1 : 0]);
     if (ws == nullptr) return R;
     const WsLayout& W = *Wp;
     R.d_out = WSF(W.d_out); R.d_in = WSF(W.d_in); R.dp2 = WSF(W.dp2); R.heads_part = WSF(W.heads_part);
diff --git a/dcase2019_task4_amd/csrc/gcrnn.hip b/dcase2019_task4_amd/csrc/gcrnn.hip
--- a/dcase2019_task4_amd/csrc/gcrnn.hip
+++ b/dcase2019_task4_amd/csrc/gcrnn.hip
@@ -115,6 +115,20 @@
     for (auto& t : tab)
         if (strcmp(t.n, name) == 0) { *offset = t.o; *bytes = t.b; return SED_OK; }
     sed_set_error("sed_crnn_ctx_view: unknown buffer '%s'", name);
+    return SED_ERR_BAD_ARG;
+}
+
+int gen_ws_view(const Geo& g, const char* name, size_t* offset, size_t* bytes) {
+    const GWs W = make_gws(g);
+    const size_t H = g.H, bt = (size_t)g.B * g.T3;
+    struct { const char* n; size_t o, b; } tab[] = {
+        {"d_out", W.d_out, bt * 2 * H * 4}, {"dgi0", W.dgi[0], bt * 6 * H * 4}, {"dgh0", W.dgh[0], bt * 6 * H * 4}, {"hprev0", W.hprev[0], bt * 2 * H * 4},
+        {"dgi1", W.dgi[1], bt * 6 * H * 4}, {"dgh1", W.dgh[1], bt * 6 * H * 4}, {"hprev1", W.hprev[1], bt * 2 * H * 4},
+        {"d_in", W.d_in, (H == 64 ? 2 : 1) * bt * 2 * H * 4}, {"dp2", W.dp[2], (H == 64 ? 2 : 1) * bt * g.C * 4},
+    };
+    for (auto& t : tab)
+        if (strcmp(t.n, name) == 0) { *offset = t.o; *bytes = t.b; return SED_OK; }
+    sed_set_error("sed_crnn_ws_view: unknown buffer '%s'", name);
     return SED_ERR_BAD_ARG;
 }
 
diff --git a/dcase2019_task4_amd/csrc/gkernels.h b/dcase2019_task4_amd/csrc/gkernels.h
--- a/dcase2019_task4_amd/csrc/gkernels.h
+++ b/dcase2019_task4_amd/csrc/gkernels.h
@@ -83,6 +83,7 @@
 size_t gen_ws_bytes(const Geo& g);
 int gen_buffers_init(const Geo& g, void* ctx, size_t ctx_bytes, void* ws, size_t ws_bytes, hipStream_t st);
 int gen_ctx_view(const Geo& g, const char* name, size_t* offset, size_t* bytes);
+int gen_ws_view(const Geo& g, const char* name, size_t* offset, size_t* bytes);
 int gen_mompart(const Geo& g, void* ctx, size_t ctx_bytes, double** out);
 int gen_forward(const Geo& g, const ParamOff& P, const float* params, float* bn_running, int64_t* bn_tracked, const float* x,
                 int train, int update_bn, const uint64_t* seed_dev, void* ctx, size_t ctx_bytes, float* strong, float* weak,
diff --git a/dcase2019_task4_amd/csrc/gru4.hip b/dcase2019_task4_amd/csrc/gru4.hip
--- a/dcase2019_task4_amd/csrc/gru4.hip
+++ b/dcase2019_task4_amd/csrc/gru4.hip
@@ -495,6 +495,535 @@
     TSW(3, 0);
 }
 
+#define G4_SPIN_LIMIT (1 << 22)
+__device__ __forceinline__ void g4_pair_ids(int& b, int& dir) {
+    const int i = blockIdx.x;
+    b = (i >> 4) * 8 + (i & 7);
+    dir = (i >> 3) & 1;
+}
+static int g4_pair_grid(int B) { return 16 * ((B + 7) / 8); }
+__device__ __forceinline__ void g4_store_wt(float* p, float v) { __hip_atomic_store(p, v, __ATOMIC_RELAXED, __HIP_MEMORY_SCOPE_AGENT); }
+__device__ __forceinline__ float g4_load_wt(const float* p) { return __hip_atomic_load(p, __ATOMIC_RELAXED, __HIP_MEMORY_SCOPE_AGENT); }
+__device__ __forceinline__ void g4_drain_stores() { asm volatile("s_waitcnt vmcnt(0)" ::: "memory"); }
+__device__ __forceinline__ void g4_handover(const GruPairSync& sy, int b, int dir, unsigned int tag) {
+    g4_drain_stores();
+    if ((threadIdx.x & 63) == 0) {
+        __hip_atomic_store(sy.flag + 2 * b + dir, tag, __ATOMIC_RELAXED, __HIP_MEMORY_SCOPE_AGENT);
+        int it = 0;
+        while (__hip_atomic_load(sy.flag + 2 * b + 1 - dir, __ATOMIC_RELAXED, __HIP_MEMORY_SCOPE_AGENT) != tag && ++it < G4_SPIN_LIMIT)
+            __builtin_amdgcn_s_sleep(1);
+        if (it >= G4_SPIN_LIMIT) atomicAdd(sy.err, 1);
+        if (dir == 0) __hip_atomic_store(sy.epoch + b, tag, __ATOMIC_RELAXED, __HIP_MEMORY_SCOPE_AGENT);
+    }
+    __builtin_amdgcn_fence(__ATOMIC_ACQUIRE, "wavefront");
+}
+
+struct G4Smem { float *zero, *gi_s, *hist, *xs; };
+__device__ __forceinline__ G4Smem g4f_smem(float* gsm) {
+    G4Smem S;
+    S.zero = gsm; S.gi_s = S.zero + 64; S.hist = S.gi_s + 2 * G4_SB * 192; S.xs = S.hist + 2 * G4_SB * 320;
+    return S;
+}
+template <int NIN, bool HAND> __device__ __forceinline__ void g4f_io(const float* x, float* __restrict__ out, float* __restrict__ gates,
+                                                                     int b, int dir, int l, int T, const G4Smem& S) {
+    constexpr int XS = NIN + 4, XPL = NIN / 64;
+    const int nblk = (T + G4_SB - 1) / G4_SB;
+    auto t_of = [&](int step) { return dir ? (T - 1 - step) : step; };
+    auto x_load = [&](int blk, float (&v)[G4_SB * XPL]) {
+#pragma unroll
+        for (int i = 0; i < G4_SB * XPL; ++i) {
+            const int st = min(blk * G4_SB + i / XPL, T - 1);
+            const float* p = x + (size_t)(b * T + t_of(st)) * NIN + 64 * (i % XPL) + l;
+            v[i] = (HAND && NIN == 128) ? g4_load_wt(p) : *p;
+        }
+    };
+    auto x_store = [&](int blk, const float (&v)[G4_SB * XPL]) {
+        float* d = S.xs + (blk & 1) * G4_SB * XS;
+#pragma unroll
+        for (int i = 0; i < G4_SB * XPL; ++i) d[(i / XPL) * XS + 64 * (i % XPL) + l] = v[i];
+    };
+    auto put_row = [&](int blk, int s) {
+        const float* hp = S.hist + (blk & 1) * G4_SB * 320 + s * 320;
+        const int t = t_of(blk * G4_SB + s);
+        float v[5];
+#pragma unroll
+        for (int a = 0; a < 5; ++a) v[a] = hp[64 * a + l];
+        if (HAND && NIN == 64) g4_store_wt(out + (size_t)(b * T + t) * 128 + dir * 64 + l, v[0]);
+        else out[(size_t)(b * T + t) * 128 + dir * 64 + l] = v[0];
+        if (gates) {
+#pragma unroll
+            for (int a = 1; a < 5; ++a) gates[((size_t)(b * T + t) * 2 + dir) * 256 + 64 * (a - 1) + l] = v[a];
+        }
+    };
+    {
+        float xv0[G4_SB * XPL], xv1[G4_SB * XPL];
+        x_load(0, xv0);
+        if (nblk > 1) x_load(1, xv1);
+        x_store(0, xv0);
+        if (nblk > 1) x_store(1, xv1);
+    }
+    __syncthreads();
+    __syncthreads();
+    for (int blk = 0; blk < nblk; ++blk) {
+        const int sb = min(G4_SB, T - blk * G4_SB);
+        float nxt[G4_SB * XPL];
+        const bool more = blk + 2 < nblk;
+        if (more) x_load(blk + 2, nxt);
+        for (int s = 0; s < sb; ++s) {
+            if (blk > 0) put_row(blk - 1, s);
+            if (s == sb - 1 && more) x_store(blk + 2, nxt);
+            lds_barrier();
+        }
+    }
+    const int blk = nblk - 1, sb = T - blk * G4_SB;
+    if (blk > 0)
+        for (int s = sb; s < G4_SB; ++s) put_row(blk - 1, s);
+    for (int s = 0; s < sb; ++s) put_row(blk, s);
+}
+template <int NIN> __device__ __forceinline__ void g4f_proj_load(const float* __restrict__ wih, const float* __restrict__ bih, int pw,
+                                                                 int i16, int kq, float (&bw)[3][NIN / 4], float (&bi)[3]) {
+#pragma unroll
+    for (int c = 0; c < 3; ++c) {
+        const int gcol = 16 * (pw * 3 + c) + i16;
+#pragma unroll
+        for (int s16 = 0; s16 < NIN / 16; ++s16) {
+            const v4f w4 = *(const v4f*)(wih + (size_t)gcol * NIN + 16 * s16 + 4 * kq);
+            bw[c][4 * s16] = w4.x; bw[c][4 * s16 + 1] = w4.y; bw[c][4 * s16 + 2] = w4.z; bw[c][4 * s16 + 3] = w4.w;
+        }
+        bi[c] = bih[gcol];
+    }
+}
+template <int NIN, class Idle> __device__ __forceinline__ void g4f_proj(const float (&bw)[3][NIN / 4], const float (&bi)[3], int pw, int i16,
+                                                                       int kq, int T, const G4Smem& S, Idle idle) {
+    constexpr int XS = NIN + 4, KS = NIN / 4, KPS = KS / G4_SB;
+    const int nblk = (T + G4_SB - 1) / G4_SB;
+    auto proj_block = [&](int blk, bool sync) {
+        const float* A = S.xs + (blk & 1) * G4_SB * XS + i16 * XS + 4 * kq;
+        v4f acc[3];
+#pragma unroll
+        for (int c = 0; c < 3; ++c) acc[c] = (v4f){0.f, 0.f, 0.f, 0.f};
+        v4f a4 = {0.f, 0.f, 0.f, 0.f};
+#pragma unroll
+        for (int ks = 0; ks < KS; ++ks) {
+            if ((ks & 3) == 0) a4 = *(const v4f*)(A + 4 * ks);
+#pragma unroll
+            for (int c = 0; c < 3; ++c) acc[c] = __builtin_amdgcn_mfma_f32_16x16x4f32(a4[ks & 3], bw[c][ks], acc[c], 0, 0, 0);
+            if (sync && (ks + 1) % KPS == 0 && ks + 1 >= 2 * KPS) lds_barrier();
+        }
+        float* gd = S.gi_s + (blk & 1) * G4_SB * 192;
+#pragma unroll
+        for (int c = 0; c < 3; ++c)
+#pragma unroll
+            for (int r = 0; r < 4; ++r) gd[(4 * kq + r) * 192 + 16 * (pw * 3 + c) + i16] = acc[c][r] + bi[c];
+        if (sync) lds_barrier();
+    };
+    __syncthreads();
+    proj_block(0, false);
+    __syncthreads();
+    for (int blk = 0; blk + 1 < nblk; ++blk) proj_block(blk + 1, true);
+    idle();
+    const int sb = T - (nblk - 1) * G4_SB;
+    for (int s = 0; s < sb; ++s) lds_barrier();
+}
+struct G4RecW { v2f wr[8], wz[8], wn[8]; float bh_r, bh_z, bh_n; };
+__device__ __forceinline__ void g4f_rec_load(const float* __restrict__ whh, const float* __restrict__ bhh, int j, int kq, G4RecW& W) {
+#pragma unroll
+    for (int q = 0; q < 4; ++q) {
+        const v4f a = *(const v4f*)(whh + (size_t)j * 64 + 16 * kq + 4 * q);
+        const v4f c = *(const v4f*)(whh + (size_t)(64 + j) * 64 + 16 * kq + 4 * q);
+        const v4f d = *(const v4f*)(whh + (size_t)(128 + j) * 64 + 16 * kq + 4 * q);
+        W.wr[2 * q] = a.xy; W.wr[2 * q + 1] = a.zw;
+        W.wz[2 * q] = c.xy; W.wz[2 * q + 1] = c.zw;
+        W.wn[2 * q] = d.xy; W.wn[2 * q + 1] = d.zw;
+    }
+    W.bh_r = bhh[j]; W.bh_z = bhh[64 + j]; W.bh_n = bhh[128 + j];
+}
+__device__ __forceinline__ void g4f_rec_pin(G4RecW& W) {
+#pragma unroll
+    for (int q = 0; q < 8; ++q) asm volatile("" : "+v"(W.wr[q]), "+v"(W.wz[q]), "+v"(W.wn[q]));
+    asm volatile("" : "+v"(W.bh_r), "+v"(W.bh_z), "+v"(W.bh_n));
+}
+__device__ __forceinline__ void g4f_rec_steps(const G4RecW& W, int j, int kq, int T, const G4Smem& S) {
+    const int nblk = (T + G4_SB - 1) / G4_SB;
+    const float* hrow = S.zero;
+    float hprev = 0.f;
+    const int wofs = 64 * kq + j;
+    const bool is0 = kq == 0, is1 = kq == 1, is2 = kq == 2, is3 = kq == 3;
+    for (int blk = 0; blk < nblk; ++blk) {
+        const int cur = blk & 1, sb = min(G4_SB, T - blk * G4_SB);
+        const float* gib = S.gi_s + cur * G4_SB * 192;
+        float* hb = S.hist + cur * G4_SB * 320;
+        float gi_r = gib[j], gi_z = gib[64 + j], gi_n = gib[128 + j];
+        for (int s = 0; s < sb; ++s) {
+            v4f h4[4];
+#pragma unroll
+            for (int q = 0; q < 4; ++q) h4[q] = *(const v4f*)(hrow + 16 * kq + 4 * q);
+            const float* gr = gib + min(s + 1, G4_SB - 1) * 192;
+            const float gn_r = gr[j], gn_z = gr[64 + j], gn_n = gr[128 + j];
+            __builtin_amdgcn_sched_barrier(0);
+            v2f ar0 = {is0 ? gi_r + W.bh_r : 0.f, 0.f}, ar1 = {0.f, 0.f}, az0 = {is0 ? gi_z + W.bh_z : 0.f, 0.f}, az1 = {0.f, 0.f};
+            v2f an0 = {is0 ? W.bh_n : 0.f, 0.f}, an1 = {0.f, 0.f};
+#pragma unroll
+            for (int q = 0; q < 4; ++q) {
+                ar0 = g4_pkfma(W.wr[2 * q], h4[q].xy, ar0); ar1 = g4_pkfma(W.wr[2 * q + 1], h4[q].zw, ar1);
+                az0 = g4_pkfma(W.wz[2 * q], h4[q].xy, az0); az1 = g4_pkfma(W.wz[2 * q + 1], h4[q].zw, az1);
+                an0 = g4_pkfma(W.wn[2 * q], h4[q].xy, an0); an1 = g4_pkfma(W.wn[2 * q + 1], h4[q].zw, an1);
+            }
+            const v2f sr = ar0 + ar1, sz = az0 + az1, sn = an0 + an1;
+            const float pre_r = g4_quad_sum(sr.x + sr.y);
+            const float pre_z = g4_quad_sum(sz.x + sz.y);
+            const float ghn = g4_quad_sum(sn.x + sn.y);
+            const float r = sigmoidf_fast(pre_r);
+            const float z = sigmoidf_fast(pre_z);
+            const float nn = g4_tanh(gi_n + r * ghn);
+            const float h = (1.0f - z) * nn + z * hprev;
+            float* ho = hb + s * 320;
+            float v = h;
+            v = is1 ? r : v;
+            v = is2 ? z : v;
+            v = is3 ? nn : v;
+            ho[wofs] = v;
+            ho[256 + j] = ghn;
+            hrow = ho;
+            hprev = h;
+            gi_r = gn_r; gi_z = gn_z; gi_n = gn_n;
+            lds_barrier();
+        }
+    }
+}
+
+__global__ __launch_bounds__(G4_THREADS) void k_gru4_fwd2(const float* __restrict__ x, GruLayerW w0, GruLayerW w1, float* out0,
+                                                           float* __restrict__ gates0, float* __restrict__ out1,
+                                                           float* __restrict__ gates1, GruPairSync sy, int B, int T) {
+    extern __shared__ __attribute__((aligned(16))) float gsm[];
+    const G4Smem S = g4f_smem(gsm);
+    int b, dir;
+    g4_pair_ids(b, dir);
+    if (b >= B) return;
+    const int tid = threadIdx.x, role = tid >> 6, l = tid & 63;
+    if (role == 4) {
+        const unsigned int tag = __hip_atomic_load(sy.epoch + b, __ATOMIC_RELAXED, __HIP_MEMORY_SCOPE_AGENT) + 1u;
+        g4f_io<64, true>(x, out0, gates0, b, dir, l, T, S);
+        g4_handover(sy, b, dir, tag);
+        g4f_io<128, true>(out0, out1, gates1, b, dir, l, T, S);
+        return;
+    }
+    if (role >= 5) {
+        const int pw = role - 5, i16 = l & 15, kq = l >> 4;
+        float bwa[3][16], bia[3], bwb[3][32], bib[3];
+        g4f_proj_load<64>(w0.w_ih[dir], w0.b_ih[dir], pw, i16, kq, bwa, bia);
+        g4f_proj<64>(bwa, bia, pw, i16, kq, T, S, [&]() { g4f_proj_load<128>(w1.w_ih[dir], w1.b_ih[dir], pw, i16, kq, bwb, bib); });
+#pragma unroll
+        for (int c = 0; c < 3; ++c) {
+#pragma unroll
+            for (int k = 0; k < 32; ++k) asm volatile("" : "+v"(bwb[c][k]));
+            asm volatile("" : "+v"(bib[c]));
+        }
+        g4f_proj<128>(bwb, bib, pw, i16, kq, T, S, []() {});
+        return;
+    }
+    const int w = role, u = l >> 2, kq = l & 3, j = 16 * w + u;
+    G4RecW Wa, Wb;
+    g4f_rec_load(w0.w_hh[dir], w0.b_hh[dir], j, kq, Wa);
+    g4f_rec_load(w1.w_hh[dir], w1.b_hh[dir], j, kq, Wb);
+    if (w == 0) S.zero[l] = 0.f;
+    __syncthreads();
+    g4f_rec_pin(Wa);
+    g4f_rec_pin(Wb);
+    __syncthreads();
+    __builtin_amdgcn_s_setprio(3);
+    g4f_rec_steps(Wa, j, kq, T, S);
+    __syncthreads();
+    __syncthreads();
+    g4f_rec_steps(Wb, j, kq, T, S);
+}
+
+struct G4BTens { const float *out, *gates; float *dgi, *dgh, *hprev, *dx; };
+struct G4BW { const float *w_hh[2], *w_ih[2]; };
+struct G4BSmem { float *zero, *ops, *hist, *dout_s; };
+__device__ __forceinline__ int g4_opaque(int v) { asm volatile("" : "+s"(v)); return v; }
+__device__ __forceinline__ const float* g4_opaque(const float* p) { asm volatile("" : "+s"(p)); return p; }
+__device__ __forceinline__ int g4_opaque_lane(int v) { asm volatile("" : "+v"(v)); return v; }
+__device__ __forceinline__ G4BSmem g4b_smem(float* gsm) {
+    G4BSmem S;
+    S.zero = gsm; S.ops = S.zero + 192; S.hist = S.ops + 2 * G4_SB * 384; S.dout_s = S.hist + 2 * G4_SB * G4_HS;
+    return S;
+}
+__device__ __forceinline__ int g4b_t_of(int dir, int T, int step) { return dir ? step : (T - 1 - step); }
+template <bool HEADS, bool HAND = false> __device__ __forceinline__ float g4b_op_load(const G4BTens& Y, const float* d_out, const float* d_out2, const G4BSmem& S, int b, int dir, int l, int T,
+                                                                   int step, int a, bool& ok) {
+    const int t = g4b_t_of(dir, T, min(step, T - 1));
+    const int tp = dir ? t + 1 : t - 1;
+    const int tpc = min(max(tp, 0), T - 1);
+    ok = (step < T) && (a != 5 || (tp >= 0 && tp < T));
+    if constexpr (HEADS) {
+        if (a == 0) return S.dout_s[t * 64 + l];
+    }
+    if constexpr (HAND) {
+        if (a == 0) return g4_load_wt(d_out + (size_t)(b * T + t) * 128 + dir * 64 + l);
+    }
+    const float* p = (a == 0) ? d_out + (size_t)(b * T + t) * 128 + dir * 64 + l
+                   : (a < 5) ? Y.gates + ((size_t)(b * T + t) * 2 + dir) * 256 + (a - 1) * 64 + l
+                             : Y.out + (size_t)(b * T + tpc) * 128 + dir * 64 + l;
+    return *p;
+}
+__device__ __forceinline__ void g4b_pre_load(const G4BTens& Y, const G4BSmem& S, int b, int dir, int l, int T, int io, float (&pre)[48],
+                                             unsigned long long& pre_ok) {
+#pragma unroll
+    for (int i = 0; i < 6 * G4_SB / 2; ++i) {
+        bool ok = false;
+        pre[i] = (i % 6 == 0) ? 0.f : g4b_op_load<false>(Y, nullptr, nullptr, S, b, dir, l, T, 2 * (i / 6) + io, i % 6, ok);
+        pre_ok |= (ok ? 1ull : 0ull) << i;
+    }
+}
+template <bool HEADS, bool PRE, bool HAND, class Idle>
+__device__ __forceinline__ void g4b_io(const G4BTens& Y, const float* d_out, const float* d_out2, const G4BSmem& S, int b, int dir, int l, int T, int io, float (&pre)[48],
+                                       unsigned long long pre_ok, Idle idle) {
+    const int nblk = (T + G4_SB - 1) / G4_SB;
+    auto ops_load = [&](int blk, float (&v)[6 * G4_SB / 2], float (&v2)[G4_SB / 2], unsigned long long& okm) {
+        okm = 0;
+#pragma unroll
+        for (int i = 0; i < 6 * G4_SB / 2; ++i) {
+            bool ok;
+            v[i] = g4b_op_load<HEADS, HAND>(Y, d_out, d_out2, S, b, dir, l, T, blk * G4_SB + 2 * (i / 6) + io, i % 6, ok);
+            okm |= (ok ? 1ull : 0ull) << i;
+        }
+#pragma unroll
+        for (int i = 0; i < G4_SB / 2; ++i) {
+            const int t = g4b_t_of(dir, T, min(blk * G4_SB + 2 * i + io, T - 1));
+            v2[i] = (!HEADS && d_out2) ? (HAND ? g4_load_wt(d_out2 + (size_t)(b * T + t) * 128 + dir * 64 + l) : d_out2[(size_t)(b * T + t) * 128 + dir * 64 + l]) : 0.f;
+        }
+    };
+    auto ops_store = [&](int blk, const float (&v)[6 * G4_SB / 2], const float (&v2)[G4_SB / 2], unsigned long long okm) {
+        float* on = S.ops + (blk & 1) * G4_SB * 384;
+#pragma unroll
+        for (int i = 0; i < 6 * G4_SB / 2; ++i) {
+            const float x = (i % 6 == 0) ? v[i] + v2[i / 6] : v[i];
+            on[(2 * (i / 6) + io) * 384 + 64 * (i % 6) + l] = ((okm >> i) & 1ull) ? x : 0.f;
+        }
+    };
+    auto put_row = [&](int blk, int s) {
+        const float* hp = S.hist + (blk & 1) * G4_SB * G4_HS + s * G4_HS;
+        const size_t bt = (size_t)(b * T + g4b_t_of(dir, T, blk * G4_SB + s)) * 2 + dir;
+        float v[7];
+#pragma unroll
+        for (int a = 0; a < 7; ++a) v[a] = hp[64 * a + l];
+#pragma unroll
+        for (int a = 0; a < 3; ++a) Y.dgi[bt * 192 + 64 * a + l] = v[a];
+#pragma unroll
+        for (int a = 3; a < 6; ++a) Y.dgh[bt * 192 + 64 * (a - 3) + l] = v[a];
+        Y.hprev[bt * 64 + l] = v[6];
+    };
+    if constexpr (PRE) {
+        float first2[G4_SB / 2];
+#pragma unroll
+        for (int i = 0; i < G4_SB / 2; ++i) {
+            bool ok = false;
+            pre[6 * i] = g4b_op_load<HEADS, HAND>(Y, d_out, d_out2, S, b, dir, l, T, 2 * i + io, 0, ok);
+            pre_ok |= (ok ? 1ull : 0ull) << (6 * i);
+            const int t = g4b_t_of(dir, T, min(2 * i + io, T - 1));
+            first2[i] = (!HEADS && d_out2) ? (HAND ? g4_load_wt(d_out2 + (size_t)(b * T + t) * 128 + dir * 64 + l) : d_out2[(size_t)(b * T + t) * 128 + dir * 64 + l]) : 0.f;
+        }
+        ops_store(0, pre, first2, pre_ok);
+    } else {
+        float first[6 * G4_SB / 2], first2[G4_SB / 2];
+        unsigned long long okm;
+        ops_load(0, first, first2, okm);
+        ops_store(0, first, first2, okm);
+    }
+    __syncthreads();
+    for (int blk = 0; blk + 1 < nblk; ++blk) {
+        float nxt[6 * G4_SB / 2], nxt2[G4_SB / 2];
+        unsigned long long okm = 0;
+        ops_load(blk + 1, nxt, nxt2, okm);
+        for (int s = 0; s < G4_SB; ++s) {
+            if (blk > 0 && (s & 1) == io) put_row(blk - 1, s);
+            if (s == G4_SB - 1) ops_store(blk + 1, nxt, nxt2, okm);
+            lds_barrier();
+        }
+    }
+    const int blk = nblk - 1, sb = T - blk * G4_SB;
+    idle();
+    for (int s = 0; s < sb; ++s) {
+        if (blk > 0 && (s & 1) == io) put_row(blk - 1, s);
+        lds_barrier();
+    }
+    if (blk > 0)
+        for (int s = sb + ((sb ^ io) & 1); s < G4_SB; s += 2) put_row(blk - 1, s);
+    for (int s = io; s < sb; s += 2) put_row(blk, s);
+}
+template <int NIN> __device__ __forceinline__ void g4b_gemm_load(const float* __restrict__ wih, int gw, int i16, int kq, float (&bw)[NIN / 64][48]) {
+    constexpr int CT = NIN / 64;
+#pragma unroll
+    for (int c = 0; c < CT; ++c)
+#pragma unroll
+        for (int s4 = 0; s4 < 48; ++s4) {
+            bw[c][s4] = wih[(size_t)(4 * s4 + kq) * NIN + 16 * (gw * CT + c) + i16];
+            if (s4 % 16 == 15) __builtin_amdgcn_sched_barrier(0);
+        }
+}
+template <int NIN, bool HAND> __device__ __forceinline__ void g4b_gemm(const float (&bw)[NIN / 64][48], float* plane, const G4BSmem& S, int b, int dir,
+                                                            int gw, int i16, int kq, int T) {
+    constexpr int CT = NIN / 64;
+    const int nblk = (T + G4_SB - 1) / G4_SB;
+    lds_barrier();
+    auto gemm_block = [&](int blk, int n_sync, auto sync_tag) {
+        constexpr bool SYNC = decltype(sync_tag)::value;
+        const int s0 = blk * G4_SB, sb = min(G4_SB, T - s0);
+        const float* hp = S.hist + (blk & 1) * G4_SB * G4_HS + i16 * G4_HS + kq;
+        const bool rowok = i16 < sb;
+        v4f acc[CT];
+#pragma unroll
+        for (int c = 0; c < CT; ++c) acc[c] = (v4f){0.f, 0.f, 0.f, 0.f};
+#pragma unroll
+        for (int s4 = 0; s4 < 48; ++s4) {
+            const float a = rowok ? hp[4 * s4] : 0.f;
+#pragma unroll
+            for (int c = 0; c < CT; ++c) acc[c] = __builtin_amdgcn_mfma_f32_16x16x4f32(a, bw[c][s4], acc[c], 0, 0, 0);
+            if (SYNC && (s4 + 1) % 3 == 0 && (s4 + 1) / 3 <= n_sync) lds_barrier();
+        }
+#pragma unroll
+        for (int r = 0; r < 4; ++r) {
+            const int s = 4 * kq + r;
+            if (s < sb) {
+                float* dst = plane + (size_t)(b * T + g4b_t_of(dir, T, s0 + s)) * NIN + 16 * gw * CT + i16;
+#pragma unroll
+                for (int c = 0; c < CT; ++c) {
+                    if constexpr (HAND) g4_store_wt(dst + 16 * c, acc[c][r]);
+                    else dst[16 * c] = acc[c][r];
+                }
+            }
+        }
+    };
+    for (int blk = 0; blk < nblk; ++blk) {
+        const int sb = min(G4_SB, T - blk * G4_SB);
+        if (blk > 0) gemm_block(blk - 1, sb, std::true_type{});
+        else
+            for (int s = 0; s < sb; ++s) lds_barrier();
+    }
+    gemm_block(nblk - 1, 0, std::false_type{});
+}
+__device__ __forceinline__ void g4b_rec_steps(const float (&wt)[48], const G4BSmem& S, int kq, int u, int j, int T) {
+    const int nblk = (T + G4_SB - 1) / G4_SB;
+    const int wofs1 = (kq < 3) ? 64 * kq + j : 384 + j;
+    const int wofs2 = (kq < 3) ? 192 + 64 * kq + j : 384 + j;
+    const int rofs = 48 * kq + u;
+    const float* dgrow = S.zero;
+    float dhz = 0.f;
+    const bool is1 = kq == 1, is2 = kq == 2, is3 = kq == 3;
+    for (int blk = 0; blk < nblk; ++blk) {
+        const int cur = blk & 1, sb = min(G4_SB, T - blk * G4_SB);
+        const float* ob = S.ops + cur * G4_SB * 384;
+        float* hb = S.hist + cur * G4_SB * G4_HS;
+        float dout = ob[j], r = ob[64 + j], z = ob[128 + j], nn = ob[192 + j], ghn = ob[256 + j], hp = ob[320 + j];
+        for (int s = 0; s < sb; ++s) {
+            float dgv[3];
+#pragma unroll
+            for (int m = 0; m < 3; ++m) dgv[m] = dgrow[rofs + 16 * m];
+            const float* o = ob + min(s + 1, G4_SB - 1) * 384;
+            const float n_dout = o[j], n_r = o[64 + j], n_z = o[128 + j], n_nn = o[192 + j], n_ghn = o[256 + j], n_hp = o[320 + j];
+            __builtin_amdgcn_sched_barrier(0);
+            float acc[3] = {0.f, 0.f, 0.f};
+            G4Rot<0>::dot3(acc, dgv, wt);
+            const float dh = dout + (dhz + g4_row4_sum((acc[0] + acc[1]) + acc[2]));
+            const float dn_pre = dh * (1.0f - z) * (1.0f - nn * nn);
+            const float dz_pre = dh * (hp - nn) * z * (1.0f - z);
+            const float dr_pre = dn_pre * ghn * r * (1.0f - r);
+            const float dghn = dn_pre * r;
+            float* ho = hb + s * G4_HS;
+            float v1 = dr_pre, v2 = dr_pre;
+            v1 = is1 ? dz_pre : v1; v2 = is1 ? dz_pre : v2;
+            v1 = is2 ? dn_pre : v1; v2 = is2 ? dghn : v2;
+            v1 = is3 ? hp : v1;     v2 = is3 ? hp : v2;
+            ho[wofs1] = v1;
+            ho[wofs2] = v2;
+            dgrow = ho + 192;
+            dhz = dh * z;
+            dout = n_dout; r = n_r; z = n_z; nn = n_nn; ghn = n_ghn; hp = n_hp;
+            lds_barrier();
+        }
+    }
+}
+
+struct G4BLate { G4BTens y0; G4BW w0; GruPairSync sy; };
+typedef const __attribute__((address_space(4))) G4BLate* G4BLatePtr;
+__device__ __forceinline__ G4BLatePtr g4b_late() {
+    G4BLatePtr p = (G4BLatePtr)__builtin_amdgcn_kernarg_segment_ptr();
+    asm volatile("" : "+s"(p));
+    return p;
+}
+__device__ __forceinline__ G4BTens g4b_late_y0() {
+    const G4BLatePtr p = g4b_late();
+    return G4BTens{p->y0.out, p->y0.gates, p->y0.dgi, p->y0.dgh, p->y0.hprev, p->y0.dx};
+}
+__device__ __forceinline__ GruPairSync g4b_late_sy() {
+    const G4BLatePtr p = g4b_late();
+    return GruPairSync{p->sy.flag, p->sy.epoch, p->sy.err};
+}
+
+template <bool HEADS>
+__global__ __launch_bounds__(G4B_THREADS) void k_gru4_bwd2(G4BLate, const float* __restrict__ d_top, G4BTens y1, G4BW w1, int B, int T, HeadsFuse hf) {
+    extern __shared__ __attribute__((aligned(16))) float gsm[];
+    const G4BSmem S = g4b_smem(gsm);
+    int b, dir;
+    g4_pair_ids(b, dir);
+    if (b >= B) return;
+    const int tid = threadIdx.x, role = tid >> 6, l = tid & 63;
+    float pre[48], wt0[48];
+    unsigned long long pre_ok = 0;
+    unsigned int tag = 0;
+    if (role < 4) {
+        G4Rot<0>::load_bwd(pre, w1.w_hh[dir], l >> 4, l & 15, 16 * role + (l & 15));
+    } else if (role < 6) {
+        if (role == 4) tag = __hip_atomic_load(g4b_late()->sy.epoch + b, __ATOMIC_RELAXED, __HIP_MEMORY_SCOPE_AGENT) + 1u;
+        if constexpr (HEADS) g4b_pre_load(y1, S, b, dir, l, T, role - 4, pre, pre_ok);
+    }
+    if constexpr (HEADS) heads_fused_phase<G4B_THREADS>(hf, y1.out, b, dir, 2 * B, 2 * b + dir, T, S.ops, S.dout_s);
+
+    if (role == 4 || role == 5) {
+        const int io = role - 4;
+        float pre0[48];
+        unsigned long long pre0_ok = 0;
+        g4b_io<HEADS, HEADS, false>(y1, d_top, nullptr, S, b, dir, l, T, io, pre, pre_ok, [&]() { g4b_pre_load(g4b_late_y0(), S, b, dir, l, g4_opaque(T), io, pre0, pre0_ok); });
+        __syncthreads();
+        if (io == 0) g4_handover(g4b_late_sy(), b, dir, tag);
+        lds_barrier();
+        __builtin_amdgcn_fence(__ATOMIC_ACQUIRE, "wavefront");
+        const int T0 = g4_opaque(T);
+        g4b_io<false, true, true>(g4b_late_y0(), y1.dx, y1.dx + (size_t)B * T0 * 128, S, b, dir, l, T0, io, pre0, pre0_ok, []() {});
+        return;
+    }
+    if (role >= 6) {
+        const int gw = role - 6, i16 = l & 15, kq = l >> 4;
+        {
+            float bw[2][48];
+            g4b_gemm_load<128>(w1.w_ih[dir], gw, i16, kq, bw);
+            g4b_gemm<128, true>(bw, y1.dx + (size_t)dir * B * T * 128, S, b, dir, gw, i16, kq, T);
+        }
+        g4_drain_stores();
+        __syncthreads();
+        float bw[1][48];
+        const int T0 = g4_opaque(T), tid0 = g4_opaque_lane(tid), gw0 = (tid0 >> 6) - 6, i16b = tid0 & 15, kqb = (tid0 & 63) >> 4;
+        const G4BLatePtr late = g4b_late();
+        g4b_gemm_load<64>(late->w0.w_ih[dir], gw0, i16b, kqb, bw);
+        lds_barrier();
+        g4b_gemm<64, false>(bw, late->y0.dx + (size_t)dir * B * T0 * 64, S, b, dir, gw0, i16b, kqb, T0);
+        return;
+    }
+    const int w = role, kq = l >> 4, u = l & 15, j = 16 * w + u;
+    for (int e = tid; e < 192; e += 256) S.zero[e] = 0.f;
+#pragma unroll
+    for (int i = 0; i < 48; ++i) asm volatile("" : "+v"(pre[i]));
+    G4Rot<0>::load_bwd(wt0, g4b_late()->w0.w_hh[dir], kq, u, j);
+    __syncthreads();
+    __builtin_amdgcn_s_setprio(3);
+    g4b_rec_steps(pre, S, kq, u, j, T);
+    __syncthreads();
+    lds_barrier();
+    __syncthreads();
+    g4b_rec_steps(wt0, S, kq, u, j, g4_opaque(T));
+}
+
 template <int NIN> static constexpr size_t gru4_fwd_lds() { return (size_t)(64 + 2 * G4_SB * 192 + 2 * G4_SB * 320 + 2 * G4_SB * (NIN + 4)) * sizeof(float); }
 static const size_t GRU4_BWD_LDS = (size_t)(192 + 2 * G4_SB * 384 + 2 * G4_SB * G4_HS) * sizeof(float);
 static_assert(2 * G4_SB * 384 + 2 * G4_SB * G4_HS >= HF_TMAX * HF_S + HF_MAXO * HF_S + HF_TMAX * HF_SD + HF_TMAX * 8 + HF_MISC,
@@ -517,6 +1046,20 @@
         sed_set_error("gru forward: unsupported input width %d", nin);
         return SED_ERR_UNSUPPORTED;
     }
+    SED_CHECK_LAUNCH();
+    return SED_OK;
+}
+
+int launch_gru_fwd2(const float* x, const GruLayerW& w0, const GruLayerW& w1, float* out0, float* gates0, float* out1, float* gates1,
+                    const GruPairSync& sy, int B, int T, hipStream_t st) {
+    if (sy.flag == nullptr || sy.epoch == nullptr || sy.err == nullptr) {
+        sed_set_error("gru forward, both layers: no hand-over words");
+        return SED_ERR_BAD_ARG;
+    }
+    static thread_local SedAttrOnce attr_done;
+    if (attr_done.need())
+        SED_CHECK_HIP(hipFuncSetAttribute((const void*)k_gru4_fwd2, hipFuncAttributeMaxDynamicSharedMemorySize, (int)gru4_fwd_lds<128>()));
+    k_gru4_fwd2<<<g4_pair_grid(B), G4_THREADS, gru4_fwd_lds<128>(), st>>>(x, w0, w1, out0, gates0, out1, gates1, sy, B, T);
     SED_CHECK_LAUNCH();
     return SED_OK;
 }
@@ -569,3 +1112,33 @@
     SED_CHECK_LAUNCH();
     return SED_OK;
 }
+
+int launch_gru_bwd2(const G4BLayer& y1, const G4BLayer& y0, const GruLayerW& lw1, const GruLayerW& lw0, const GruPairSync& sy, int B, int T,
+                    const HeadsFuse* hf, hipStream_t st) {
+    const G4BTens t1 = {y1.out, y1.gates, y1.dgi, y1.dgh, y1.hprev, y1.dx}, t0 = {y0.out, y0.gates, y0.dgi, y0.dgh, y0.hprev, y0.dx};
+    if (y1.d_out2 != nullptr || y0.d_out != y1.dx || y0.d_out2 != y1.dx + (size_t)B * T * 128) {
+        sed_set_error("gru backward, both layers: layer 0's upstream gradient must be the two planes of layer 1's dx");
+        return SED_ERR_BAD_ARG;
+    }
+    const G4BW w1 = {{lw1.w_hh[0], lw1.w_hh[1]}, {lw1.w_ih[0], lw1.w_ih[1]}}, w0 = {{lw0.w_hh[0], lw0.w_hh[1]}, {lw0.w_ih[0], lw0.w_ih[1]}};
+    if (sy.flag == nullptr || sy.epoch == nullptr || sy.err == nullptr) {
+        sed_set_error("gru backward, both layers: no hand-over words");
+        return SED_ERR_BAD_ARG;
+    }
+    if (hf && (T > HF_TMAX || hf->NC < 1 || hf->NC > 16 || hf->hl.strong_ema == nullptr)) {
+        sed_set_error("fused heads + gru backward: needs T/8 <= %d, nclass <= 16 and the loss inputs (got T/8 = %d)", HF_TMAX, T);
+        return SED_ERR_UNSUPPORTED;
+    }
+    const G4BLate late = {t0, w0, sy};
+    static thread_local SedAttrOnce attr_done;
+    if (attr_done.need()) {
+        SED_CHECK_HIP(hipFuncSetAttribute((const void*)k_gru4_bwd2<false>, hipFuncAttributeMaxDynamicSharedMemorySize, (int)GRU4_BWD_LDS));
+        SED_CHECK_HIP(hipFuncSetAttribute((const void*)k_gru4_bwd2<true>, hipFuncAttributeMaxDynamicSharedMemorySize, (int)GRU4_BWD_HEADS_LDS_MAX));
+    }
+    if (hf)
+        k_gru4_bwd2<true><<<g4_pair_grid(B), G4B_THREADS, GRU4_BWD_LDS + (size_t)((T + 15) & ~15) * 64 * sizeof(float), st>>>(late, nullptr, t1, w1, B, T, *hf);
+    else
+        k_gru4_bwd2<false><<<g4_pair_grid(B), G4B_THREADS, GRU4_BWD_LDS, st>>>(late, y1.d_out, t1, w1, B, T, HeadsFuse{});
+    SED_CHECK_LAUNCH();
+    return SED_OK;
+}
diff --git a/dcase2019_task4_amd/csrc/kernels.h b/dcase2019_task4_amd/csrc/kernels.h
--- a/dcase2019_task4_amd/csrc/kernels.h
+++ b/dcase2019_task4_amd/csrc/kernels.h
@@ -186,6 +186,10 @@
 int launch_gru_bwd(const float* d_out, const float* d_out2, const float* out, const float* gates, const float* w_hh_f,
                    const float* w_hh_r, const float* w_ih_f, const float* w_ih_r, int nin, float* dgi, float* dgh, float* hprev,
                    float* dx_planes, int B, int T, hipStream_t st);
+struct GruLayerW { const float *w_ih[2], *b_ih[2], *w_hh[2], *b_hh[2]; };
+struct GruPairSync { unsigned int *flag, *epoch; int* err; };
+int launch_gru_fwd2(const float* x, const GruLayerW& w0, const GruLayerW& w1, float* out0, float* gates0, float* out1, float* gates1,
+                    const GruPairSync& sy, int B, int T, hipStream_t st);
 
 int launch_heads_fwd(const float* h , const float* wd, const float* bd, const float* ws, const float* bs,
                      float* strong, float* weak, float* strong_sv, float* weak_sv, float* logits_s, float* den, int B, int T,
@@ -269,4 +273,10 @@
 int launch_gru_bwd_heads(const float* out, const float* gates, const float* w_hh_f, const float* w_hh_r, const float* w_ih_f,
                          const float* w_ih_r, int nin, float* dgi, float* dgh, float* hprev, float* dx_planes, int B, int T,
                          const HeadsFuse& hf, hipStream_t st);
+struct G4BLayer {
+    const float *d_out, *d_out2, *out, *gates;
+    float *dgi, *dgh, *hprev, *dx;
+};
+int launch_gru_bwd2(const G4BLayer& y1, const G4BLayer& y0, const GruLayerW& w1, const GruLayerW& w0, const GruPairSync& sy, int B, int T,
+                    const HeadsFuse* hf, hipStream_t st);
 int launch_heads_fin(const float* part, float* g_wd, int B, int T, int NC, int n_cols, const HeadsLoss& hl, hipStream_t st);
diff --git a/dcase2019_task4_amd/csrc/rnn.hip b/dcase2019_task4_amd/csrc/rnn.hip
--- a/dcase2019_task4_amd/csrc/rnn.hip
+++ b/dcase2019_task4_amd/csrc/rnn.hip
@@ -1,5 +1,16 @@
 #include "rnn.h"
 #include "gkernels.h"
+
+static bool rnn_layers_fused(const Geo& g) { return g.H == 64 && g.L == 2 && g.C == 64 && !(g_sed_debug & SED_DEBUG_SPLIT_GRU_LAYERS); }
+static GruLayerW rnn_layer_w(const ParamOff& P, const float* params, int l) {
+    GruLayerW w;
+    for (int dir = 0; dir < 2; ++dir) {
+        w.w_ih[dir] = params + P.w_ih[l][dir]; w.b_ih[dir] = params + P.b_ih[l][dir];
+        w.w_hh[dir] = params + P.w_hh[l][dir]; w.b_hh[dir] = params + P.b_hh[l][dir];
+    }
+    return w;
+}
+static GruPairSync rnn_pair_sync(const RnnBufs& R) { return GruPairSync{R.epoch[0], R.epoch[1], R.err}; }
 
 int rnn_forward(const Geo& g, const ParamOff& P, const float* params, const RnnBufs& R, int train, const uint64_t* seed_dev,
                 float* strong, float* weak, int n_whh_packed, hipStream_t st) {
@@ -9,7 +20,11 @@
     const float* in = R.p2;
     int nin = g.C;
     for (int l = 0; l < g.L; ++l) {
-        if (H == 64) {
+        if (rnn_layers_fused(g)) {
+            SED_TRY(launch_gru_fwd2(in, rnn_layer_w(P, params, 0), rnn_layer_w(P, params, 1), R.out[0], train ? R.gates[0] : nullptr, R.out[1],
+                                    train ? R.gates[1] : nullptr, rnn_pair_sync(R), g.B, g.T3, st));
+            l = 1;
+        } else if (H == 64) {
             SED_TRY(launch_gru_fwd(in, nin, params + P.w_ih[l][0], params + P.w_ih[l][1], params + P.b_ih[l][0], params + P.b_ih[l][1],
                                    params + P.w_hh[l][0], params + P.w_hh[l][1], params + P.b_hh[l][0], params + P.b_hh[l][1],
                                    R.out[l], train ? R.gates[l] : nullptr, g.B, g.T3, st));
@@ -114,15 +129,28 @@
                                      R.n_zero, rb.defer_colsum ? 1 : 0, rb.hl, st, 2 * H));
         const float* d_cur = R.d_out;
         const float* d_cur2 = nullptr;
+        HeadsFuse hf = {};
+        if (rb.fuse) {
+            hf.wd = params + P.dense_w; hf.strong = rb.ho->strong; hf.weak = rb.ho->weak; hf.part = R.heads_part;
+            hf.NC = g.NC; hf.use_drop = use_drop; hf.p_drop = g.p; hf.seed = rb.seed_dev;
+            hf.zero = (parts & 2) ? R.zero : nullptr; hf.n_zero = (parts & 2) ? R.n_zero : 0; hf.hl = *rb.hl;
+        }
         for (int l = g.L - 1; l >= 0; --l) {
             const int nin = (l == 0) ? g.C : 2 * H;
             float* d_in = (l == 0) ? R.dp2 : R.d_in;
+            if (rnn_layers_fused(g)) {
+                const G4BLayer y1 = {R.d_out, nullptr, R.out[1], R.gates[1], R.dgi[1], R.dgh[1], R.hprev[1], R.d_in};
+                const G4BLayer y0 = {R.d_in, R.d_in + (size_t)BT * 128, R.out[0], R.gates[0], R.dgi[0], R.dgh[0], R.hprev[0], R.dp2};
+                SED_TRY(launch_gru_bwd2(y1, y0, rnn_layer_w(P, params, 1), rnn_layer_w(P, params, 0), rnn_pair_sync(R), g.B, g.T3,
+                                        rb.fuse ? &hf : nullptr, st));
+                if (rb.fuse) {
+                    if (!rb.defer_colsum) SED_TRY(rnn_heads_colsum(rb, st));
+                    else if (parts & 4) SED_TRY(launch_heads_fin(R.heads_part, grads + P.dense_w, g.B, g.T3, g.NC, 0, *rb.hl, st));
+                }
+                break;
+            }
             if (H == 64) {
                 if (rb.fuse && l == g.L - 1) {
-                    HeadsFuse hf = {};
-                    hf.wd = params + P.dense_w; hf.strong = rb.ho->strong; hf.weak = rb.ho->weak; hf.part = R.heads_part;
-                    hf.NC = g.NC; hf.use_drop = use_drop; hf.p_drop = g.p; hf.seed = rb.seed_dev;
-                    hf.zero = (parts & 2) ? R.zero : nullptr; hf.n_zero = (parts & 2) ? R.n_zero : 0; hf.hl = *rb.hl;
                     SED_TRY(launch_gru_bwd_heads(R.out[l], R.gates[l], params + P.w_hh[l][0], params + P.w_hh[l][1], params + P.w_ih[l][0],
                                                  params + P.w_ih[l][1], nin, R.dgi[l], R.dgh[l], R.hprev[l], d_in, g.B, g.T3, hf, st));
                     if (!rb.defer_colsum) SED_TRY(rnn_heads_colsum(rb, st));
diff --git a/dcase2019_task4_amd/train.py b/dcase2019_task4_amd/train.py
--- a/dcase2019_task4_amd/train.py
+++ b/dcase2019_task4_amd/train.py
@@ -109,11 +109,9 @@
         if teacher is not None:
             _lib.check(self.l.sed_crnn_buffers_init(C.byref(self.dims), _lib.ptr(self.ctx_t), self.ctx_bytes, None, 0,
                                                     _lib.stream_ptr()), "sed_crnn_buffers_init")
-        self._err_view = None
-        if student._H == 256:
-            off, nb = C.c_size_t(), C.c_size_t()
-            _lib.check(self.l.sed_crnn_ctx_view(C.byref(self.dims), b"gru_err", C.byref(off), C.byref(nb)), "sed_crnn_ctx_view")
-            self._err_view = (off.value, nb.value)
+        off, nb = C.c_size_t(), C.c_size_t()
+        _lib.check(self.l.sed_crnn_ctx_view(C.byref(self.dims), b"gru_err", C.byref(off), C.byref(nb)), "sed_crnn_ctx_view")
+        self._err_view = (off.value, nb.value)
         self.x = torch.zeros(self.B, 1, self.T, 64, **f32)
         self.x_ema = torch.zeros(self.B, 1, self.T, 64, **f32)
         self.target = torch.zeros(self.B, self.T3, self.NC, **f32)
@@ -540,15 +538,13 @@
             if n:
                 raise _lib.SedError(f"peer all-reduce: {n} cross-rank waits timed out (a rank did not launch the same "
                                     "sequence of collectives, or died); gradients since then are invalid")
-        if self._err_view is None:
-            return
         off, nb = self._err_view
         for name, ctx in (("student", self.ctx_s), ("teacher", self.ctx_t)):
             if ctx.numel():
                 n = int(ctx[off:off + 4].view(torch.int32).item())
                 if n:
-                    raise _lib.SedError(f"cluster GRU recurrence: {n} cross-workgroup waits timed out in the {name} model "
-                                        "(the four workgroups of a chain were not co-resident); results are invalid")
+                    raise _lib.SedError(f"GRU recurrence: {n} cross-workgroup waits timed out in the {name} model "
+                                        "(the workgroups of a chain or a clip were not co-resident); results are invalid")
 
     def read_state(self):
         raw = bytes(self.state.cpu().numpy().tobytes())
diff --git a/include/dcase_sed.h b/include/dcase_sed.h
--- a/include/dcase_sed.h
+++ b/include/dcase_sed.h
@@ -74,6 +74,7 @@
 int sed_crnn_buffers_init(const sed_dims* d, void* ctx, size_t ctx_bytes, void* ws, size_t ws_bytes, void* stream);
 
 int sed_crnn_ctx_view(const sed_dims* d, const char* name, size_t* offset, size_t* bytes);
+int sed_crnn_ws_view(const sed_dims* d, const char* name, size_t* offset, size_t* bytes);
 
 #define SED_LOSS_FLOATS(B) (8 + 8 * (B) + 8)
 int sed_mt_loss(const sed_dims* d, const float* strong, const float* weak, const float* strong_ema,
@@ -223,6 +224,7 @@
 #define SED_DEBUG_SLAB_WGRAD     (1 << 26)
 #define SED_DEBUG_STRICT_F32     (1 << 27)
 #define SED_DEBUG_SAVED_GATES    (1 << 28)
+#define SED_DEBUG_SPLIT_GRU_LAYERS (1 << 29)
 #define SED_DEBUG_NO_SIDE_STREAM (1 << 30)
 int sed_debug_set(int flags);
 int sed_build_flags(void);
```

After: 34680, median of 6. About the same (+0.7%).
